# JiaoLab2021/varigraph

Measured on AMD Instinct MI355X. Metric: 150 bp reads/sec genotyped (k=27), higher is better.
Workload: dtype u64

## Files before the change

### include/vgmi.h

```cpp
#ifndef VGMI_H
#define VGMI_H

#include <stddef.h>
#include <stdint.h>

#ifdef __cplusplus
extern "C" {
#endif

typedef struct vgmi_ctx vgmi_ctx;

typedef enum vgmi_status {
    VGMI_OK = 0,
    VGMI_E_INVALID = -1,
    VGMI_E_NO_DEVICE = -2,
    VGMI_E_HIP = -3,
    VGMI_E_STATE = -4,
    VGMI_E_DUPLICATE_KEY = -5,
    VGMI_E_BAD_KEY = -6,
    VGMI_E_EMPTY_READ = -7,
    VGMI_E_NOMEM = -8
} vgmi_status;

int vgmi_device_count(void);
int vgmi_create(int device, size_t buffer_mib, vgmi_ctx **out);
void vgmi_destroy(vgmi_ctx *ctx);
const char *vgmi_last_error(const vgmi_ctx *ctx);
int vgmi_device_memory(vgmi_ctx *ctx, size_t *free_bytes, size_t *total_bytes);
void *vgmi_stream(vgmi_ctx *ctx);
int vgmi_device_of(vgmi_ctx *ctx, int *device);

int vgmi_table_upload(vgmi_ctx *ctx, const uint64_t *host_keys, size_t n_keys, uint32_t k);
int vgmi_table_image_bytes(vgmi_ctx *ctx, size_t *bytes);
int vgmi_table_export(vgmi_ctx *ctx, void *dev_dst, size_t bytes);
int vgmi_table_import(vgmi_ctx *ctx, const void *dev_src, size_t bytes);
int vgmi_table_clone(vgmi_ctx *dst, vgmi_ctx *src);
int vgmi_rccl_unique_id(void *id128);
int vgmi_table_broadcast(vgmi_ctx *ctx, int rank, int world, const void *id128);
typedef struct vgmi_comm vgmi_comm;
int vgmi_comm_create(int device, int rank, int world, const void *id128, vgmi_comm **out);
int vgmi_table_broadcast_comm(vgmi_ctx *ctx, vgmi_comm *comm);
int vgmi_table_snapshot(vgmi_ctx *ctx);
void vgmi_comm_destroy(vgmi_comm *comm);
int vgmi_table_info(vgmi_ctx *ctx, size_t *n_keys, uint32_t *k, size_t *n_slots, size_t *filter_bits);
int vgmi_table_lookup(vgmi_ctx *ctx, const uint64_t *host_keys, size_t n, uint32_t *index_out);
int vgmi_xtable_info(vgmi_ctx *ctx, size_t *n_lines, size_t *overflow_pairs);
int vgmi_ctable_info(vgmi_ctx *ctx, size_t *n_buckets, size_t *n_entries, size_t *n_unitigs, size_t *moved_entries,
                     size_t *overflow_kmers);
int vgmi_ctable_defer_info(vgmi_ctx *ctx, uint64_t *deferred_launches, uint64_t *plain_launches, uint32_t *n_bins,
                           uint32_t *region, uint32_t *room, uint32_t *cap);

int vgmi_nodes_upload(vgmi_ctx *ctx, const uint64_t *host_node_off, const uint32_t *host_key_index,
                      size_t n_nodes);
int vgmi_flags_upload(vgmi_ctx *ctx, const uint8_t *host_hom_flag);

int vgmi_counts_reset(vgmi_ctx *ctx);
int vgmi_reads_submit(vgmi_ctx *ctx, const char *host_bases, size_t n_bytes,
                      const uint64_t *host_read_off, size_t n_reads);
int vgmi_reads_submit_device(vgmi_ctx *ctx, const char *dev_bases, size_t n_bytes,
                             const uint64_t *dev_read_off, size_t n_reads);
int vgmi_read_base(vgmi_ctx *ctx, uint64_t *read_base);
int vgmi_counts_finish(vgmi_ctx *ctx, uint8_t *host_cov_out, uint8_t *host_cov_node_out,
                       uint64_t *host_hist256_out);
int vgmi_counts_finish_device(vgmi_ctx *ctx, uint8_t *dev_cov_out, uint8_t *dev_cov_node_out,
                              uint64_t *dev_hist256_out);
int vgmi_counts_export_device(vgmi_ctx *ctx, uint32_t *dev_counts_out );
int vgmi_counts_import_device(vgmi_ctx *ctx, const uint32_t *dev_counts );
int vgmi_count_kernel_ms(vgmi_ctx *ctx, float *ms, uint64_t *launches);

typedef struct vgmi_fastq vgmi_fastq;
int vgmi_fastq_open(vgmi_ctx *ctx, vgmi_fastq **out);
int vgmi_fastq_acquire(vgmi_fastq *fq, char **host_buf, size_t *capacity);
int vgmi_fastq_commit(vgmi_fastq *fq, size_t n_bytes);
int vgmi_fastq_text_capacity(vgmi_fastq *fq, size_t *text_bytes);
int vgmi_fastq_bgzf_want(vgmi_fastq *fq, size_t *comp_bytes);
int vgmi_fastq_commit_bgzf(vgmi_fastq *fq, size_t n_bytes, size_t *taken, size_t *n_text, int *not_bgzf);
int vgmi_fastq_open_bam(vgmi_ctx *ctx, uint64_t header_bytes, int32_t n_ref, vgmi_fastq **out);
int vgmi_fastq_open_fasta(vgmi_ctx *ctx, vgmi_fastq **out);
int vgmi_gunzip_buffer(vgmi_ctx *ctx, const void *host_gz, size_t n, void *host_out, size_t cap, size_t *n_out, size_t *consumed,
                       int *member_end, uint32_t *reason);
int vgmi_fastq_commit_gzip(vgmi_fastq *fq, size_t n_bytes, int at_eof, size_t *taken, size_t *n_text, int *stop);
int vgmi_fastq_gzip_status(vgmi_fastq *fq, uint64_t *device_text_bytes, uint32_t *reason);
int vgmi_fastq_bgzf_status(vgmi_fastq *fq, int *failed, uint64_t *good_compressed_bytes, uint32_t *reason);
int vgmi_fastq_close(vgmi_fastq *fq, uint64_t *n_records, uint64_t *n_bases, uint64_t *consumed_bytes, int *stopped,
                     char *tail_out, size_t tail_cap, size_t *tail_len);

int vgmi_sketch_keys(vgmi_ctx *ctx, const char *host_bases, size_t n_bytes,
                     const uint64_t *host_read_off, size_t n_reads, uint32_t k,
                     uint64_t *host_keys_out);

int vgmi_bloom_params(uint64_t n, double p, uint64_t *m, uint32_t *n_hash);
int vgmi_bloom_create(vgmi_ctx *ctx, uint64_t m, uint32_t n_hash, const uint64_t *host_seeds);
int vgmi_bloom_add_seq(vgmi_ctx *ctx, const char *host_bases, uint64_t len, uint32_t k);
int vgmi_bloom_add_seq_device(vgmi_ctx *ctx, const char *dev_bases, uint64_t len, uint32_t k);
int vgmi_bloom_fetch(vgmi_ctx *ctx, uint8_t *host_filter_out );
int vgmi_bloom_load(vgmi_ctx *ctx, const uint8_t *host_filter );
int vgmi_bloom_save_file(vgmi_ctx *ctx, const char *path);
int vgmi_bloom_load_file(vgmi_ctx *ctx, const char *path);
int vgmi_bloom_query(vgmi_ctx *ctx, const uint64_t *host_keys, size_t n, uint8_t *host_min_out,
                     uint8_t *host_all_nonzero_out);

typedef struct vgmi_hmm_chain {
    uint64_t first_step, n_steps;
    uint32_t keep_index, pad;
} vgmi_hmm_chain;
int vgmi_hmm_recursion(vgmi_ctx *ctx, uint32_t n_gt, uint32_t ploidy, const uint8_t *keep, uint32_t n_windows,
                       const void *obs, uint64_t n_rows, const uint32_t *row, const uint8_t *restart, const void *pow,
                       uint64_t n_steps, const void *uniform, const vgmi_hmm_chain *chains, uint32_t n_chains, void *out);
int vgmi_hmm_recursion_fre(vgmi_ctx *ctx, uint32_t n_gt, uint32_t ploidy, const void *freq, uint32_t n_tables, const void *obs,
                           uint64_t n_rows, const uint32_t *row, const uint8_t *restart, uint64_t n_steps, const void *uniform,
                           const vgmi_hmm_chain *chains, uint32_t n_chains, void *out);
int vgmi_hmm_calls(vgmi_ctx *ctx, uint32_t n_gt, uint32_t ploidy, const uint8_t *keep, uint32_t n_windows, const void *obs,
                   uint64_t n_rows, const uint32_t *row, const uint8_t *restart, const void *pow, uint64_t n_steps,
                   const void *uniform, const vgmi_hmm_chain *chains, uint32_t n_chains, const uint8_t *gid, const uint8_t *order,
                   const uint64_t *fwd_step, const uint64_t *bwd_step, void *prob, uint32_t *winner, void *alpha_beta_or_null);
int vgmi_hmm_calls_part(vgmi_ctx *ctx, uint32_t n_gt, uint32_t ploidy, const uint8_t *keep, uint32_t n_windows, const void *obs,
                        uint64_t row_lo, uint64_t row_hi, const uint32_t *row, const uint8_t *restart, const void *pow,
                        uint64_t step_lo, uint64_t step_hi, const void *uniform, const vgmi_hmm_chain *chains, uint32_t n_chains,
                        const uint8_t *gid, const uint8_t *order, const uint64_t *fwd_step, const uint64_t *bwd_step, void *prob,
                        uint32_t *winner);

typedef struct vgmi_hmm_part vgmi_hmm_part;
int vgmi_hmm_entries_upload(vgmi_ctx *ctx, const uint64_t *host_entries, size_t n_entries);
int vgmi_hmm_sample_upload(vgmi_ctx *ctx, const uint8_t *host_cov_node, size_t n_entries);
int vgmi_hmm_emissions(vgmi_ctx *ctx, uint32_t n_gt, uint32_t n_used, const uint8_t *used, const uint8_t *pos_a, const uint8_t *pos_b,
                       uint64_t top_mask, uint32_t bit_len, float ave, double lower, double upper, const void *tables,
                       uint64_t n_rows, const uint64_t *entry_begin, const uint32_t *entry_count, const uint16_t *gt0,
                       uint32_t *n_kept_out, uint8_t *flags_out, vgmi_hmm_part **out);
int vgmi_hmm_emissions_ploidy(vgmi_ctx *ctx, uint32_t n_gt, uint32_t ploidy, uint32_t n_used, const uint8_t *used, const uint8_t *pos,
                              uint64_t top_mask, uint32_t bit_len, float ave, double lower, double upper, const void *tables, uint64_t n_rows,
                              const uint64_t *entry_begin, const uint32_t *entry_count, const uint16_t *gt0, uint32_t *n_kept_out,
                              uint8_t *flags_out, vgmi_hmm_part **out);
int vgmi_hmm_part_set_rows(vgmi_hmm_part *part, uint64_t n, const uint64_t *rows, const void *obs_rows );
int vgmi_hmm_part_fix_rows(vgmi_hmm_part *part, uint64_t n, const uint64_t *rows, const uint32_t *fix_off, const uint32_t *fix_j,
                           const uint16_t *fix_mask);
int vgmi_hmm_part_calls(vgmi_hmm_part *part, uint32_t ploidy, const uint8_t *keep, uint32_t n_windows, const uint32_t *row,
                        const uint8_t *restart, const void *pow, uint64_t n_steps, const void *uniform, const vgmi_hmm_chain *chains,
                        uint32_t n_chains, const uint8_t *gid, const uint8_t *order, const uint64_t *fwd_step, const uint64_t *bwd_step,
                        void *prob, uint32_t *winner);
int vgmi_hmm_part_calls_fre(vgmi_hmm_part *part, uint32_t ploidy, const void *freq, uint32_t n_tables, const uint32_t *row,
                            const uint8_t *restart, uint64_t n_steps, const void *uniform, const vgmi_hmm_chain *chains, uint32_t n_chains,
                            const uint8_t *gid, const uint8_t *order, const uint64_t *fwd_step, const uint64_t *bwd_step, void *prob,
                            uint32_t *winner);
typedef struct vgmi_hmm_plan vgmi_hmm_plan;
int vgmi_hmm_plan_create(vgmi_ctx *ctx, uint32_t n_gt, uint32_t ploidy, const uint8_t *keep, uint32_t n_windows, uint64_t n_rows,
                         const uint32_t *row, const uint8_t *restart, const void *pow, uint64_t n_steps, const void *uniform,
                         const vgmi_hmm_chain *chains, uint32_t n_chains, const uint8_t *gid, const uint8_t *order, const uint64_t *fwd_step,
                         const uint64_t *bwd_step, vgmi_hmm_plan **out);
int vgmi_hmm_part_calls_plan(vgmi_hmm_part *part, const vgmi_hmm_plan *plan, void *prob, uint32_t *winner);
void vgmi_hmm_plan_free(vgmi_hmm_plan *plan);
int vgmi_hmm_tallies(vgmi_ctx *ctx, uint64_t n_rows, const uint64_t *entry_begin, const uint32_t *entry_count, const uint32_t *winner,
                     uint32_t n_gt, const uint8_t *hap_ab, uint32_t n_hap, uint64_t sel_mask, uint32_t *out, uint8_t *unique_out);
int vgmi_hmm_alive_upload(vgmi_ctx *ctx, const uint8_t *host_alive, size_t n_entries);
int vgmi_hmm_alive_fetch(vgmi_ctx *ctx, uint8_t *host_alive_out, size_t n_entries);
int vgmi_hmm_support(vgmi_ctx *ctx, uint32_t n_hap, uint32_t n_windows, uint64_t n_rows, const uint64_t *entry_begin,
                     const uint32_t *entry_count, const uint32_t *row_win, uint32_t *support_out );
int vgmi_hmm_emissions_select(vgmi_ctx *ctx, uint32_t n_gt, uint32_t n_used, const uint8_t *pos_a, const uint8_t *pos_b, uint32_t n_windows,
                              const uint8_t *win_used , const uint64_t *win_top_mask, uint32_t bit_len, float ave,
                              double lower, double upper, const void *tables, uint64_t n_rows, const uint64_t *entry_begin,
                              const uint32_t *entry_count, const uint32_t *row_win, const uint16_t *gt0, uint32_t *n_kept_out,
                              uint8_t *flags_out, vgmi_hmm_part **out);
int vgmi_hmm_tallies_select(vgmi_ctx *ctx, uint64_t n_rows, const uint64_t *entry_begin, const uint32_t *entry_count, const uint32_t *row_win,
                            const uint32_t *winner, uint32_t n_gt, const uint8_t *pos_a, const uint8_t *pos_b, uint32_t n_used,
                            uint32_t n_windows, const uint8_t *win_used, uint32_t *out, uint8_t *unique_out);
int vgmi_hmm_emissions_select_ploidy(vgmi_ctx *ctx, uint32_t n_gt, uint32_t ploidy, uint32_t n_windows, const uint32_t *win_n_gt,
                                     const uint8_t *win_haps , const uint64_t *win_top_mask, uint32_t bit_len,
                                     float ave, double lower, double upper, const void *tables, uint64_t n_rows, const uint64_t *entry_begin,
                                     const uint32_t *entry_count, const uint32_t *row_win, const uint64_t *gt0, uint32_t *n_kept_out,
                                     uint8_t *flags_out, vgmi_hmm_part **out);
int vgmi_hmm_part_fix_rows_wide(vgmi_hmm_part *part, uint64_t n, const uint64_t *rows, const uint32_t *fix_off, const uint32_t *fix_j,
                                const uint64_t *fix_mask);
int vgmi_hmm_tallies_ploidy(vgmi_ctx *ctx, uint32_t ploidy, uint32_t n_gt, uint32_t n_windows, const uint32_t *win_n_gt ,
                            const uint8_t *win_haps , const uint64_t *win_sel_mask ,
                            uint64_t n_rows, const uint64_t *entry_begin, const uint32_t *entry_count, const uint32_t *row_win ,
                            const uint32_t *winner, int use_alive, uint32_t *out , uint8_t *unique_out);
int vgmi_hmm_entries_upload_wide(vgmi_ctx *ctx, const uint8_t *f, const uint8_t *bits , size_t n_entries, uint32_t bit_len);
int vgmi_hmm_entries_reserve_wide(vgmi_ctx *ctx, size_t n_entries, uint32_t bit_len);
int vgmi_hmm_entries_fill_wide(vgmi_ctx *ctx, size_t first, size_t n, const uint8_t *f, const uint8_t *bits );
int vgmi_hmm_support_wide(vgmi_ctx *ctx, uint32_t bit_len, uint32_t n_hap, uint32_t n_windows, uint64_t n_rows, const uint64_t *entry_begin,
                          const uint32_t *entry_count, const uint32_t *row_win, uint32_t *support_out );
int vgmi_hmm_emissions_select_wide(vgmi_ctx *ctx, uint32_t n_gt, uint32_t n_used, const uint8_t *pos_a, const uint8_t *pos_b, uint32_t n_windows,
                                   const uint8_t *win_used , const uint64_t *win_top_mask ,
                                   uint32_t bit_len, float ave, double lower, double upper, const void *tables, uint64_t n_rows,
                                   const uint64_t *entry_begin, const uint32_t *entry_count, const uint32_t *row_win, const uint16_t *gt0,
                                   uint32_t *n_kept_out, uint8_t *flags_out, vgmi_hmm_part **out);
int vgmi_hmm_tallies_select_wide(vgmi_ctx *ctx, uint32_t bit_len, uint64_t n_rows, const uint64_t *entry_begin, const uint32_t *entry_count,
                                 const uint32_t *row_win, const uint32_t *winner, uint32_t n_gt, const uint8_t *pos_a, const uint8_t *pos_b,
                                 uint32_t n_used, uint32_t n_windows, const uint8_t *win_used, uint32_t *out, uint8_t *unique_out);
int vgmi_hmm_emissions_select_ploidy_wide(vgmi_ctx *ctx, uint32_t n_gt, uint32_t ploidy, uint32_t n_windows, const uint32_t *win_n_gt,
                                          const uint8_t *win_haps , const uint64_t *win_top_mask ,
                                          uint32_t bit_len, float ave, double lower, double upper, const void *tables, uint64_t n_rows,
                                          const uint64_t *entry_begin, const uint32_t *entry_count, const uint32_t *row_win,
                                          const uint64_t *gt0 , uint32_t *n_kept_out, uint8_t *flags_out, vgmi_hmm_part **out);
int vgmi_hmm_part_fix_rows_ploidy_wide(vgmi_hmm_part *part, uint64_t n, const uint64_t *rows, const uint32_t *fix_off, const uint32_t *fix_j,
                                       const uint64_t *fix_mask );
int vgmi_hmm_tallies_ploidy_wide(vgmi_ctx *ctx, uint32_t bit_len, uint32_t ploidy, uint32_t n_gt, uint32_t n_windows, const uint32_t *win_n_gt,
                                 const uint8_t *win_haps, const uint64_t *win_sel_mask , uint64_t n_rows,
                                 const uint64_t *entry_begin, const uint32_t *entry_count, const uint32_t *row_win, const uint32_t *winner,
                                 int use_alive, uint32_t *out , uint8_t *unique_out);
int vgmi_hmm_part_fetch(vgmi_hmm_part *part, void *obs_out);
void vgmi_hmm_part_free(vgmi_hmm_part *part);


#ifdef __cplusplus
}
#endif
#endif
```

### varigraph_amd/csrc/vgmi_api.cpp

```cpp
#include "vgmi_ctx.h"

namespace vgapi {

thread_local std::string g_create_error;

thread_local uint64_t t_err_ctx = 0;
thread_local std::string t_err_msg;

int fail(vgmi_ctx* c, int code, const std::string& msg)
{
    static std::mutex mu;
    std::lock_guard<std::mutex> lock(mu);
    if (c) {
        c->err = msg;
        t_err_ctx = c->id;
        t_err_msg = msg;
    } else g_create_error = msg;
    return code;
}

uint32_t ceil_log2(uint64_t x)
{
    uint32_t l = 0;
    while ((1ULL << l) < x) ++l;
    return l;
}

hipEvent_t get_event(vgmi_ctx* c)
{
    if (!c->event_pool.empty()) {
        hipEvent_t e = c->event_pool.back();
        c->event_pool.pop_back();
        return e;
    }
    hipEvent_t e = nullptr;
    if (hipEventCreate(&e) != hipSuccess) return nullptr;
    return e;
}

void free_table(vgmi_ctx* c)
{
    if (c->d_image) (void)hipFree(c->d_image);
    c->d_image = nullptr;
    if (c->d_snapshot) (void)hipFree(c->d_snapshot);
    c->d_snapshot = nullptr;
    c->image_bytes = 0;
    c->has_table = false;
    if (c->d_cov) (void)hipFree(c->d_cov);
    c->d_cov = nullptr;
    if (c->d_flag) (void)hipFree(c->d_flag);
    c->d_flag = nullptr;
    if (c->d_counts) (void)hipFree(c->d_counts);
    c->d_counts = nullptr;
    if (c->d_sat_dirty) (void)hipFree(c->d_sat_dirty);
    c->d_sat_dirty = nullptr;
    if (c->d_xt_lines) (void)hipFree(c->d_xt_lines);
    if (c->d_xt_counts) (void)hipFree(c->d_xt_counts);
    if (c->d_xt_id) (void)hipFree(c->d_xt_id);
    if (c->d_xt_over) (void)hipFree(c->d_xt_over);
    c->d_xt_over = nullptr;
    c->xt_over_keys = 0;
    if (c->d_ct_buckets && c->ct_vmm_bytes) {
        (void)hipMemUnmap(c->d_ct_buckets, c->ct_vmm_bytes);
        (void)hipMemRelease(c->ct_vmm_handle);
        (void)hipMemAddressFree(c->d_ct_buckets, c->ct_vmm_bytes);
        c->ct_vmm_bytes = 0;
    } else if (c->d_ct_buckets) (void)hipFree(c->d_ct_buckets);
    c->d_ct_buckets = nullptr;
    c->ct_entries = c->ct_unitigs = c->ct_moved = 0;
    for (void* q : {(void*)c->d_pt_index, (void*)c->d_pt_S, (void*)c->d_pt_VB, (void*)c->d_pt_SB, (void*)c->d_pt_SLOT, (void*)c->d_pt_PLACE})
        if (q) (void)hipFree(q);
    c->d_pt_index = nullptr;
    c->d_pt_S = c->d_pt_VB = c->d_pt_SB = c->d_pt_SLOT = c->d_pt_PLACE = nullptr;
    c->tv.pt = PathView{};
    c->d_xt_lines = nullptr;
    c->d_xt_counts = nullptr;
    c->d_xt_id = nullptr;
    c->tv.xt = XTableView{};
}

void free_nodes(vgmi_ctx* c)
{
    if (c->d_node_key_index) (void)hipFree(c->d_node_key_index);
    if (c->d_cov_node) (void)hipFree(c->d_cov_node);
    c->d_node_key_index = nullptr;
    c->d_cov_node = nullptr;
    c->n_nodes = 0;
    c->n_node_entries = 0;
}

int debit_list_of(vgmi_ctx* c, hipStream_t st, unsigned long long** out)
{
    {
        std::lock_guard<std::mutex> lk(c->mu);
        auto it = c->debit_lists.find(st);
        if (it != c->debit_lists.end()) {
            *out = it->second;
            return VGMI_OK;
        }
    }
    unsigned long long* list = nullptr;
    HIPCHK(c, hipMalloc(reinterpret_cast<void**>(&list), (size_t)VG_DEBIT_LIST * 8 + (size_t)VG_DEBIT_SUBLISTS * 64));
    std::lock_guard<std::mutex> lk(c->mu);
    c->debit_lists[st] = list;
    *out = list;
    return VGMI_OK;
}

int ctd_prepare(vgmi_ctx* c, size_t n_bytes, hipStream_t st, CtDefer* d)
{
    const char* const e_on = getenv("VGMI_CT_DEFER");
    const int on = e_on ? atoi(e_on) : VGMI_CT_DEFER_DEFAULT;
    const char* const e_min = getenv("VGMI_CT_DEFER_MIN");
    const size_t min_bytes = e_min ? (size_t)atoll(e_min) : (size_t)512 << 20;
    *d = CtDefer{};
    if (!on || !c->tv.xt.cb || n_bytes < min_bytes) return VGMI_OK;
    const size_t need = ctd_scratch_bytes(n_bytes, c->xt_n_counts, (uint32_t)c->n_cu, d);
    if (!need) return VGMI_OK;
    uint8_t* buf = nullptr;
    size_t have = 0;
    {
        std::lock_guard<std::mutex> lk(c->mu);
        auto it = c->ctd_scratch.find(st);
        if (it != c->ctd_scratch.end()) {
            buf = it->second.first;
            have = it->second.second;
        }
    }
    if (have < need) {
        if (buf) {
            HIPCHK(c, hipStreamSynchronize(st));
            (void)hipFree(buf);
            buf = nullptr;
        }
        if (hipMalloc(reinterpret_cast<void**>(&buf), need) != hipSuccess) {
            (void)hipGetLastError();
            std::lock_guard<std::mutex> lk(c->mu);
            c->ctd_scratch.erase(st);
            *d = CtDefer{};
            return VGMI_OK;
        }
        std::lock_guard<std::mutex> lk(c->mu);
        c->ctd_scratch[st] = std::make_pair(buf, need);
    }
    ctd_layout(buf, d);
    HIPCHK(c, launch_ctd_reset(*d, st));
    return VGMI_OK;
}

int launch_ctable_count(vgmi_ctx* c, const RowParams& p, size_t n_bytes, hipStream_t st)
{
    CtDefer d;
    int rc = ctd_prepare(c, n_bytes, st, &d);
    if (rc) return rc;
    {
        std::lock_guard<std::mutex> lk(c->mu);
        if (d.rec) {
            ++c->ctd_deferred;
            c->ctd_last[0] = d.n_bins, c->ctd_last[1] = d.region, c->ctd_last[2] = d.room, c->ctd_last[3] = d.cap;
        } else
            ++c->ctd_plain;
    }
    HIPCHK(c, launch_count27c(p, c->tv.xt, (uint32_t)c->n_cu, st, &d));
    if (d.rec) HIPCHK(c, launch_ctd_apply(c->tv.xt, d, (uint32_t)c->n_cu, st));
    return VGMI_OK;
}

int xt_clamp_if_due(vgmi_ctx* c, size_t n_bytes, hipStream_t st)
{
    bool due = false;
    {
        std::lock_guard<std::mutex> lk(c->mu);
        c->xt_bytes_since_clamp += n_bytes;
        if (c->xt_bytes_since_clamp >= (1ULL << 31)) {
            c->xt_bytes_since_clamp = 0;
            due = true;
        }
    }
    if (due) HIPCHK(c, launch_xclamp(c->tv.xt, c->xt_n_counts, st));
    return VGMI_OK;
}

}


uint32_t vgmi_dbg_env()
{
    static const uint32_t v = [] {
        const char* d = getenv("VGMI_DBG");
        const uint32_t x = d ? (uint32_t)atoi(d) : 0u;
#ifdef VGMI_ABLATION
        if (x) fprintf(stderr, "[vgmi] WARNING: VGMI_DBG=%u in an ablation build: counters and genotypes are WRONG on purpose\n", x);
        return x;
#else
        if (x) fprintf(stderr, "[vgmi] VGMI_DBG=%u ignored: this library was built without -DVGMI_ABLATION\n", x);
        return 0u;
#endif
    }();
    return v;
}

namespace vgapi {
RowParams row_params(vgmi_ctx* c, const char* d_bases, size_t n_bytes, uint32_t k)
{
    RowParams p{};
    p.bases = reinterpret_cast<const uint8_t*>(d_bases);
    p.n_bytes = n_bytes;
    p.k = k;
    p.status = c->d_status;
    p.table = c->tv;
    p.keys_out = nullptr;
    p.dbg = vgmi_dbg_env();
    static const uint32_t l1_min = [] {
        const char* e = getenv("VGMI_L1_MIN");
        const int v = e ? atoi(e) : 60;
        return (uint32_t)(v < 1 ? 1 : v > 64 ? 64 : v);
    }();
    p.l1_min = l1_min;
    p.bloom = c->bv;
    return p;
}

void rows_geometry(vgmi_ctx* c, bool flds, uint32_t& grid, uint32_t& block)
{
    if (flds) { block = 1024; grid = (uint32_t)c->n_cu; }
    else      { block = 256;  grid = (uint32_t)c->n_cu * 8; }
// ... 295 lines not shown
    if (!c) return VGMI_E_INVALID;
    if (!c->has_table) return fail(c, VGMI_E_STATE, "no table");
    if (n_bytes == 0) return VGMI_OK;
    if (!bases) return fail(c, VGMI_E_INVALID, "bases is NULL");
    if (bases[n_bytes - 1] != '\n') return fail(c, VGMI_E_INVALID, "a read block must end with '\\n'");
    if (n_reads > n_bytes) return fail(c, VGMI_E_INVALID, "n_reads > n_bytes");
    HIPCHK(c, hipSetDevice(c->device));
    const bool need_off = (c->hdr.k & 1) == 0;
    std::vector<uint64_t> derived;
    if (need_off && !read_off) {
        derived = offsets_from_newlines(bases, n_bytes);
        if (derived.size() != n_reads + 1) return fail(c, VGMI_E_INVALID, "n_reads does not match the number of '\\n'");
        read_off = derived.data();
    }
    size_t pos = 0, read_i = 0;
    while (pos < n_bytes) {
        size_t len = n_bytes - pos;
        size_t piece_reads = n_reads - read_i;
        if (len > c->buffer_bytes) {
            len = c->buffer_bytes;
            while (len > 0 && bases[pos + len - 1] != '\n') --len;
            if (len == 0) return fail(c, VGMI_E_INVALID, "a single read exceeds the staging buffer (--buffer)");
            if (need_off) {
                size_t j = read_i;
                while (read_off[j] < pos + len) ++j;
                piece_reads = j - read_i;
            } else {
                piece_reads = 0;
            }
        }
        Stage& s = c->stage[c->next_stage];
        c->next_stage ^= 1;
        int rc = ensure_stage(c, s);
        if (rc) return rc;
        if (s.busy) { HIPCHK(c, hipEventSynchronize(s.done)); s.busy = false; }
        if (s.after_reset) { HIPCHK(c, hipStreamWaitEvent(s.stream, c->reset_done, 0)); s.after_reset = false; }
        memcpy(s.h, bases + pos, len);
        HIPCHK(c, hipMemcpyAsync(s.d, s.h, len, hipMemcpyHostToDevice, s.stream));
        const uint64_t* d_off = nullptr;
        if (need_off) {
            if (s.d_off_cap < piece_reads + 1) {
                if (s.d_off) (void)hipFree(s.d_off);
                s.d_off_cap = (piece_reads + 1) * 2;
                HIPCHK(c, hipMalloc(reinterpret_cast<void**>(&s.d_off), s.d_off_cap * 8));
            }
            std::vector<uint64_t> rel(piece_reads + 1);
            for (size_t j = 0; j <= piece_reads; ++j) rel[j] = read_off[read_i + j] - pos;
            HIPCHK(c, hipMemcpy(s.d_off, rel.data(), rel.size() * 8, hipMemcpyHostToDevice));
            d_off = s.d_off;
        }
        rc = launch_count(c, s.d, len, d_off, piece_reads, s.stream);
        if (rc) return rc;
        HIPCHK(c, hipEventRecord(s.done, s.stream));
        s.busy = true;
        pos += len;
        read_i += piece_reads;
    }
    std::lock_guard<std::mutex> lk(c->mu);
    c->read_base += n_bytes - n_reads;
    return VGMI_OK;
}

int vgmi_read_base(vgmi_ctx* c, uint64_t* rb)
{
    if (!c || !rb) return VGMI_E_INVALID;
    *rb = c->read_base;
    return VGMI_OK;
}

static int finish_common(vgmi_ctx* c, uint8_t* d_cov, uint8_t* d_cov_node, unsigned long long* d_hist)
{
    for (auto& s : c->stage)
        if (s.busy) HIPCHK(c, hipStreamWaitEvent(c->stream, s.done, 0));
    if (d_hist) HIPCHK(c, hipMemsetAsync(d_hist, 0, 256 * 8, c->stream));
    if (c->tv.xt.counts) HIPCHK(c, launch_xcov(c->tv.xt, c->d_xt_id, c->hdr.n_keys, c->d_flag, d_cov, d_hist, c->stream));
    else HIPCHK(c, launch_cov(c->tv, c->d_key_slot, c->hdr.n_keys, c->d_flag, d_cov, d_hist, c->stream));
    if (d_cov_node && c->n_node_entries)
        HIPCHK(c, launch_node_gather(d_cov, c->d_node_key_index, c->n_node_entries, d_cov_node, c->stream));
    return VGMI_OK;
}

int vgmi_counts_finish(vgmi_ctx* c, uint8_t* cov_out, uint8_t* cov_node_out, uint64_t* hist_out)
{
    if (!c) return VGMI_E_INVALID;
    if (!c->has_table) return fail(c, VGMI_E_STATE, "no table");
    if (cov_node_out && !c->d_node_key_index) return fail(c, VGMI_E_STATE, "no nodes uploaded");
    if (hist_out && !c->d_flag) return fail(c, VGMI_E_STATE, "no flags uploaded");
    if (c->open_fastq) return fail(c, VGMI_E_STATE, "close the FASTQ streams first");
    HIPCHK(c, hipSetDevice(c->device));
    int rc = finish_common(c, c->d_cov, cov_node_out ? c->d_cov_node : nullptr, hist_out ? c->d_hist : nullptr);
    if (rc) return rc;
    if (cov_out && c->hdr.n_keys)
        HIPCHK(c, hipMemcpyAsync(cov_out, c->d_cov, c->hdr.n_keys, hipMemcpyDeviceToHost, c->stream));
    if (cov_node_out && c->n_node_entries)
        HIPCHK(c, hipMemcpyAsync(cov_node_out, c->d_cov_node, c->n_node_entries, hipMemcpyDeviceToHost, c->stream));
    if (hist_out) HIPCHK(c, hipMemcpyAsync(hist_out, c->d_hist, 256 * 8, hipMemcpyDeviceToHost, c->stream));
    HIPCHK(c, hipStreamSynchronize(c->stream));
    rc = sync_stages(c);
    if (rc) return rc;
    rc = collect_timing(c);
    if (rc) return rc;
    return check_status(c);
}

int vgmi_counts_finish_device(vgmi_ctx* c, uint8_t* dev_cov, uint8_t* dev_cov_node, uint64_t* dev_hist)
{
    if (!c) return VGMI_E_INVALID;
    if (!c->has_table) return fail(c, VGMI_E_STATE, "no table");
    if (dev_cov_node && !c->d_node_key_index) return fail(c, VGMI_E_STATE, "no nodes uploaded");
    if (dev_hist && !c->d_flag) return fail(c, VGMI_E_STATE, "no flags uploaded");
    HIPCHK(c, hipSetDevice(c->device));
    int rc = finish_common(c, dev_cov ? dev_cov : c->d_cov, dev_cov_node,
                           reinterpret_cast<unsigned long long*>(dev_hist));
    if (rc) return rc;
    HIPCHK(c, hipStreamSynchronize(c->stream));
    rc = sync_stages(c);
    if (rc) return rc;
    rc = collect_timing(c);
    if (rc) return rc;
    return check_status(c);
}

static int counts_xfer(vgmi_ctx* c, uint32_t* dev, bool import)
{
    if (!c || !dev) return VGMI_E_INVALID;
    if (!c->has_table) return fail(c, VGMI_E_STATE, "no table");
    if (reinterpret_cast<uintptr_t>(dev) & 3) return fail(c, VGMI_E_INVALID, "device pointer must be 4-byte aligned");
    HIPCHK(c, hipSetDevice(c->device));
    for (auto& s : c->stage)
        if (s.busy) HIPCHK(c, hipStreamWaitEvent(c->stream, s.done, 0));
    if (c->tv.xt.counts) HIPCHK(c, launch_xcounts_xfer(c->tv.xt, c->d_xt_id, dev, c->hdr.n_keys, import, c->stream));
    else HIPCHK(c, launch_counts_xfer(c->tv, c->d_key_slot, dev, c->hdr.n_keys, import, c->stream));
    HIPCHK(c, hipStreamSynchronize(c->stream));
    return VGMI_OK;
}

int vgmi_counts_export_device(vgmi_ctx* c, uint32_t* dev_counts_out) { return counts_xfer(c, dev_counts_out, false); }

int vgmi_counts_import_device(vgmi_ctx* c, const uint32_t* dev_counts)
{
    return counts_xfer(c, const_cast<uint32_t*>(dev_counts), true);
}

int vgmi_count_kernel_ms(vgmi_ctx* c, float* ms, uint64_t* launches)
{
    if (!c) return VGMI_E_INVALID;
    int rc = collect_timing(c);
    if (rc) return rc;
    if (ms) *ms = c->kernel_ms;
    if (launches) *launches = c->launches;
    return VGMI_OK;
}


int vgmi_sketch_keys(vgmi_ctx* c, const char* bases, size_t n_bytes, const uint64_t* read_off, size_t n_reads,
                     uint32_t k, uint64_t* keys_out)
{
    if (!c) return VGMI_E_INVALID;
    if (k < 1 || k > 28) return fail(c, VGMI_E_INVALID, "k must be in 1..28");
    if (n_bytes == 0) return VGMI_OK;
    if (!bases || !keys_out) return fail(c, VGMI_E_INVALID, "NULL buffer");
    if (bases[n_bytes - 1] != '\n') return fail(c, VGMI_E_INVALID, "a read block must end with '\\n'");
    HIPCHK(c, hipSetDevice(c->device));
    std::vector<uint64_t> derived;
    if (!(k & 1) && !read_off) {
        derived = offsets_from_newlines(bases, n_bytes);
        if (derived.size() != n_reads + 1) return fail(c, VGMI_E_INVALID, "n_reads does not match the number of '\\n'");
        read_off = derived.data();
    }
    char* d_b = nullptr;
    uint64_t* d_k = nullptr;
    uint64_t* d_off = nullptr;
    int rc = VGMI_OK;
    auto cleanup = [&]() {
        if (d_b) (void)hipFree(d_b);
        if (d_k) (void)hipFree(d_k);
        if (d_off) (void)hipFree(d_off);
    };
#define HIPCHK_CL(call) do { hipError_t ecl_ = (call); if (ecl_ != hipSuccess) { cleanup(); HIPCHK(c, ecl_); } } while (0)
    HIPCHK_CL(hipMalloc(reinterpret_cast<void**>(&d_b), n_bytes + 16));
    HIPCHK_CL(hipMalloc(reinterpret_cast<void**>(&d_k), n_bytes * 8));
    HIPCHK_CL(hipMemcpyAsync(d_b, bases, n_bytes, hipMemcpyHostToDevice, c->stream));
    HIPCHK_CL(hipMemsetAsync(c->d_status, 0, 4, c->stream));
    RowParams p = row_params(c, d_b, n_bytes, k);
    p.keys_out = d_k;
    if (k & 1) {
        uint32_t grid, block;
        rows_geometry(c, false, grid, block);
        HIPCHK_CL(launch_rows(K_MODE_KEYS, false, p, grid, block, c->stream));
    } else {
        HIPCHK_CL(hipMalloc(reinterpret_cast<void**>(&d_off), (n_reads + 1) * 8));
        HIPCHK_CL(hipMemcpyAsync(d_off, read_off, (n_reads + 1) * 8, hipMemcpyHostToDevice, c->stream));
        HIPCHK_CL(launch_seq(K_MODE_KEYS, p, d_off, n_reads, c->stream));
    }
    HIPCHK_CL(hipMemcpyAsync(keys_out, d_k, n_bytes * 8, hipMemcpyDeviceToHost, c->stream));
    HIPCHK_CL(hipStreamSynchronize(c->stream));
    rc = check_status(c);
    cleanup();
    return rc;
}

int vgmi_device_of(vgmi_ctx* c, int* device)
{
    if (!c || !device) return VGMI_E_INVALID;
    *device = c->device;
    return VGMI_OK;
}

int vgmi_device_memory(vgmi_ctx* c, size_t* free_bytes, size_t* total_bytes)
{
    if (!c) return VGMI_E_INVALID;
    HIPCHK(c, hipSetDevice(c->device));
    size_t f = 0, t = 0;
    HIPCHK(c, hipMemGetInfo(&f, &t));
    {
        std::lock_guard<std::mutex> lock(c->hmm_mu);
        for (const auto& b : c->hmm_blocks) f += b.second;
    }
    if (free_bytes) *free_bytes = f;
    if (total_bytes) *total_bytes = t;
    return VGMI_OK;
}

}
```

### varigraph_amd/csrc/vgmi_api_table.cpp

```cpp
#include "vgmi_ctx.h"

namespace vgapi {

void layout_image(ImageHeader& h, uint32_t k, uint64_t n_keys)
{
    memset(&h, 0, sizeof h);
    memcpy(h.magic, "VGMITBL1", 8);
    h.k = k;
    h.n_keys = n_keys;
    const bool smallk = k >= 19 && k <= 25 && n_keys <= VG_GRID_LDS_MAX_KEYS && !(getenv("VGMI_SMALLK") && getenv("VGMI_SMALLK")[0] == '0');
    const bool off_k = (getenv("VGMI_CTABLE_K") && getenv("VGMI_CTABLE_K")[0] == '0') || (getenv("VGMI_CTABLE") && getenv("VGMI_CTABLE")[0] == '0') ||
                       (getenv("VGMI_XTABLE") && getenv("VGMI_XTABLE")[0] == '0');
    const bool largek = ((k >= 19 && k <= 25 && n_keys > VG_GRID_LDS_MAX_KEYS) || ((k == 26 || k == 28) && n_keys > 0)) && n_keys < (1ULL << 31) - 16 && !off_k;
    const bool compact = (k == 27 || smallk || largek) && !getenv("VGMI_WIDE_SLOTS");
    h.slot_bytes = compact ? 8 : 16;
    uint64_t cap = 64;
    uint64_t lf_mul = compact ? 8 : 4;
    if (const char* e = getenv("VGMI_TABLE_MUL")) lf_mul = (uint64_t)atoi(e) > 1 ? (uint64_t)atoi(e) : 2;
    while (cap < lf_mul * n_keys) cap <<= 1;
    while (cap > (1ULL << 32) && cap / 2 >= 2 * n_keys) cap >>= 1;
    h.cap = cap;
    h.home_bucket_log2 = 0;
    if (k == 27 && n_keys > VG_GRID_LDS_MAX_KEYS) {
        h.home_bucket_log2 = 5;
// ... 323 lines not shown
        if (he == hipSuccess) he = hipMalloc(reinterpret_cast<void**>(&link2), n * 8);
        if (he == hipSuccess) he = hipMalloc(reinterpret_cast<void**>(&mark), n * 4);
        if (he == hipSuccess) he = hipMalloc(reinterpret_cast<void**>(&cursor), 8);
        if (he == hipSuccess) he = hipMalloc(reinterpret_cast<void**>(&c->d_xt_id), n * 4);
        if (he == hipSuccess) he = hipMemsetAsync(c->d_xt_id, 0xFF, n * 4, c->stream);
        if (he == hipSuccess) he = hipMemsetAsync(mark, 0, n * 4, c->stream);
        if (he == hipSuccess) he = hipMemsetAsync(cursor, 0, 8, c->stream);
        if (he == hipSuccess) he = launch_xtable_number(x, c->tv.slots8, c->d_key_slot, n, link, link2, c->d_xt_id, cursor, mark, c->d_status, c->stream);
        unsigned long long used = 0;
        if (he == hipSuccess) he = hipStreamSynchronize(c->stream);
        if (he == hipSuccess) he = hipMemcpy(&used, cursor, 8, hipMemcpyDeviceToHost);
        if (he == hipSuccess) he = hipMemcpy(&st, c->d_status, 4, hipMemcpyDeviceToHost);
        for (void* q : {(void*)link, (void*)link2, (void*)mark, (void*)cursor})
            if (q) (void)hipFree(q);
        HIPCHK(c, he);
        if ((st & 16u) || used != n) {
            (void)hipFree(c->d_xt_id);
            c->d_xt_id = nullptr;
            HIPCHK(c, hipMemsetAsync(c->d_status, 0, 4, c->stream));
        } else {
            rc = xtable_fill(c, x, c->d_xt_id);
            if (rc != VGMI_OK) return rc;
        }
    }
    c->tv.xt = x;
    return VGMI_OK;
}

int build_ptable(vgmi_ctx* c)
{
    const ImageHeader& h = c->hdr;
    c->tv.pt = PathView{};
    if (!(c->fast27_small || c->fastk_small) || h.n_keys == 0) return VGMI_OK;
    const uint32_t K = h.k;
    const uint32_t lead = K == 27 ? 15u : K - 12u;
    if (const char* e = getenv("VGMI_PTABLE"))
        if (e[0] == '0') return VGMI_OK;
    const uint64_t n = h.n_keys;
    uint32_t bucket_log2 = 13;
    while (bucket_log2 < 19 && (1ull << bucket_log2) < 8 * n) ++bucket_log2;
    uint32_t *key_of_slot = nullptr, *link = nullptr, *link2 = nullptr, *pos = nullptr, *mark = nullptr;
    unsigned long long* cursor = nullptr;
    ulonglong2* d_P = nullptr;
    hipError_t he = hipMalloc(reinterpret_cast<void**>(&key_of_slot), h.cap * 4);
    if (he == hipSuccess) he = hipMalloc(reinterpret_cast<void**>(&link), n * 8);
    if (he == hipSuccess) he = hipMalloc(reinterpret_cast<void**>(&link2), n * 8);
    if (he == hipSuccess) he = hipMalloc(reinterpret_cast<void**>(&pos), n * 4);
    if (he == hipSuccess) he = hipMalloc(reinterpret_cast<void**>(&mark), n * 4);
    if (he == hipSuccess) he = hipMalloc(reinterpret_cast<void**>(&cursor), 8);
    if (he == hipSuccess) he = hipMalloc(reinterpret_cast<void**>(&d_P), 2 * n * sizeof(ulonglong2));
    if (he == hipSuccess) he = hipMemsetAsync(pos, 0xFF, n * 4, c->stream);
    if (he == hipSuccess) he = hipMemsetAsync(mark, 0, n * 4, c->stream);
    if (he == hipSuccess) he = hipMemsetAsync(cursor, 0, 8, c->stream);
    if (he == hipSuccess) he = launch_ptable_order(c->tv, c->d_key_slot, n, key_of_slot, link, link2, pos, cursor, mark, c->d_status, c->stream);
    unsigned long long used = 0;
    uint32_t st = 0;
    if (he == hipSuccess) he = hipStreamSynchronize(c->stream);
    if (he == hipSuccess) he = hipMemcpy(&used, cursor, 8, hipMemcpyDeviceToHost);
    if (he == hipSuccess) he = hipMemcpy(&st, c->d_status, 4, hipMemcpyDeviceToHost);
    const bool ordered = !(st & 16u) && used == n;
    if (he == hipSuccess && (st & 16u)) he = hipMemsetAsync(c->d_status, 0, 4, c->stream);
    if (he == hipSuccess) he = launch_ptable_fill(c->tv, c->d_key_slot, ordered ? pos : nullptr, n, d_P, c->stream);
    std::vector<ulonglong2> P(2 * n);
    if (he == hipSuccess) he = hipStreamSynchronize(c->stream);
    if (he == hipSuccess) he = hipMemcpy(P.data(), d_P, 2 * n * sizeof(ulonglong2), hipMemcpyDeviceToHost);
    for (void* q : {(void*)key_of_slot, (void*)link, (void*)link2, (void*)pos, (void*)mark, (void*)cursor, (void*)d_P})
        if (q) (void)hipFree(q);
    HIPCHK(c, he);

    const uint64_t M54 = (1ULL << (2 * K)) - 1;
    std::vector<uint32_t> kpos(n);
    uint64_t chains = 0;
    for (uint64_t i = 0; i < n; ++i) {
        const uint64_t a = i ? (uint64_t)P[i - 1].x & M54 : 0, b = (uint64_t)P[i].x & M54;
        if (i == 0 || (b >> 2) != (a & (M54 >> 2))) ++chains;
        kpos[i] = (uint32_t)(i + (K - 1) * (chains - 1));
    }
    const uint64_t Th = n + (K - 1) * chains, T = 2 * Th, Tp = T + 64;
    if (Tp + 64 >= (1u << 19) - 1) return VGMI_OK;
    std::vector<uint8_t> base(Tp, 0), vb(Tp, 0);
    std::vector<uint32_t> slot(Tp, 0), chain_end(Tp, 0);
    {
        uint64_t span_start = 0;
        for (uint64_t i = 0; i < n; ++i) {
            const uint64_t km = (uint64_t)P[i].x & M54;
            for (uint32_t t = 0; t < K; ++t) base[32 + kpos[i] + t] = (uint8_t)((km >> (2 * (K - 1 - t))) & 3u);
            bool own_rc = false;
            if (!(K & 1u)) {
                uint64_t r = 0;
                for (uint32_t t = 0; t < K; ++t) r |= (3ull - ((km >> (2 * t)) & 3ull)) << (2 * (K - 1 - t));
                own_rc = r == km;
            }
            vb[32 + kpos[i]] = !own_rc;
            slot[32 + kpos[i]] = (uint32_t)P[i].y;
            vb[32 + T - K - kpos[i]] = !own_rc;
            slot[32 + T - K - kpos[i]] = (uint32_t)P[i].y;
            const bool last_of_chain = i + 1 == n || kpos[i + 1] != kpos[i] + 1;
            if (last_of_chain) {
                chain_end[span_start] = (uint32_t)(kpos[i] + K);
                span_start = kpos[i] + K;
            }
        }
        for (uint64_t j = 0; j < Th; ++j) base[32 + T - 1 - j] = (uint8_t)(3u - base[32 + j]);
        for (uint64_t j = 0; j < 32; ++j) base[Tp - 1 - j] = (uint8_t)(3u - base[j]);
    }
    const size_t s_words = (size_t)(Tp + 15) / 16 + 8, b_words = (size_t)(Tp + 31) / 32 + 4;
    std::vector<uint32_t> S(s_words, 0), VB(b_words, 0);
    for (uint64_t j = 0; j < Tp; ++j) {
        S[j >> 4] |= (uint32_t)base[j] << (2 * (15 - (j & 15)));
        if (vb[j]) VB[j >> 5] |= 1u << (j & 31);
    }
    std::vector<unsigned long long> index((size_t)4 << bucket_log2, 0ULL);
    uint64_t slow_cx = 0, bucket_ovf = 0;
    auto add = [&](uint32_t x, uint32_t place) {
        unsigned long long* B = &index[(size_t)(vg_idx_hash(x) >> (32 - bucket_log2)) << 2];
        for (int e = 0; e < 2; ++e) {
            unsigned long long& lo = B[2 * e];
            unsigned long long& hi = B[2 * e + 1];
            const uint32_t q0 = (uint32_t)(lo >> 24) & 0x7FFFFu, q1 = (uint32_t)(lo >> 43) & 0x7FFFFu;
            const uint32_t q2 = (uint32_t)hi & 0x7FFFFu, q3 = (uint32_t)(hi >> 19) & 0x7FFFFu;
            if (q0 == 0) {
                lo = (lo & (1ULL << 62)) | x | (unsigned long long)place << 24;
                return;
            }
            if (((uint32_t)lo & 0xFFFFFFu) != x) continue;
            if (q1 == 0) lo |= (unsigned long long)place << 43;
            else if (q2 == 0) hi |= place;
            else if (q3 == 0) hi |= (unsigned long long)place << 19;
            else if (!(hi >> 38 & 1)) {
                hi |= 1ULL << 38;
                ++slow_cx;
            }
            return;
        }
        if (!(B[0] >> 62 & 1)) ++bucket_ovf;
        B[0] |= 1ULL << 62;
    };
    for (uint64_t s0 = 0; s0 < Th;) {
        const uint64_t e0 = chain_end[s0];
        for (int halfno = 0; halfno < 2; ++halfno) {
            const uint64_t lo = halfno ? T - e0 : s0, hi = halfno ? T - s0 : e0;
            uint32_t x = 0;
            for (uint64_t b = lo; b < hi; ++b) {
                x = ((x << 2) | base[32 + b]) & 0xFFFFFFu;
                if (b + 1 < lo + 12) continue;
                const uint64_t first = b + 1 - 12;
                if (x <= vg_revcomp12(x)) add(x, (uint32_t)(32 + first - lead));
            }
        }
        s0 = e0;
    }
    c->pt_slow_cx = slow_cx;
    c->pt_bucket_ovf = bucket_ovf;
    he = hipMalloc(reinterpret_cast<void**>(&c->d_pt_index), index.size() * 8);
    if (he == hipSuccess) he = hipMalloc(reinterpret_cast<void**>(&c->d_pt_S), S.size() * 4);
    if (he == hipSuccess) he = hipMalloc(reinterpret_cast<void**>(&c->d_pt_VB), VB.size() * 4);
    const size_t pc_words = (size_t)Tp + 64;
    if (he == hipSuccess) he = hipMalloc(reinterpret_cast<void**>(&c->d_pt_SB), (VB.size() + pc_words) * 4);
    if (he == hipSuccess) he = hipMalloc(reinterpret_cast<void**>(&c->d_pt_SLOT), (size_t)(Tp + 64) * 4);
    if (he == hipSuccess) he = hipMemcpy(c->d_pt_index, index.data(), index.size() * 8, hipMemcpyHostToDevice);
    if (he == hipSuccess) he = hipMemcpy(c->d_pt_S, S.data(), S.size() * 4, hipMemcpyHostToDevice);
    if (he == hipSuccess) he = hipMemcpy(c->d_pt_VB, VB.data(), VB.size() * 4, hipMemcpyHostToDevice);
    if (he == hipSuccess) he = hipMemset(c->d_pt_SB, 0, (VB.size() + pc_words) * 4);
    if (he == hipSuccess) he = hipMemset(c->d_pt_SLOT, 0, (size_t)(Tp + 64) * 4);
    if (he == hipSuccess) he = hipMemcpy(c->d_pt_SLOT, slot.data(), (size_t)Tp * 4, hipMemcpyHostToDevice);
    {
        std::vector<uint32_t> place_of_slot(h.cap, 0u);
        for (uint64_t i = 0; i < n; ++i) place_of_slot[(uint32_t)P[i].y] = (uint32_t)(32 + kpos[i]);
        if (he == hipSuccess) he = hipMalloc(reinterpret_cast<void**>(&c->d_pt_PLACE), h.cap * 4);
        if (he == hipSuccess) he = hipMemcpy(c->d_pt_PLACE, place_of_slot.data(), h.cap * 4, hipMemcpyHostToDevice);
    }
    HIPCHK(c, he);
    c->pt_sb_bytes = (VB.size() + pc_words) * 4;
    if (getenv("VGMI_VERBOSE"))
        fprintf(stderr, "[vgmi] path table: %llu k-mers in %llu chains, %llu bases, %llu 12-mers with a fifth place, %llu buckets with a third 12-mer\n",
                (unsigned long long)n, (unsigned long long)chains, (unsigned long long)Tp, (unsigned long long)slow_cx, (unsigned long long)bucket_ovf);
    c->tv.pt.index = c->d_pt_index;
    c->tv.pt.S = c->d_pt_S;
    c->tv.pt.VB = c->d_pt_VB;
    c->tv.pt.SB = c->d_pt_SB;
    c->tv.pt.SLOT = c->d_pt_SLOT;
    c->tv.pt.PLACE = c->d_pt_PLACE;
    const char* pcv = getenv("VGMI_PT_POSCOUNT");
    c->tv.pt.PC = pcv && pcv[0] == '0' ? nullptr : c->d_pt_SB + VB.size();
    c->tv.pt.bucket_log2 = bucket_log2;
    c->tv.pt.Tp = (uint32_t)Tp;
    return VGMI_OK;
}

}

extern "C" {


int vgmi_table_upload(vgmi_ctx* c, const uint64_t* keys, size_t n_keys, uint32_t k)
{
    if (!c) return VGMI_E_INVALID;
    if (k < 1 || k > 28) return fail(c, VGMI_E_INVALID, "k must be in 1..28 (reference assert, kmer.cpp:124)");
    if (n_keys && !keys) return fail(c, VGMI_E_INVALID, "keys is NULL");
    if (n_keys >= (1ULL << 31)) return fail(c, VGMI_E_INVALID, "too many keys");
    HIPCHK(c, hipSetDevice(c->device));
    HIPCHK(c, hipStreamSynchronize(c->stream));
    free_table(c);
    layout_image(c->hdr, k, n_keys);
    c->image_bytes = c->hdr.total_bytes;
    HIPCHK(c, hipMalloc(reinterpret_cast<void**>(&c->d_image), c->image_bytes));
    HIPCHK(c, hipMemsetAsync(c->d_image, 0, c->image_bytes, c->stream));
    HIPCHK(c, hipMemcpyAsync(c->d_image, &c->hdr, sizeof c->hdr, hipMemcpyHostToDevice, c->stream));
    HIPCHK(c, hipMemsetAsync(c->d_status, 0, 4, c->stream));
    int rc = adopt_image(c);
    if (rc) return rc;
    HIPCHK(c, launch_table_clear(c->tv, c->stream));
    uint64_t* d_keys = nullptr;
    if (n_keys) {
        HIPCHK(c, hipMalloc(reinterpret_cast<void**>(&d_keys), n_keys * 8));
        HIPCHK(c, hipMemcpyAsync(d_keys, keys, n_keys * 8, hipMemcpyHostToDevice, c->stream));
        hipError_t e = launch_table_insert(c->tv, d_keys, n_keys, k, c->d_key_slot,
                                           const_cast<uint32_t*>(c->tv.filter), const_cast<uint32_t*>(c->tv.grid),
                                           c->hdr.grid_mer == 12, c->d_status, c->stream);
        if (e != hipSuccess) { (void)hipFree(d_keys); HIPCHK(c, e); }
    }
    hipError_t e = hipStreamSynchronize(c->stream);
    if (d_keys) (void)hipFree(d_keys);
    HIPCHK(c, e);
    rc = check_status(c);
    if (rc) { free_table(c); return rc; }
    rc = build_xtable(c);
    if (rc) { free_table(c); return rc; }
    rc = build_ptable(c);
    if (rc) { free_table(c); return rc; }
    c->read_base = 0;
    return VGMI_OK;
}

int vgmi_table_lookup(vgmi_ctx* c, const uint64_t* keys, size_t n, uint32_t* index_out)
{
    if (!c || (n && (!keys || !index_out))) return VGMI_E_INVALID;
    if (!c->has_table) return fail(c, VGMI_E_STATE, "no table");
    if (n == 0) return VGMI_OK;
    HIPCHK(c, hipSetDevice(c->device));
    const TableView tv = c->tv;
    const uint64_t cap = c->hdr.cap, n_keys = c->hdr.n_keys;
    const size_t chunk = std::min<size_t>(n, (size_t)1 << 25);
    hipStream_t st = nullptr;
    uint32_t* key_of_slot = nullptr;
    uint64_t* d_keys[2] = {nullptr, nullptr};
    uint32_t* d_out[2] = {nullptr, nullptr};
    hipEvent_t done[2] = {nullptr, nullptr};
    hipError_t he = hipStreamCreateWithFlags(&st, hipStreamNonBlocking);
    if (he == hipSuccess && tv.slots8) {
        he = hipMalloc(reinterpret_cast<void**>(&key_of_slot), cap * 4);
        if (he == hipSuccess) he = hipMemsetAsync(key_of_slot, 0xFF, cap * 4, st);
        if (he == hipSuccess) he = launch_table_key_of_slot(c->d_key_slot, n_keys, key_of_slot, st);
    }
    for (int b = 0; b < 2 && he == hipSuccess; ++b) {
        he = hipMalloc(reinterpret_cast<void**>(&d_keys[b]), chunk * 8);
        if (he == hipSuccess) he = hipMalloc(reinterpret_cast<void**>(&d_out[b]), chunk * 4);
        if (he == hipSuccess) he = hipEventCreateWithFlags(&done[b], hipEventDisableTiming);
    }
    size_t at[2] = {0, 0}, len[2] = {0, 0};
    auto collect = [&](int b) {
        if (he != hipSuccess || !len[b]) return;
        he = hipEventSynchronize(done[b]);
        len[b] = 0;
    };
    int b = 0;
    for (size_t off = 0; off < n && he == hipSuccess; off += chunk, b ^= 1) {
        collect(b);
        if (he != hipSuccess) break;
        at[b] = off;
        len[b] = std::min(chunk, n - off);
        he = hipMemcpyAsync(d_keys[b], keys + off, len[b] * 8, hipMemcpyHostToDevice, st);
        if (he == hipSuccess) he = launch_table_lookup(tv, d_keys[b], len[b], c->hdr.k, key_of_slot, d_out[b], st);
        if (he == hipSuccess) he = hipMemcpyAsync(index_out + off, d_out[b], len[b] * 4, hipMemcpyDeviceToHost, st);
        if (he == hipSuccess) he = hipEventRecord(done[b], st);
    }
    if (he == hipSuccess) he = hipStreamSynchronize(st);
    for (int q = 0; q < 2; ++q) {
        if (d_keys[q]) (void)hipFree(d_keys[q]);
        if (d_out[q]) (void)hipFree(d_out[q]);
        if (done[q]) (void)hipEventDestroy(done[q]);
    }
    if (key_of_slot) (void)hipFree(key_of_slot);
    if (st) (void)hipStreamDestroy(st);
    (void)at;
    HIPCHK(c, he);
    return VGMI_OK;
}

int vgmi_table_image_bytes(vgmi_ctx* c, size_t* bytes)
{
    if (!c || !bytes) return VGMI_E_INVALID;
    if (!c->has_table) return fail(c, VGMI_E_STATE, "no table");
    *bytes = c->image_bytes;
    return VGMI_OK;
}

int vgmi_table_export(vgmi_ctx* c, void* dev_dst, size_t bytes)
{
    if (!c || !dev_dst) return VGMI_E_INVALID;
    if (!c->has_table) return fail(c, VGMI_E_STATE, "no table");
    if (bytes < c->image_bytes) return fail(c, VGMI_E_INVALID, "destination smaller than the image");
    HIPCHK(c, hipSetDevice(c->device));
    HIPCHK(c, hipMemcpyAsync(dev_dst, c->d_image, c->image_bytes, hipMemcpyDeviceToDevice, c->stream));
    HIPCHK(c, hipStreamSynchronize(c->stream));
    return VGMI_OK;
}

int vgmi_table_snapshot(vgmi_ctx* c)
{
    if (!c) return VGMI_E_INVALID;
    if (!c->has_table) return fail(c, VGMI_E_STATE, "no table");
    HIPCHK(c, hipSetDevice(c->device));
    if (c->d_snapshot) (void)hipFree(c->d_snapshot);
    c->d_snapshot = nullptr;
    HIPCHK(c, hipMalloc(reinterpret_cast<void**>(&c->d_snapshot), c->image_bytes));
    HIPCHK(c, hipMemcpyAsync(c->d_snapshot, c->d_image, c->image_bytes, hipMemcpyDeviceToDevice, c->stream));
    HIPCHK(c, hipStreamSynchronize(c->stream));
    return VGMI_OK;
}

int vgmi_table_import(vgmi_ctx* c, const void* dev_src, size_t bytes)
{
    if (!c || !dev_src) return VGMI_E_INVALID;
    if (bytes < sizeof(ImageHeader)) return fail(c, VGMI_E_INVALID, "image too small");
    HIPCHK(c, hipSetDevice(c->device));
    HIPCHK(c, hipStreamSynchronize(c->stream));
    ImageHeader h;
    HIPCHK(c, hipMemcpy(&h, dev_src, sizeof h, hipMemcpyDeviceToHost));
    if (memcmp(h.magic, "VGMITBL1", 8) != 0 || h.total_bytes > bytes || h.k < 1 || h.k > 28)
        return fail(c, VGMI_E_INVALID, "not a table image");
    ImageHeader chk;
    layout_image(chk, h.k, h.n_keys);
    if (memcmp(&chk, &h, sizeof h) != 0) return fail(c, VGMI_E_INVALID, "table image layout mismatch");
    free_table(c);
    c->hdr = h;
    c->image_bytes = h.total_bytes;
// ... 100 lines not shown
```

### varigraph_amd/csrc/vgmi_ctx.h

```cpp
#ifndef VGMI_CTX_H
#define VGMI_CTX_H
#include "../../include/vgmi.h"

#include <dlfcn.h>
#include <hip/hip_runtime.h>

#include <atomic>
#include <chrono>
#include <cmath>
#include <cstdio>
#include <cstdlib>
#include <cstring>
#include <map>
#include <mutex>
#include <string>
#include <vector>

#include "vgmi_device.h"
#include "vgmi_kernels.h"

using namespace vgk;

struct ImageHeader {
    char magic[8];
    uint32_t k;
    uint32_t filter_words_log2;
    uint64_t n_keys;
    uint64_t cap;
    uint64_t off_slots, off_key_slot, off_filter, off_grid, total_bytes;
    uint32_t grid_words_log2;
    uint32_t slot_bytes;
    uint32_t home_bucket_log2;
    uint32_t home_by_offset;
    uint32_t grid_mer;
    uint8_t pad[256 - 8 - 4 - 4 - 8 - 8 - 40 - 8 - 4 - 4 - 4];
};
static_assert(sizeof(ImageHeader) == 256, "image header is 256 bytes");

struct Stage {
    char* h = nullptr;
    char* d = nullptr;
    uint64_t* d_off = nullptr;
    size_t d_off_cap = 0;
    hipStream_t stream = nullptr;
    hipEvent_t done = nullptr;
    bool busy = false;
    bool after_reset = false;
};

struct ncclUniqueIdBytes { char internal[128]; };

struct vgmi_ctx {
    uint64_t id = 0;
    int device = 0;
    int n_cu = 0;
    size_t buffer_bytes = 0;
    std::string err;
    hipStream_t stream = nullptr;
    unsigned long long* d_hmm_entries = nullptr;
    uint8_t* d_hmm_cov = nullptr;
    uint8_t* d_hmm_alive = nullptr;
    size_t hmm_n_entries = 0;
    uint8_t* d_hmm_f = nullptr;
    unsigned long long* d_hmm_bits = nullptr;
    uint32_t hmm_bit_len = 0, hmm_words = 0;
    std::mutex hmm_mu;
    std::vector<std::pair<uint8_t*, size_t>> hmm_blocks;

    uint8_t* d_image = nullptr;
    uint8_t* d_snapshot = nullptr;
    size_t image_bytes = 0;
    ImageHeader hdr{};
    bool has_table = false;
    TableView tv{};
    uint32_t* d_key_slot = nullptr;
    uint64_t xt_bytes_since_clamp = 0;
    uint64_t xt_n_counts = 0;
    unsigned long long* d_xt_lines = nullptr;
    uint32_t* d_xt_counts = nullptr;
    uint32_t* d_xt_id = nullptr;
    ulonglong2* d_xt_over = nullptr;
    uint4* d_ct_buckets = nullptr;
    size_t ct_vmm_bytes = 0;
    hipMemGenericAllocationHandle_t ct_vmm_handle{};
    uint64_t ct_entries = 0, ct_unitigs = 0, ct_moved = 0;
    unsigned long long* d_pt_index = nullptr;
    uint32_t *d_pt_S = nullptr, *d_pt_VB = nullptr, *d_pt_SB = nullptr, *d_pt_SLOT = nullptr, *d_pt_PLACE = nullptr;
    size_t pt_sb_bytes = 0;
    uint64_t pt_slow_cx = 0, pt_bucket_ovf = 0;
    uint64_t xt_over_keys = 0;
    uint8_t* d_sat_dirty = nullptr;
    uint64_t n_sat_regions = 0;
    uint32_t* d_counts = nullptr;
    uint64_t n_counts = 0;
    bool filter_in_lds = false;
    bool fast27 = false;
    bool fast27_lds = false;
    bool fast27_small = false;
    bool fastk_small = false;
    uint32_t wgs_per_cu = 0;
    bool force_generic = false;

    size_t n_nodes = 0;
    uint64_t n_node_entries = 0;
    uint32_t* d_node_key_index = nullptr;
    uint8_t* d_flag = nullptr;
    uint8_t* d_cov = nullptr;
    uint8_t* d_cov_node = nullptr;
    unsigned long long* d_hist = nullptr;
    uint32_t* d_status = nullptr;
    std::map<hipStream_t, std::pair<uint8_t*, size_t>> ctd_scratch;
    uint64_t ctd_deferred = 0, ctd_plain = 0;
    uint32_t ctd_last[4] = {0, 0, 0, 0};
    std::map<hipStream_t, unsigned long long*> debit_lists;

    std::mutex mu;
    int open_fastq = 0;
    std::vector<struct vgmi_fastq*> fastq_pool;
    uint64_t read_base = 0;
    hipEvent_t reset_done = nullptr;
    Stage stage[2];
    int next_stage = 0;
    std::vector<std::pair<hipEvent_t, hipEvent_t>> timed;
    std::vector<hipEvent_t> event_pool;
    float kernel_ms = 0.f;
    uint64_t launches = 0;

    bool has_bloom = false;
    uint8_t* bb_scratch = nullptr;
    size_t bb_cap = 0;
    BloomView bv{};
    uint64_t bloom_seeds64[VG_BLOOM_MAX_HASH] = {0};
    size_t bloom_alloc = 0;
};

namespace vgapi {

extern thread_local std::string g_create_error;
int fail(vgmi_ctx* c, int code, const std::string& msg);
uint32_t ceil_log2(uint64_t x);
hipEvent_t get_event(vgmi_ctx* c);
void free_table(vgmi_ctx* c);
void free_nodes(vgmi_ctx* c);
void layout_image(ImageHeader& h, uint32_t k, uint64_t n_keys);
int adopt_image(vgmi_ctx* c);
bool xtable_wanted(const ImageHeader& h);
bool ctable_wanted(const ImageHeader& h);
int launch_count(vgmi_ctx* c, const char* d_bases, size_t n_bytes, const uint64_t* d_read_off, size_t n_reads, hipStream_t st,
                 const unsigned long long* n_bytes_dev = nullptr, const unsigned long long* n_reads_dev = nullptr);
int collect_timing(vgmi_ctx* c);
int ensure_stage(vgmi_ctx* c, Stage& s);
int sync_stages(vgmi_ctx* c);
std::vector<uint64_t> offsets_from_newlines(const char* b, size_t n);
int check_status(vgmi_ctx* c);
RowParams row_params(vgmi_ctx* c, const char* d_bases, size_t n_bytes, uint32_t k);
void rows_geometry(vgmi_ctx* c, bool flds, uint32_t& grid, uint32_t& block);
void fastq_free(vgmi_fastq* f);

}
using namespace vgapi;

#define HIPCHK(c, call)                                                                            \
    do {                                                                                           \
        hipError_t e_ = (call);                                                                    \
        if (e_ != hipSuccess) {                                                                    \
            char b_[512];                                                                          \
            snprintf(b_, sizeof b_, "%s:%d: %s failed: %s", __FILE__, __LINE__, #call,             \
                     hipGetErrorString(e_));                                                       \
            return fail((c), VGMI_E_HIP, b_);                                                      \
        }                                                                                          \
    } while (0)

#endif
```

### varigraph_amd/csrc/vgmi_kernels.h

```cpp
#ifndef VGMI_KERNELS_H
#define VGMI_KERNELS_H
#include <hip/hip_runtime.h>
#include <stdint.h>

#include "vgmi_count_plan.h"
#include "vgmi_ctable.h"
#include "vgmi_device.h"

#ifdef VGMI_ABLATION
#define VG_DBG(x) (x)
#else
#define VG_DBG(x) 0u
#endif
uint32_t vgmi_dbg_env();

namespace vgk {

enum { K_MODE_COUNT = 0, K_MODE_KEYS = 1, K_MODE_BLOOM = 2, K_MODE_DEBIT = 3 };

#define XT_HOPS 3u
struct XTableView {
    unsigned long long* lines;
    uint32_t n_lines;
    uint32_t tag_bits;
    uint32_t id_shift;
    uint32_t* counts;
    const ulonglong2* over;
    uint32_t over_mask;
    const uint4* cb;
    uint32_t n_buckets;
    uint32_t k;
};

struct PathView {
    const unsigned long long* index;
    const uint32_t* S;
    const uint32_t* VB;
    uint32_t* SB;
    const uint32_t* SLOT;
    const uint32_t* PLACE;
    uint32_t* PC;
    uint32_t bucket_log2;
    uint32_t Tp;
};

struct TableView {
    VgSlot* slots;
    unsigned long long* slots8;
    uint64_t cap_mask;
    uint32_t k;
    uint32_t home_bucket_log2;
    uint32_t home_by_offset;
    const uint32_t* filter;
    uint32_t filter_words_log2;
    uint32_t filter_shift;
    const uint32_t* grid;
    uint32_t grid_words_log2;
    uint8_t* sat_dirty;
    XTableView xt;
    PathView pt;
    uint32_t* counts;
};

#define VG_BLOOM_MAX_HASH 32
struct BloomView {
    uint8_t* filter;
    uint64_t m;
    uint64_t magic;
    uint32_t n_hash;
    uint32_t seeds[VG_BLOOM_MAX_HASH];
};

struct RowParams {
    const uint8_t* bases;
    uint64_t n_bytes;
    uint64_t row_begin;
    uint64_t row_end;
    uint64_t emit_from;
    uint32_t k;
    uint32_t dbg;
    uint32_t* status;
    const unsigned long long* n_bytes_dev;
    uint32_t tail27;
    uint32_t l1_min;
    TableView table;
    uint64_t* keys_out;
    BloomView bloom;
};

struct FqState {
    unsigned long long n_records;
    unsigned long long n_bases;
    unsigned long long consumed;
    unsigned long long packed_bytes;
    uint32_t stopped;
    uint32_t tail_len;
    uint32_t start;
    uint32_t consumed_end;
    uint32_t n_lines, n_good, first_bad, dirty;
};
struct FqBuffers {
    const uint8_t* raw;
    uint8_t* raw_next;
    uint8_t* packed;
    uint32_t* tile;
    uint32_t* nlpos;
    uint32_t* rec_bytes;
    uint32_t* out_off;
    uint32_t* block_sum;
    FqState* state;
    uint32_t cap_lines, tail_max;
};
hipError_t launch_fastq_init(FqState* st, uint32_t tail_max, hipStream_t s);
hipError_t launch_fastq_chunk(const FqBuffers& b, uint32_t n_new, hipStream_t s, const uint32_t* n_new_dev = nullptr);
hipError_t launch_scan_small(uint32_t* v, uint32_t n, uint32_t* total, hipStream_t s);

hipError_t launch_fastq_lines(const FqBuffers& b, uint32_t n_new, hipStream_t s, const uint32_t* n_new_dev = nullptr);

struct FaBuffers {
    FqBuffers q;
    unsigned long long* total;
    unsigned long long* bsum;
    uint32_t* dest;
    uint32_t* rec_d;
    uint32_t* rec_pos;
};
__host__ __device__ inline uint32_t fasta_cap_rec(uint32_t cap_lines) { return cap_lines / 2u + 4u; }
hipError_t launch_fasta_chunk(const FaBuffers& b, uint32_t n_new, hipStream_t s, const uint32_t* n_new_dev = nullptr);

struct BamState {
    unsigned long long hdr_left;
    uint32_t n_cand;
    uint32_t last;
    uint32_t n_kept;
    uint32_t pad;
};
struct BamBuffers {
    const uint8_t* raw;
    uint8_t* raw_next;
    uint8_t* packed;
    uint32_t* tile;
    uint32_t* cand;
    uint32_t *j0, *ja, *jb;
    uint8_t* mark;
    uint32_t* rec_bytes;
    uint32_t* out_off;
    uint32_t* block_sum;
    FqState* state;
    BamState* bam;
    uint32_t cap_cand, tail_max;
    int32_t n_ref;
};
hipError_t launch_bam_init(BamState* bs, unsigned long long header_bytes, hipStream_t s);
hipError_t launch_bam_chunk(const BamBuffers& b, uint32_t n_new, hipStream_t s, const uint32_t* n_new_dev = nullptr);

struct BgzfMember {
    uint32_t c_off, c_len;
    uint32_t u_off, u_len;
    uint32_t crc, pad;
};
struct BgzfVerdict {
    uint32_t first_bad_batch, first_bad_member, reason;
    uint32_t good_bytes;
    uint32_t batches;
};
struct BloomBinPlan {
    int ok;
    uint32_t n_chunks, n_bins, n_sub, bin_shift, cap1, cap2;
    size_t scratch_bytes;
};
BloomBinPlan bloom_bin_plan(uint64_t m, uint32_t n_hash, uint64_t n_keys_max);
hipError_t launch_bloom_binned(const BloomView& b, const uint64_t* keys, uint64_t n_keys, const BloomBinPlan& plan, uint8_t* scratch, int n_cu, hipStream_t st,
                               int* overflowed);
uint32_t bgzf_wave_slots(int n_cu);
hipError_t launch_bgzf_inflate(const uint8_t* comp, const BgzfMember* members, uint32_t n_members, uint8_t* out_base, uint32_t* status,
                               const uint32_t* crc_table, BgzfVerdict* verdict, hipStream_t s);

struct GzSegHost {
    uint32_t start_bit, stop_bit, sym_off, sym_cap, win_avail, pad;
};
struct GzSegOutHost {
    uint32_t n_sym, end_bit, status, final_block;
};
hipError_t launch_gz_find(const uint8_t* comp, uint32_t n_bytes, uint32_t sub_bytes, uint32_t n_sub, uint32_t per, uint32_t* starts, hipStream_t st);
hipError_t launch_gz_decode(const uint8_t* comp, uint32_t n_bytes, const void* segs, uint32_t n_seg, uint16_t* pool, void* outs, hipStream_t st);
hipError_t launch_gz_resolve(const uint16_t* pool, const void* segs, const void* outs, const uint64_t* text_off, uint32_t n_seg, uint16_t* w1, uint8_t* t,
                             uint8_t* text, hipStream_t st);
uint32_t gz_groups(uint32_t n_seg);
struct GzCrcState {
    uint32_t r, pad;
    uint64_t len;
};
hipError_t launch_gz_crc(const uint8_t* text, uint64_t n, uint32_t* chunk_r, GzCrcState* state, hipStream_t st);
size_t gz_crc_chunks(size_t n_text);
uint32_t gz_crc_finish(uint32_t r, uint64_t len);

struct HmmChain {
// ... 6 lines not shown
    uint32_t n_gt, ploidy;
    const uint8_t* keep;
    const uint8_t* obs;
    const uint32_t* row;
    const uint8_t* restart;
    const uint8_t* pow;
    const uint8_t* uniform;
    const HmmChain* chains;
    uint8_t* out;
    uint32_t dbg;
};
hipError_t launch_hmm_recursion(const HmmParams& P, uint32_t n_chains, hipStream_t st);
struct HmmFreParams {
    uint32_t n_gt, ploidy;
    const uint8_t* freq;
    const uint8_t* obs;
    const uint32_t* row;
    const uint8_t* restart;
    const uint8_t* uniform;
    const HmmChain* chains;
    uint8_t* out;
};
hipError_t launch_hmm_recursion_fre(const HmmFreParams& P, uint32_t n_chains, hipStream_t st);
struct HmmPostParams {
    uint32_t n_gt;
    uint64_t row0;
    const uint8_t* ab;
    const uint64_t* fwd_step;
    const uint64_t* bwd_step;
    const uint8_t* gid;
    const uint8_t* order;
    uint8_t* prob;
    uint32_t* winner;
};
hipError_t launch_hmm_posterior(const HmmPostParams& P, uint64_t n_rows, hipStream_t st);
struct HmmEntries {
    const uint8_t* f;
    uint32_t W;
    const unsigned long long* words;
};
struct HmmEmitParams {
    HmmEntries ent;
    const uint8_t* cov;
    const uint64_t* entry_begin;
    const uint32_t* entry_count;
    const uint16_t* gt0;
    uint64_t row_lo;
    uint32_t n_gt, n_used, bl8;
    uint8_t used[16], pos_a[128], pos_b[128];
    uint8_t pos_more[6][128];
    uint32_t ploidy;
    unsigned long long top_mask;
    float ave;
    double lower, upper;
    const uint8_t* tables;
    uint8_t* obs;
    uint32_t* n_kept;
    uint8_t* flags;
    const uint64_t* fix_rows;
    const uint32_t* fix_off;
    const uint32_t* fix_j;
    const uint16_t* fix_mask;
    const uint32_t* row_win;
    const uint8_t* win_used;
    const unsigned long long* win_top_mask;
    uint8_t* alive;
};
hipError_t launch_hmm_emissions(const HmmEmitParams& P, uint64_t n_rows, hipStream_t st);
struct HmmEmitWinParams {
    HmmEntries ent;
    const uint8_t* cov;
    uint8_t* alive;
    const uint64_t* entry_begin;
    const uint32_t* entry_count;
    const uint32_t* row_win;
    const unsigned long long* gt0;
    uint32_t n_gt, ploidy, bl8;
    float ave;
    double lower, upper;
    const uint8_t* tables;
    const uint32_t* win_n_gt;
    const uint8_t* win_haps;
    const unsigned long long* win_top_mask;
    const unsigned long long* win_used_mask;
    uint8_t* obs;
    uint32_t* n_kept;
    uint8_t* flags;
    uint64_t n_items;
    const uint64_t* fix_rows;
    const uint32_t* fix_off;
    const uint32_t* fix_j;
    const unsigned long long* fix_mask;
};
hipError_t launch_hmm_emissions_win(const HmmEmitWinParams& P, hipStream_t st);
hipError_t launch_hmm_support(const HmmEntries& ent, const uint8_t* cov, const uint8_t* alive, const uint64_t* entry_begin, const uint32_t* entry_count,
                              const uint32_t* row_win, uint64_t n_rows, uint32_t n_hap, uint32_t* support, hipStream_t st);
hipError_t launch_hmm_tally_select(const HmmEntries& ent, const uint8_t* cov, const uint8_t* alive, const uint64_t* entry_begin, const uint32_t* entry_count,
                                   const uint32_t* row_win, const uint32_t* winner, const uint8_t* pos_ab, const uint8_t* win_used, uint32_t n_gt, uint64_t n_rows,
                                   uint32_t* out, uint8_t* uniq, hipStream_t st);
hipError_t launch_hmm_tally_ploidy(const HmmEntries& ent, const uint8_t* cov, const uint8_t* alive, const uint64_t* entry_begin, const uint32_t* entry_count,
                                   const uint32_t* row_win, const uint32_t* winner, const uint32_t* win_n_gt, const uint8_t* win_haps,
                                   const unsigned long long* win_sel_mask, uint32_t n_gt, uint32_t ploidy, uint32_t bl8, uint64_t n_rows, uint32_t* out, uint8_t* uniq,
                                   hipStream_t st);
hipError_t launch_hmm_scatter_rows(uint8_t* obs, const uint64_t* rows, const uint8_t* src, uint32_t n_gt, uint64_t n, hipStream_t st);
size_t hmm_lds_bytes(uint32_t n_gt, uint32_t ploidy);
hipError_t launch_hmm_tally(const unsigned long long* packed, const uint8_t* cov, const uint64_t* entry_begin, const uint32_t* entry_count, const uint32_t* winner,
                            const uint8_t* hap_ab, uint32_t n_gt, uint32_t n_hap, unsigned long long sel_mask, uint64_t n_rows, uint32_t* out, uint8_t* uniq,
                            hipStream_t st);

hipError_t launch_xtable_build(const XTableView& t, const unsigned long long* slots8, const uint32_t* key_slot, const uint32_t* id_of_key,
                               uint64_t n_keys, uint32_t* over_list, uint32_t over_cap, unsigned long long* over_n, hipStream_t st);
hipError_t launch_xtable_over(ulonglong2* over, uint32_t over_mask, const unsigned long long* slots8, const uint32_t* key_slot,
                              const uint32_t* id_of_key, const uint32_t* over_list, uint64_t n_over, hipStream_t st);
hipError_t launch_xtable_number(const XTableView& t, const unsigned long long* slots8, const uint32_t* key_slot, uint64_t n, uint32_t* link,
                                uint32_t* link2, uint32_t* id_of_key, unsigned long long* cursor, uint32_t* mark, uint32_t* status,
                                hipStream_t st);
hipError_t launch_count27x(const RowParams& p, const XTableView& t, uint32_t grid, hipStream_t st);
hipError_t launch_ctable_okmer(const TableView& t, const uint32_t* key_slot, uint32_t* pos_of_key, const uint32_t* link2, uint64_t n, bool identity,
                               unsigned long long* okmer, uint32_t* id_of_key, unsigned long long* n_unitigs, hipStream_t st);
hipError_t launch_ctable_build(const XTableView& t, const unsigned long long* okmer, uint64_t n_places, uint32_t* over_list, uint32_t over_cap,
                               unsigned long long* over_n, unsigned long long* n_moved, hipStream_t st);
hipError_t launch_ctable_over(ulonglong2* over, uint32_t over_mask, const unsigned long long* okmer, const uint32_t* over_list, uint64_t n_over,
                              uint32_t k, hipStream_t st);
#define CTD_CHUNK 256u
#ifndef VGMI_CT_DEFER_DEFAULT
#define VGMI_CT_DEFER_DEFAULT 1
#endif
#define CTD_MAX_BINS 2048u
struct CtDefer {
    uint2* rec;
    uint32_t cap;
    unsigned int* cursor;
    uint32_t n_bins, room;
    unsigned int* bin_cursor;
    uint32_t* binned;
    uint64_t n_counts;
    uint32_t region, inv;
    uint32_t n_wg;
};
hipError_t launch_count27c(const RowParams& p, const XTableView& t, uint32_t n_cu, hipStream_t st, const CtDefer* defer = nullptr);
size_t ctd_scratch_bytes(uint64_t n_bytes, uint64_t n_counts, uint32_t n_cu, CtDefer* layout);
void ctd_layout(uint8_t* scratch, CtDefer* d);
hipError_t launch_ctd_reset(const CtDefer& d, hipStream_t st);
hipError_t launch_ctd_apply(const XTableView& t, const CtDefer& d, uint32_t n_cu, hipStream_t st);
hipError_t launch_xclamp(const XTableView& t, uint64_t n, hipStream_t st);
hipError_t launch_xcov(const XTableView& t, const uint32_t* id_of_key, uint64_t n, const uint8_t* flag, uint8_t* cov, unsigned long long* hist,
                       hipStream_t st);
hipError_t launch_xcounts_xfer(const XTableView& t, const uint32_t* id_of_key, uint32_t* ext, uint64_t n, bool import, hipStream_t st);
hipError_t launch_count27(bool lds_bitmap, const RowParams& p, uint32_t grid, uint32_t block, hipStream_t st);
hipError_t launch_count27s(const RowParams& p, uint32_t grid, hipStream_t st);
hipError_t launch_ptable_order(const TableView& t, const uint32_t* key_slot, uint64_t n, uint32_t* key_of_slot, uint32_t* link, uint32_t* link2,
                               uint32_t* pos_of_key, unsigned long long* cursor, uint32_t* mark, uint32_t* status, hipStream_t st, uint32_t align = 1);
hipError_t launch_ptable_check(const uint32_t* pos_of_key, uint64_t n, uint64_t total, uint32_t* mark, uint32_t* status, hipStream_t st);
hipError_t launch_ptable_fill(const TableView& t, const uint32_t* key_slot, const uint32_t* pos_of_key, uint64_t n, ulonglong2* P, hipStream_t st);
hipError_t launch_rows(int mode, bool flds, const RowParams& p, uint32_t grid, uint32_t block, hipStream_t st);
hipError_t launch_bloom_even(const RowParams& p, hipStream_t st);
hipError_t launch_seq(int mode, const RowParams& p, const uint64_t* read_off, uint64_t n_reads, hipStream_t st, const unsigned long long* n_reads_dev = nullptr);
#define VG_DEBIT_LIST (1u << 20)
#define VG_DEBIT_SUBLISTS 256u
hipError_t launch_even_debit(const RowParams& p, const uint64_t* read_off, uint64_t n_reads, unsigned long long* list, uint32_t list_cap, hipStream_t st,
                             const unsigned long long* n_reads_dev = nullptr);
hipError_t launch_read_offsets(const uint8_t* packed, uint64_t n_bytes_bound, const unsigned long long* n_bytes_dev, uint32_t* tile, uint64_t* read_off,
                               uint64_t cap_reads, unsigned long long* n_reads_dev, hipStream_t st);
size_t read_offsets_tiles(uint64_t n_bytes_bound);
hipError_t launch_table_clear(const TableView& t, hipStream_t st);
hipError_t launch_table_insert(const TableView& t, const uint64_t* keys, uint64_t n, uint32_t k, uint32_t* key_slot,
                               uint32_t* filter_rw, uint32_t* grid_rw, bool grid12, uint32_t* status, hipStream_t st);
hipError_t launch_table_key_of_slot(const uint32_t* key_slot, uint64_t n, uint32_t* key_of_slot, hipStream_t st);
hipError_t launch_table_lookup(const TableView& t, const uint64_t* keys, uint64_t n, uint32_t k, const uint32_t* key_of_slot, uint32_t* out,
                               hipStream_t st);
hipError_t launch_counts_reset(const TableView& t, hipStream_t st);
hipError_t launch_cov(const TableView& t, const uint32_t* key_slot, uint64_t n, const uint8_t* flag,
                      uint8_t* cov, unsigned long long* hist, hipStream_t st);
hipError_t launch_counts_xfer(const TableView& t, const uint32_t* key_slot, uint32_t* ext, uint64_t n, bool import,
                              hipStream_t st);
hipError_t launch_node_gather(const uint8_t* cov, const uint32_t* key_index, uint64_t n, uint8_t* cov_node, hipStream_t st);
hipError_t launch_bloom_query(const BloomView& b, const uint64_t* keys, uint64_t n, uint8_t* min_out, uint8_t* nz_out,
                              hipStream_t st);

}
#endif
```

### varigraph_amd/csrc/vgmi_kernels.hip

```cpp
#include <hip/hip_runtime.h>
#include <stdint.h>

#include "vgmi_device.h"
#include "vgmi_kernels.h"
#include "vgmi_xtable.h"

namespace vgk {

__device__ __forceinline__ uint32_t funnel(uint32_t hi, uint32_t lo, uint32_t sh)
{
    return __builtin_amdgcn_alignbit(hi, lo, sh);
}

__device__ __forceinline__ uint32_t rc_word(uint32_t x)
{
    uint32_t r = __builtin_bitreverse32(x);
    r = ((r >> 1) & 0x55555555u) | ((r & 0x55555555u) << 1);
    return ~r;
}

__device__ __forceinline__ uint64_t mod_u64(uint64_t x, uint64_t m, uint64_t magic)
{
    uint64_t q = __umul64hi(x, magic);
    uint64_t r = x - q * m;
    while (r >= m) r -= m;
    return r;
}

__device__ __forceinline__ void bloom_inc(uint8_t* filter, uint64_t pos)
{
    uint32_t* w = reinterpret_cast<uint32_t*>(filter + (pos & ~3ULL));
    const uint32_t sh = (uint32_t)(pos & 3) * 8;
    uint32_t old = __hip_atomic_load(w, __ATOMIC_RELAXED, __HIP_MEMORY_SCOPE_AGENT);
    for (;;) {
        if (((old >> sh) & 0xFFu) == 0xFFu) return;
        const uint32_t prev = atomicCAS(w, old, old + (1u << sh));
        if (prev == old) return;
        old = prev;
    }
}

__device__ __forceinline__ void bloom_add_key(const BloomView& b, uint64_t key)
{
    for (uint32_t i = 0; i < b.n_hash; ++i) {
        const uint64_t pos = mod_u64(vg_murmur_sum(key, b.seeds[i]), b.m, b.magic);
        bloom_inc(b.filter, pos);
    }
}

__device__ __forceinline__ void bloom_add_key_n(const BloomView& b, uint64_t key, uint32_t n)
{
    for (uint32_t i = 0; i < b.n_hash; ++i) {
        const uint64_t pos = mod_u64(vg_murmur_sum(key, b.seeds[i]), b.m, b.magic);
        uint32_t* w = reinterpret_cast<uint32_t*>(b.filter + (pos & ~3ULL));
        const uint32_t sh = (uint32_t)(pos & 3) * 8;
        uint32_t old = __hip_atomic_load(w, __ATOMIC_RELAXED, __HIP_MEMORY_SCOPE_AGENT);
        for (;;) {
            const uint32_t v = (old >> sh) & 0xFFu;
            if (v == 0xFFu) break;
            const uint32_t nv = v + n > 255u ? 255u : v + n;
            const uint32_t prev = atomicCAS(w, old, (old & ~(0xFFu << sh)) | (nv << sh));
            if (prev == old) break;
            old = prev;
        }
    }
}

#define VG_BPRIV_CELLS 128u
__device__ __forceinline__ void bloom_add_wave(const BloomView& b, unsigned long long* cell_key, uint32_t* cell_cnt, bool active,
                                               uint64_t key)
{
    uint32_t slot = 0;
    bool owner = false;
    if (active) {
        slot = (uint32_t)((key * 0x9E3779B97F4A7C15ULL) >> 57);
        for (;;) {
            const unsigned long long old = atomicCAS(&cell_key[slot], ~0ULL, (unsigned long long)key);
            if (old == ~0ULL) { owner = true; break; }
            if (old == key) break;
            slot = (slot + 1) & (VG_BPRIV_CELLS - 1);
        }
        atomicAdd(&cell_cnt[slot], 1u);
    }
    __builtin_amdgcn_fence(__ATOMIC_ACQ_REL, "wavefront");
    __builtin_amdgcn_wave_barrier();
    if (owner) {
        const uint32_t n = cell_cnt[slot];
        cell_cnt[slot] = 0;
        cell_key[slot] = ~0ULL;
        bloom_add_key_n(b, key, n);
    }
    __builtin_amdgcn_fence(__ATOMIC_ACQ_REL, "wavefront");
    __builtin_amdgcn_wave_barrier();
}

__device__ __forceinline__ uint32_t* count_cell(const TableView& t, uint64_t s, uint32_t key_index)
{
    if (t.slots8) return &t.counts[s];
    return t.counts ? &t.counts[key_index] : &t.slots[s].count;
}

__device__ __forceinline__ uint32_t* pt_cell(const TableView& t, uint64_t s)
{
    if (!t.pt.PC) return nullptr;
    const uint32_t pos = t.pt.PLACE[s];
    if (pos == 0u) return nullptr;
    const uint32_t mir = t.pt.Tp - t.k - pos;
    return t.pt.PC + (pos < mir ? pos : mir);
}
__device__ __forceinline__ uint32_t pt_counted(const TableView& t, uint64_t s)
{
    const uint32_t* const pc = pt_cell(t, s);
    return pc ? *pc : 0u;
}

__device__ __forceinline__ uint64_t table_home(const TableView& t, uint64_t canon)
{
    if (t.home_bucket_log2) return vg_thash_local(canon, vg_revcomp(canon, 27), t.home_bucket_log2, t.home_by_offset != 0) & t.cap_mask;
    return vg_thash(canon) & t.cap_mask;
}

__device__ __forceinline__ void table_count(const TableView& t, uint64_t canon)
{
    if (t.xt.cb) {
        ct_count(t.xt, canon);
        return;
    }
    if (t.xt.lines) {
        xt_count(t.xt, canon, 0);
        return;
    }
    uint64_t s = table_home(t, canon);
    if (t.slots8) {
        for (;;) {
            const uint64_t c = t.slots8[s];
            if (c == VG_EMPTY) return;
            if ((c & VG_SLOT_KMER_MASK) == canon) {
                if (!(c & VG_SLOT_SAT) && atomicAdd(&t.counts[s], 1u) == 254u) {
                    atomicOr(reinterpret_cast<unsigned int*>(&t.slots8[s]) + 1, (unsigned int)(VG_SLOT_SAT >> 32));
                    if (t.sat_dirty) t.sat_dirty[s >> 11] = 1;
                    if (t.pt.PLACE) {
                        const uint32_t pos = t.pt.PLACE[s];
                        if (pos != 0u) {
                            const uint32_t mir = t.pt.Tp - t.k - pos;
                            atomicOr(&t.pt.SB[pos >> 5], 1u << (pos & 31u));
                            atomicOr(&t.pt.SB[mir >> 5], 1u << (mir & 31u));
                        }
                    }
                }
                return;
            }
            if (!(c & VG_SLOT_CHAIN)) return;
            s = (s + 1) & t.cap_mask;
        }
    }
    for (;;) {
        const uint4 v = *reinterpret_cast<const uint4*>(&t.slots[s]);
        const uint64_t c = ((uint64_t)v.y << 32) | v.x;
        if (c == VG_EMPTY) return;
        if ((c & VG_SLOT_KMER_MASK) == canon) {
            if (t.counts) atomicAdd(&t.counts[v.w], 1u);
            else if (v.z < 255u) atomicAdd(&t.slots[s].count, 1u);
            return;
        }
        if (!(c & VG_SLOT_CHAIN)) return;
        s = (s + 1) & t.cap_mask;
    }
}

__device__ __forceinline__ void table_debit(const TableView& t, uint64_t canon)
{
    if (t.xt.cb) {
        const uint32_t id = ct_find(t.xt, canon);
        if (id != 0xFFFFFFFFu) atomicSub(t.xt.counts + id, 1u);
        return;
    }
    if (!t.slots8) return;
    uint64_t s = table_home(t, canon);
    for (;;) {
        const uint64_t c = t.slots8[s];
        if (c == VG_EMPTY) return;
        if ((c & VG_SLOT_KMER_MASK) == canon) {
            atomicSub(&t.counts[s], 1u);
            return;
        }
        if (!(c & VG_SLOT_CHAIN)) return;
        s = (s + 1) & t.cap_mask;
    }
}

__device__ __forceinline__ bool filter_test_global(const TableView& t, uint64_t canon)
{
    const uint32_t w = t.filter[vg_fhash_word(canon) >> t.filter_shift];
    const uint32_t m = vg_fhash_bits(canon, t.filter_words_log2);
    return (w & m) == m;
}

enum { MODE_COUNT = 0, MODE_KEYS = 1, MODE_BLOOM = 2, MODE_DEBIT = 3 };

#define VG_QCAP 128u

__device__ __forceinline__ uint4 load_chunk(const uint8_t* bases, uint64_t n_bytes, uint64_t off)
{
    if (off + 16 <= n_bytes) return *reinterpret_cast<const uint4*>(bases + off);
    uint32_t w[4];
#pragma unroll
    for (int i = 0; i < 4; ++i) {
        uint32_t x = 0;
#pragma unroll
        for (int b = 0; b < 4; ++b) {
            const uint64_t o = off + 4 * i + b;
            const uint32_t c = o < n_bytes ? bases[o] : (uint32_t)'\n';
            x |= c << (8 * b);
        }
        w[i] = x;
    }
    return make_uint4(w[0], w[1], w[2], w[3]);
}

__device__ __forceinline__ void encode16(const uint4 raw, const uint8_t* lut, uint32_t& be, uint32_t& inv)
{
    const uint32_t w[4] = {raw.x, raw.y, raw.z, raw.w};
    uint32_t acc = 0, flags = 0;
#pragma unroll
    for (int i = 0; i < 4; ++i) {
#pragma unroll
        for (int b = 0; b < 4; ++b) {
            const uint8_t* e = lut + ((w[i] >> (8 * b)) & 0xFFu);
            acc = (acc << 2) | e[0];
            flags = (flags << 1) | e[256];
        }
    }
    be = acc;
    inv = __builtin_bitreverse32(flags) >> 16;
}

__device__ __forceinline__ void stage_lut(uint8_t* lut, uint32_t tid, uint32_t nthreads)
{
    for (uint32_t i = tid; i < 256; i += nthreads) {
        const uint32_t c = vg_nt4(i);
        lut[i] = (uint8_t)(c & 3u);
        lut[256 + i] = (uint8_t)(c >> 2);
    }
}

template <int MODE>
__device__ __forceinline__ void drain_queue(const TableView& t, uint64_t* queue, uint32_t head, uint32_t n, uint32_t lane)
{
    __builtin_amdgcn_fence(__ATOMIC_ACQ_REL, "wavefront");
    if (lane < n) {
        const uint64_t canon = queue[(head + lane) & (VG_QCAP - 1)];
        table_count(t, canon);
    }
    __builtin_amdgcn_fence(__ATOMIC_ACQ_REL, "wavefront");
}

template <int MODE, bool FLDS>
__global__ __launch_bounds__(1024) void rows_kernel(RowParams p)
{
    extern __shared__ __attribute__((aligned(16))) uint8_t smem[];
    const uint32_t tid = threadIdx.x;
    const uint32_t lane = tid & 63u;
    const uint32_t wave = tid >> 6;
    const uint32_t nwaves = blockDim.x >> 6;

    size_t off = 0;
    uint32_t* s_filter = reinterpret_cast<uint32_t*>(smem);
    if (FLDS) off += (size_t)4 << p.table.filter_words_log2;
    uint64_t* s_queue = reinterpret_cast<uint64_t*>(smem + off) + (size_t)wave * VG_QCAP;
    if (MODE == MODE_COUNT) off += (size_t)nwaves * VG_QCAP * 8;
    unsigned long long* s_bkey = reinterpret_cast<unsigned long long*>(smem + off) + (size_t)wave * VG_BPRIV_CELLS;
    if (MODE == MODE_BLOOM) off += (size_t)nwaves * VG_BPRIV_CELLS * 8;
    uint32_t* s_bcnt = reinterpret_cast<uint32_t*>(smem + off) + (size_t)wave * VG_BPRIV_CELLS;
    if (MODE == MODE_BLOOM) off += (size_t)nwaves * VG_BPRIV_CELLS * 4;
    if (MODE == MODE_BLOOM)
        for (uint32_t i = lane; i < VG_BPRIV_CELLS; i += 64) {
            s_bkey[i] = ~0ULL;
            s_bcnt[i] = 0;
        }
    uint8_t* s_lut = smem + off;
    stage_lut(s_lut, tid, blockDim.x);
    if (FLDS) {
        const uint32_t nq = 1u << (p.table.filter_words_log2 - 2);
        const uint4* src = reinterpret_cast<const uint4*>(p.table.filter);
        uint4* dst = reinterpret_cast<uint4*>(s_filter);
        for (uint32_t i = tid; i < nq; i += blockDim.x) dst[i] = src[i];
    }
    __syncthreads();

    uint64_t n_bytes = p.n_bytes, row_begin = p.row_begin, emit_from = p.emit_from;
    if (p.n_bytes_dev) {
        n_bytes = *p.n_bytes_dev;
        emit_from = vg_row_split(p.tail27, n_bytes).emit_from;
        row_begin = emit_from >> 10;
        if (emit_from >= n_bytes) return;
    }
    const uint64_t total_rows = (n_bytes + 1023) >> 10;
    if (row_begin >= total_rows) return;
    const uint64_t span = total_rows - row_begin;
// ... 31 lines not shown
        uint32_t be, inv;
        encode16(raw, s_lut, be, inv);
        const uint32_t rcw = rc_word(be);
        const uint32_t r1_be = __shfl(be, src1), r2_be = __shfl(be, src2);
        const uint32_t r1_rc = __shfl(rcw, src1), r2_rc = __shfl(rcw, src2);
        const uint32_t r1_inv = __shfl(inv, src1), r2_inv = __shfl(inv, src2);
        const uint32_t F0 = be;
        const uint32_t F1 = lane >= 1 ? r1_be : pr1_be;
        const uint32_t F2 = lane >= 2 ? r2_be : pr2_be;
        const uint32_t R2 = rcw;
        const uint32_t R1 = lane >= 1 ? r1_rc : pr1_rc;
        const uint32_t R0 = lane >= 2 ? r2_rc : pr2_rc;
        const uint32_t i1 = lane >= 1 ? r1_inv : pr1_inv;
        const uint32_t i2 = lane >= 2 ? r2_inv : pr2_inv;
        pr1_be = r1_be; pr2_be = r2_be; pr1_rc = r1_rc; pr2_rc = r2_rc; pr1_inv = r1_inv; pr2_inv = r2_inv;

        uint64_t sm = ((uint64_t)inv << 32) | ((uint64_t)i1 << 16) | (uint64_t)i2;
        {
            uint32_t span = 1;
            while (2 * span <= K) { sm |= sm << span; span *= 2; }
            if (span < K) sm |= sm << (K - span);
        }
        const uint32_t bad = (uint32_t)(sm >> 32);

        {
            const uint32_t prev_bit = (i1 >> 15) & 1u;
            const uint32_t adj = inv & ((inv << 1) | prev_bit);
            if (__builtin_expect(__ballot(adj != 0) != 0, 0)) {
                if (adj) {
                    const uint64_t base_off = (r << 10) + lane * 16;
                    for (uint32_t t = 0; t < 16; ++t) {
                        if (!((adj >> t) & 1u)) continue;
                        const uint64_t o = base_off + t;
                        if (o >= n_bytes) continue;
                        if (p.bases[o] == '\n' && (o == 0 || p.bases[o - 1] == '\n')) atomicOr(p.status, 1u);
                    }
                }
            }
        }
        for (uint32_t j = 0; j < 16; ++j) {
            const uint32_t fs = 2 * (15 - j);
            const uint32_t f_lo = funnel(F1, F0, fs) & mask_lo;
            const uint32_t f_hi = funnel(F2, F1, fs) & mask_hi;
            const uint32_t rs = rc_off + 2 * j;
            uint32_t r_lo, r_hi;
            if (rs < 32) {
                r_lo = funnel(R1, R0, rs);
                r_hi = funnel(R2, R1, rs);
            } else if (rs < 64) {
                r_lo = funnel(R2, R1, rs - 32);
                r_hi = R2 >> (rs - 32);
            } else {
                r_lo = R2 >> (rs - 64);
                r_hi = 0;
            }
            r_lo &= mask_lo;
            r_hi &= mask_hi;
            const uint64_t fwd = ((uint64_t)f_hi << 32) | f_lo;
            const uint64_t rc = ((uint64_t)r_hi << 32) | r_lo;
            const uint64_t canon = fwd < rc ? fwd : rc;
            const bool valid = ((bad >> j) & 1u) == 0;

            if (MODE == MODE_KEYS) {
                const uint64_t pos = (r << 10) + lane * 16 + j;
                if (pos < n_bytes) p.keys_out[pos] = valid ? (vg_hash64(canon, mask) << 8 | K) : ~0ULL;
            } else if (MODE == MODE_BLOOM) {
                const uint64_t pos = (r << 10) + lane * 16 + j;
                if (VG_DBG(p.dbg) & 128u) {
                    if (valid && pos < n_bytes) bloom_add_key(p.bloom, vg_hash64(canon, mask) << 8 | K);
                } else {
                    bloom_add_wave(p.bloom, s_bkey, s_bcnt, valid && pos < n_bytes, vg_hash64(canon, mask) << 8 | K);
                }
            } else {
                const bool emit = valid && (r << 10) + lane * 16 + j >= emit_from;
                bool pass;
                if (FLDS) {
                    const uint32_t h = vg_fhash_word(canon);
                    const uint32_t w = s_filter[h >> p.table.filter_shift];
                    const uint32_t m = vg_fhash_bits_small(h);
                    pass = emit && ((w & m) == m);
                } else {
                    pass = emit && filter_test_global(p.table, canon);
                }
                const uint64_t ball = __ballot(pass);
                if (ball) {
                    if (pass) {
                        const uint32_t rank = __builtin_amdgcn_mbcnt_hi((uint32_t)(ball >> 32),
                                              __builtin_amdgcn_mbcnt_lo((uint32_t)ball, 0u));
                        s_queue[(qtail + rank) & (VG_QCAP - 1)] = canon;
                    }
                    qtail += (uint32_t)__popcll(ball);
                    if (qtail - qhead >= 64u) {
                        drain_queue<MODE>(p.table, s_queue, qhead, 64u, lane);
                        qhead += 64u;
                    }
                }
            }
        }
    }
    if (MODE == MODE_COUNT) {
        if (qtail != qhead) drain_queue<MODE>(p.table, s_queue, qhead, qtail - qhead, lane);
    }
}

#define VG_Q_KMER_MASK ((1ULL << 54) - 1)
#define VG_SAT_REGION_LOG2 11u
#define VG_RUNQ 80u
#define VG_RUN_BATCH 5u
#define VG_REQ 64u

#define VG_HOT_CLOBBERS "v116", "v117", "v118", "v120", "v121", "v122", "v123", "v124", "v125", "v126", "v127"
#define VG_HOT_CLOBBERS_S "v116", "v117", "v118", "v119", "v120", "v121", "v122", "v123", "v124", "v125", "v126", "v127"

template <int R>
__device__ __forceinline__ void vm_load_row(const uint8_t* ptr)
{
    if (R == 0) asm volatile("global_load_dwordx3 v[116:118], %0, off nt ; VGHOT" : : "v"(ptr) : VG_HOT_CLOBBERS);
    else asm volatile("global_load_dwordx3 v[120:122], %0, off nt ; VGHOT" : : "v"(ptr) : VG_HOT_CLOBBERS);
}
template <int R>
__device__ __forceinline__ void vms_load_row(const uint8_t* ptr)
{
    if (R == 0) asm volatile("global_load_dwordx4 v[116:119], %0, off nt ; VGHOT" : : "v"(ptr) : VG_HOT_CLOBBERS_S);
    else asm volatile("global_load_dwordx4 v[120:123], %0, off nt ; VGHOT" : : "v"(ptr) : VG_HOT_CLOBBERS_S);
}
__device__ __forceinline__ void vms_load_slot(const void* ptr)
{
    asm volatile("global_load_dwordx2 v[124:125], %0, off ; VGHOT" : : "v"(ptr) : VG_HOT_CLOBBERS_S);
}
__device__ __forceinline__ void vms_atomic_inc(uint32_t* ptr, uint32_t one)
{
    asm volatile("global_atomic_add v126, %0, %1, off sc0 ; VGHOT" : : "v"(ptr), "v"(one) : "memory", VG_HOT_CLOBBERS_S);
}
__device__ __forceinline__ uint2 vms_slot_value()
{
    uint2 v;
    asm volatile("v_mov_b32 %0, v124 ; VGHOT\n\tv_mov_b32 %1, v125 ; VGHOT" : "=v"(v.x), "=v"(v.y));
    return v;
}
__device__ __forceinline__ uint32_t vms_atomic_old()
{
    uint32_t v;
    asm volatile("v_mov_b32 %0, v126 ; VGHOT" : "=v"(v));
    return v;
}

#define VG_HOT_CLOBBERS_P "v76", "v77", "v78", "v79", "v80", "v81", "v82", "v83", "v84", "v85", "v86", "v87", "v88", "v89", "v90", "v91", \
                          "v92", "v93", "v94", "v95", "v96", "v97", "v98", "v99", "v100", "v101", "v102", "v103", "v104", "v105", "v106", "v107", \
                          "v108", "v109", "v110", "v111", "v112", "v113", "v114", "v115", VG_HOT_CLOBBERS_S
__device__ __forceinline__ void vmp_load_index(const void* ptr)
{
    asm volatile("global_load_dwordx4 v[108:111], %0, off ; VGHOT\n\tglobal_load_dwordx4 v[112:115], %0, off offset:16 ; VGHOT" : : "v"(ptr) : VG_HOT_CLOBBERS_P);
}
#define VG_SEQ_ASM(C, SQ, VBR, SBR) \
    if (c == C) asm volatile("global_load_dwordx4 " SQ ", %0, off ; VGHOT\n\tglobal_load_dwordx2 " VBR ", %1, off ; VGHOT\n\tglobal_load_dwordx2 " SBR ", %2, off ; VGHOT" \
                             : : "v"(sq), "v"(vb), "v"(sb) : VG_HOT_CLOBBERS_P)
template <int c>
__device__ __forceinline__ void vmp_load_place(const void* sq, const void* vb, const void* sb)
{
    VG_SEQ_ASM(0, "v[92:95]", "v[76:77]", "v[78:79]");
    VG_SEQ_ASM(1, "v[96:99]", "v[80:81]", "v[82:83]");
    VG_SEQ_ASM(2, "v[100:103]", "v[84:85]", "v[86:87]");
    VG_SEQ_ASM(3, "v[104:107]", "v[88:89]", "v[90:91]");
}
#define VG_MOV4(A, B, C, D) asm volatile("v_mov_b32 %0, " A " ; VGHOT\n\tv_mov_b32 %1, " B " ; VGHOT\n\tv_mov_b32 %2, " C " ; VGHOT\n\tv_mov_b32 %3, " D " ; VGHOT" \
                                         : "=v"(v.x), "=v"(v.y), "=v"(v.z), "=v"(v.w))
template <int e>
__device__ __forceinline__ uint4 vmp_index_value()
{
    uint4 v;
    if (e == 0) VG_MOV4("v108", "v109", "v110", "v111");
    else VG_MOV4("v112", "v113", "v114", "v115");
    return v;
}
template <int c>
__device__ __forceinline__ uint4 vmp_seq_value()
{
    uint4 v;
    if (c == 0) VG_MOV4("v92", "v93", "v94", "v95");
    if (c == 1) VG_MOV4("v96", "v97", "v98", "v99");
    if (c == 2) VG_MOV4("v100", "v101", "v102", "v103");
    if (c == 3) VG_MOV4("v104", "v105", "v106", "v107");
    return v;
}
template <int c>
__device__ __forceinline__ uint4 vmp_bits_value()
{
    uint4 v;
    if (c == 0) VG_MOV4("v76", "v77", "v78", "v79");
    if (c == 1) VG_MOV4("v80", "v81", "v82", "v83");
    if (c == 2) VG_MOV4("v84", "v85", "v86", "v87");
    if (c == 3) VG_MOV4("v88", "v89", "v90", "v91");
    return v;
}
__device__ __forceinline__ void vm_load_dword4_sync(const uint32_t* base, const uint32_t (&idx)[4], uint32_t (&v)[4])
{
    const uint32_t o0 = idx[0] << 2, o1 = idx[1] << 2, o2 = idx[2] << 2, o3 = idx[3] << 2;
    asm volatile("global_load_dword %0, %4, %8 ; VGHOT\n\tglobal_load_dword %1, %5, %8 ; VGHOT\n\tglobal_load_dword %2, %6, %8 ; VGHOT\n\t"
                 "global_load_dword %3, %7, %8 ; VGHOT\n\ts_waitcnt vmcnt(0) ; VGHOT"
                 : "=&v"(v[0]), "=&v"(v[1]), "=&v"(v[2]), "=&v"(v[3]) : "v"(o0), "v"(o1), "v"(o2), "v"(o3), "s"(base) : "memory", VG_HOT_CLOBBERS_P);
}
__device__ __forceinline__ void vm_atomic_add4_sync(uint32_t* base, const uint32_t (&idx)[4], const uint32_t (&add)[4], uint32_t (&old)[4])
{
    const uint32_t o0 = idx[0] << 2, o1 = idx[1] << 2, o2 = idx[2] << 2, o3 = idx[3] << 2;
    asm volatile("global_atomic_add %0, %4, %8, %12 sc0 ; VGHOT\n\tglobal_atomic_add %1, %5, %9, %12 sc0 ; VGHOT\n\t"
                 "global_atomic_add %2, %6, %10, %12 sc0 ; VGHOT\n\tglobal_atomic_add %3, %7, %11, %12 sc0 ; VGHOT\n\ts_waitcnt vmcnt(0) ; VGHOT"
                 : "=&v"(old[0]), "=&v"(old[1]), "=&v"(old[2]), "=&v"(old[3])
                 : "v"(o0), "v"(o1), "v"(o2), "v"(o3), "v"(add[0]), "v"(add[1]), "v"(add[2]), "v"(add[3]), "s"(base) : "memory", VG_HOT_CLOBBERS_P);
}
__device__ __forceinline__ void vm_atomic_inc4_masked_sync(uint32_t* base, const uint32_t (&off)[4], uint32_t one, uint32_t (&old)[4])
{
    unsigned long long sv;
    asm volatile("s_mov_b64 %[sv], exec ; VGHOT\n\t"
                 "v_cmp_ne_u32_e32 vcc, -1, %[o0] ; VGHOT\n\ts_and_b64 exec, %[sv], vcc ; VGHOT\n\tglobal_atomic_add %[r0], %[o0], %[one], %[b] sc0 ; VGHOT\n\t"
                 "s_mov_b64 exec, %[sv] ; VGHOT\n\tv_cmp_ne_u32_e32 vcc, -1, %[o1] ; VGHOT\n\ts_and_b64 exec, %[sv], vcc ; VGHOT\n\tglobal_atomic_add %[r1], %[o1], %[one], %[b] sc0 ; VGHOT\n\t"
                 "s_mov_b64 exec, %[sv] ; VGHOT\n\tv_cmp_ne_u32_e32 vcc, -1, %[o2] ; VGHOT\n\ts_and_b64 exec, %[sv], vcc ; VGHOT\n\tglobal_atomic_add %[r2], %[o2], %[one], %[b] sc0 ; VGHOT\n\t"
                 "s_mov_b64 exec, %[sv] ; VGHOT\n\tv_cmp_ne_u32_e32 vcc, -1, %[o3] ; VGHOT\n\ts_and_b64 exec, %[sv], vcc ; VGHOT\n\tglobal_atomic_add %[r3], %[o3], %[one], %[b] sc0 ; VGHOT\n\t"
                 "s_mov_b64 exec, %[sv] ; VGHOT\n\ts_waitcnt vmcnt(0) ; VGHOT"
                 : [sv] "=&s"(sv), [r0] "+v"(old[0]), [r1] "+v"(old[1]), [r2] "+v"(old[2]), [r3] "+v"(old[3])
                 : [o0] "v"(off[0]), [o1] "v"(off[1]), [o2] "v"(off[2]), [o3] "v"(off[3]), [one] "v"(one), [b] "s"(base) : "vcc", "memory", VG_HOT_CLOBBERS_P);
}
__device__ __forceinline__ uint32_t vm_load_dword_sync(const uint32_t* ptr)
{
    uint32_t v;
    asm volatile("global_load_dword %0, %1, off ; VGHOT\n\ts_waitcnt vmcnt(0) ; VGHOT" : "=&v"(v) : "v"(ptr) : "memory");
    return v;
}
__device__ __forceinline__ uint32_t vm_atomic_inc_sync(uint32_t* ptr, uint32_t one)
{
    uint32_t old;
    asm volatile("global_atomic_add %0, %1, %2, off sc0 ; VGHOT\n\ts_waitcnt vmcnt(0) ; VGHOT" : "=&v"(old) : "v"(ptr), "v"(one) : "memory");
    return old;
}
__device__ __forceinline__ void vm_wait4(uint32_t n)
{
    asm volatile("s_cmp_lt_u32 %0, 4 ; VGHOT\n\t"
                 "s_cbranch_scc1 1f ; VGHOT\n\t"
                 "s_waitcnt vmcnt(4) ; VGHOT\n\t"
                 "s_branch 9f ; VGHOT\n"
                 "1:\n\t"
                 "s_cmp_lt_u32 %0, 2 ; VGHOT\n\t"
                 "s_cbranch_scc1 2f ; VGHOT\n\t"
                 "s_cmp_eq_u32 %0, 2 ; VGHOT\n\t"
                 "s_cbranch_scc1 3f ; VGHOT\n\t"
                 "s_waitcnt vmcnt(3) ; VGHOT\n\t"
                 "s_branch 9f ; VGHOT\n"
                 "3:\n\t"
                 "s_waitcnt vmcnt(2) ; VGHOT\n\t"
                 "s_branch 9f ; VGHOT\n"
                 "2:\n\t"
                 "s_cmp_eq_u32 %0, 0 ; VGHOT\n\t"
                 "s_cbranch_scc1 4f ; VGHOT\n\t"
                 "s_waitcnt vmcnt(1) ; VGHOT\n\t"
                 "s_branch 9f ; VGHOT\n"
                 "4:\n\t"
                 "s_waitcnt vmcnt(0) ; VGHOT\n"
                 "9:"
                 : : "s"(__builtin_amdgcn_readfirstlane((int)n)) : "scc", "memory");
}

template <bool COMPACT>
__device__ __forceinline__ void vm_load_slot(const void* ptr)
{
    if (COMPACT) asm volatile("global_load_dwordx2 v[124:125], %0, off ; VGHOT" : : "v"(ptr) : VG_HOT_CLOBBERS);
    else asm volatile("global_load_dwordx4 v[124:127], %0, off ; VGHOT" : : "v"(ptr) : VG_HOT_CLOBBERS);
}
__device__ __forceinline__ void vm_atomic_inc(uint32_t* ptr, uint32_t one)
{
    asm volatile("global_atomic_add v123, %0, %1, off sc0 ; VGHOT" : : "v"(ptr), "v"(one) : "memory", VG_HOT_CLOBBERS);
}
template <int N>
__device__ __forceinline__ void vm_wait_imm()
{
    asm volatile("s_waitcnt vmcnt(%0) ; VGHOT" : : "n"(N) : "memory");
}
__device__ __forceinline__ void vm_wait(uint32_t n)
{
    asm volatile("s_cmp_lt_u32 %0, 2 ; VGHOT\n\t"
                 "s_cbranch_scc1 1f ; VGHOT\n\t"
                 "s_waitcnt vmcnt(2) ; VGHOT\n\t"
                 "s_branch 3f ; VGHOT\n"
                 "1:\n\t"
                 "s_cmp_eq_u32 %0, 0 ; VGHOT\n\t"
                 "s_cbranch_scc1 2f ; VGHOT\n\t"
                 "s_waitcnt vmcnt(1) ; VGHOT\n\t"
                 "s_branch 3f ; VGHOT\n"
                 "2:\n\t"
                 "s_waitcnt vmcnt(0) ; VGHOT\n"
                 "3:"
                 : : "s"(__builtin_amdgcn_readfirstlane((int)n)) : "scc", "memory");
}
template <bool COMPACT>
__device__ __forceinline__ uint4 vm_load_slot_sync(const void* ptr)
{
    if (COMPACT) {
        typedef uint32_t u32x2_t __attribute__((ext_vector_type(2)));
        u32x2_t v;
        asm volatile("global_load_dwordx2 %0, %1, off ; VGHOT\n\ts_waitcnt vmcnt(0) ; VGHOT" : "=&v"(v) : "v"(ptr) : "memory");
        return make_uint4(v.x, v.y, 0u, 0u);
    }
    typedef uint32_t u32x4_t __attribute__((ext_vector_type(4)));
    u32x4_t v;
    asm volatile("global_load_dwordx4 %0, %1, off ; VGHOT\n\ts_waitcnt vmcnt(0) ; VGHOT" : "=&v"(v) : "v"(ptr) : "memory");
    return make_uint4(v.x, v.y, v.z, v.w);
}
__device__ __forceinline__ uint32_t vm_load_byte_sync(const uint8_t* ptr)
{
    uint32_t v;
    asm volatile("global_load_ubyte %0, %1, off ; VGHOT\n\ts_waitcnt vmcnt(0) ; VGHOT" : "=&v"(v) : "v"(ptr) : "memory");
    return v;
}
__device__ __forceinline__ void vm_atomic_or_sync(uint32_t* ptr, uint32_t bits)
{
    asm volatile("global_atomic_or %0, %1, off ; VGHOT\n\ts_waitcnt vmcnt(0) ; VGHOT" : : "v"(ptr), "v"(bits) : "memory");
}
__device__ __forceinline__ void vm_store_byte_sync(uint8_t* ptr, uint32_t v)
{
    asm volatile("global_store_byte %0, %1, off ; VGHOT\n\ts_waitcnt vmcnt(0) ; VGHOT" : : "v"(ptr), "v"(v) : "memory");
}
template <bool COMPACT>
__device__ __forceinline__ uint4 vm_slot_value()
{
    uint4 v = make_uint4(0u, 0u, 0u, 0u);
    if (COMPACT) asm volatile("v_mov_b32 %0, v124 ; VGHOT\n\tv_mov_b32 %1, v125 ; VGHOT" : "=v"(v.x), "=v"(v.y));
    else asm volatile("v_mov_b32 %0, v124 ; VGHOT\n\tv_mov_b32 %1, v125 ; VGHOT\n\tv_mov_b32 %2, v126 ; VGHOT\n\tv_mov_b32 %3, v127 ; VGHOT"
                      : "=v"(v.x), "=v"(v.y), "=v"(v.z), "=v"(v.w));
    return v;
}
__device__ __forceinline__ uint32_t vm_atomic_old()
{
    uint32_t v;
    asm volatile("v_mov_b32 %0, v123 ; VGHOT" : "=v"(v));
    return v;
}

#define VG_ROW27 768u

#define VG_LUT27_BYTES 4096u
typedef __attribute__((address_space(3))) const uint16_t lds_u16;
typedef __attribute__((address_space(3))) const uint32_t lds_u32;

__device__ __forceinline__ void stage_lut27(uint32_t tid, uint32_t nthreads)
{
    typedef __attribute__((address_space(3))) uint16_t lds_u16_rw;
    for (uint32_t i = tid; i < 2048; i += nthreads) {
        const uint32_t set = i >> 10, b = (i >> 8) & 3u, c = vg_nt4(i & 255u);
        reinterpret_cast<lds_u16_rw*>((uintptr_t)0)[i] =
            (uint16_t)(((c & 3u) << (2 * (3 - b))) | ((c >> 2) << ((set ? 12 : 8) + b)));
    }
}

struct Addr4 { uint32_t a0, a1, a2, a3; };

#define VG_SDWA_X2(REG, B) "v_lshlrev_b32_sdwa %" #B ", %4, " REG " dst_sel:DWORD dst_unused:UNUSED_PAD src0_sel:DWORD src1_sel:BYTE_" #B " ; VGHOT\n\t"
#define VG_SDWA_ROW(REG) asm volatile(VG_SDWA_X2(REG, 0) VG_SDWA_X2(REG, 1) VG_SDWA_X2(REG, 2) VG_SDWA_X2(REG, 3) \
                                      : "=&v"(a.a0), "=&v"(a.a1), "=&v"(a.a2), "=&v"(a.a3) : "v"(one))
template <int R, int D>
__device__ __forceinline__ Addr4 lut_addr4(const uint32_t one)
{
    Addr4 a;
    if (R == 0 && D == 0) VG_SDWA_ROW("v116");
    if (R == 0 && D == 1) VG_SDWA_ROW("v117");
    if (R == 0 && D == 2) VG_SDWA_ROW("v118");
    if (R == 1 && D == 0) VG_SDWA_ROW("v120");
    if (R == 1 && D == 1) VG_SDWA_ROW("v121");
    if (R == 1 && D == 2) VG_SDWA_ROW("v122");
    return a;
}

template <int R, int D>
__device__ __forceinline__ Addr4 luts_addr4(const uint32_t one)
{
    Addr4 a;
    if (R == 0 && D == 0) VG_SDWA_ROW("v116");
    if (R == 0 && D == 1) VG_SDWA_ROW("v117");
    if (R == 0 && D == 2) VG_SDWA_ROW("v118");
    if (R == 0 && D == 3) VG_SDWA_ROW("v119");
    if (R == 1 && D == 0) VG_SDWA_ROW("v120");
    if (R == 1 && D == 1) VG_SDWA_ROW("v121");
    if (R == 1 && D == 2) VG_SDWA_ROW("v122");
    if (R == 1 && D == 3) VG_SDWA_ROW("v123");
    return a;
}

// ... 220 lines not shown
                if (vm_load_byte_sync(bases + o) == '\n' && (o == 0 || vm_load_byte_sync(bases + o - 1) == '\n'))
                    vm_atomic_or_sync(p.status, 1u);
            }
        }
    };

    const uint32_t n_it = (uint32_t)(r1 - rs), n_warm = (uint32_t)(r0 - rs);
    const uint8_t* rowp = bases + rs * (2 * VG_ROW27);
    vm_load_row<0>(rowp + lane_off);
    vm_load_row<1>(rowp + VG_ROW27 + lane_off);
    for (uint32_t it = 0; it < n_it; ++it) {
        vm_wait(n_after_row);
        const Addr4 a0 = lut_addr4<0, 0>(one), a1 = lut_addr4<0, 1>(one), a2 = lut_addr4<0, 2>(one);
        const Addr4 c0 = lut_addr4<1, 0>(one), c1 = lut_addr4<1, 1>(one), c2 = lut_addr4<1, 2>(one);
        const uint8_t* const cur = rowp;
        if (it + 1 < n_it) rowp += 2 * VG_ROW27;
        vm_load_row<0>(rowp + lane_off);
        vm_load_row<1>(rowp + VG_ROW27 + lane_off);
        n_after_row = 0;
        n_after_slot += 2;
        if (run_n >= VG_RUN_BATCH || req_n >= 32u) drain_step();

        const uint32_t g0 = encode4<0>(a0), g1 = encode4<1>(a1), g2 = encode4<0>(a2);
        const uint32_t h0 = encode4<0>(c0), h1 = encode4<1>(c1), h2 = encode4<0>(c2);
        const uint32_t beA = __builtin_amdgcn_perm(g0, __builtin_amdgcn_perm(g1, g2, 0x0c0c0400u), 0x0c040100u);
        const uint32_t invA = ((g0 | g1) >> 8) | (g2 & 0xF00u);
        const uint32_t beB = __builtin_amdgcn_perm(h0, __builtin_amdgcn_perm(h1, h2, 0x0c0c0400u), 0x0c040100u);
        const uint32_t invB = ((h0 | h1) >> 8) | (h2 & 0xF00u);
        auto ror1 = [](uint32_t v) __attribute__((always_inline)) -> uint32_t {
            return (uint32_t)__builtin_amdgcn_update_dpp(0, (int)v, 0x13C , 0xF, 0xF, false);
        };
        const uint32_t a1_be = ror1(beA), a1_inv = ror1(invA), b1_be = ror1(beB), b1_inv = ror1(invB);
        const uint32_t a2_be = ror1(a1_be), a2_inv = ror1(a1_inv), b2_be = ror1(b1_be), b2_inv = ror1(b1_inv);
        const uint32_t a3_be = ror1(a2_be), a3_inv = ror1(a2_inv), b3_be = ror1(b2_be), b3_inv = ror1(b2_inv);
        const uint32_t beA1 = lane >= 1 ? a1_be : pr1_be, beA2 = lane >= 2 ? a2_be : pr2_be, beA3 = lane >= 3 ? a3_be : pr3_be;
        const uint32_t iA1 = lane >= 1 ? a1_inv : pr1_inv, iA2 = lane >= 2 ? a2_inv : pr2_inv, iA3 = lane >= 3 ? a3_inv : pr3_inv;
        const uint32_t beB1 = lane >= 1 ? b1_be : a1_be, beB2 = lane >= 2 ? b2_be : a2_be, beB3 = lane >= 3 ? b3_be : a3_be;
        const uint32_t iB1 = lane >= 1 ? b1_inv : a1_inv, iB2 = lane >= 2 ? b2_inv : a2_inv, iB3 = lane >= 3 ? b3_inv : a3_inv;
        pr1_be = b1_be; pr2_be = b2_be; pr3_be = b3_be; pr1_inv = b1_inv; pr2_inv = b2_inv; pr3_inv = b3_inv;
        if (it < n_warm) continue;

        {
            const uint32_t adjA = invA & ((invA << 1) | (iA1 >> 11));
            const uint32_t adjB = invB & ((invB << 1) | (iB1 >> 11));
            if (__builtin_expect(__ballot((adjA | adjB) != 0) != 0, 0)) {
                empty_read_check(adjA, cur);
                empty_read_check(adjB, cur + VG_ROW27);
            }
        }

        const RowScan sa = scan_probe(beA, invA, beA1, beA2, beA3, iA1, iA2, iA3);
        const RowScan sb = scan_probe(beB, invB, beB1, beB2, beB3, iB1, iB2, iB3);
        const uint64_t ballA = __builtin_amdgcn_ballot_w64(sa.ok16 && (sa.gw32 & sa.gm) == sa.gm && sa.vm != 0);
        const uint64_t ballB = __builtin_amdgcn_ballot_w64(sb.ok16 && (sb.gw32 & sb.gm) == sb.gm && sb.vm != 0);
        const uint32_t nA = (uint32_t)__builtin_popcountll(ballA), nB = (uint32_t)__builtin_popcountll(ballB);
        if (VG_DBG(p.dbg) & 1u) continue;
        enqueue(sa, ballA, run_head + run_n);
        run_n += nA;
        while (run_n + nB > VG_RUNQ) drain_step();
        enqueue(sb, ballB, run_head + run_n);
        run_n += nB;
        if (run_n >= VG_RUN_BATCH || req_n >= 32u) drain_step();
        while (run_n >= 3 * VG_RUN_BATCH || req_n >= 48u) drain_step();
    }
    do {
        drain_step();
    } while (run_n != 0 || req_n != 0 || __builtin_amdgcn_ballot_w64(b_active) != 0);
    vm_wait_imm<0>();
}

#define VG_ROW27S 1024u
#define VG_RUN_BATCH_S 4u

template <bool PT, uint32_t K = 27>
__global__ __launch_bounds__(1024) void count27s_kernel(RowParams p)
{
    static_assert(K == 27 || (PT && K >= 19 && K <= 25), "count27s_kernel: k = 27, or the path-table form for k = 19 .. 25 (a run of k + 7 bases is two words)");
    constexpr uint32_t MASK_HI = (1u << (2 * K - 32)) - 1;
    extern __shared__ __attribute__((aligned(16))) uint8_t smem[];
    const uint32_t tid = threadIdx.x;
    const uint32_t lane = tid & 63u;
    const uint32_t wave = tid >> 6;
    const uint32_t nwaves = blockDim.x >> 6;
    typedef uint32_t u32x4 __attribute__((ext_vector_type(4)));
    typedef __attribute__((address_space(3))) u32x4 lds_u4_rw;
    typedef __attribute__((address_space(3))) uint64_t lds_u64_rw;
    const uint32_t wave_u = (uint32_t)__builtin_amdgcn_readfirstlane((int)wave);
    const uint32_t rings0 = VG_LUT27_BYTES + VG_GRID_LDS_WORDS * 4u;
    const uint32_t runs_base = rings0 + wave_u * (VG_RUNQ * 16u);
    const uint32_t req_base = rings0 + nwaves * (VG_RUNQ * 16u) + wave_u * (VG_REQ * 8u);
    stage_lut27(tid, blockDim.x);
    {
        const uint4* src = reinterpret_cast<const uint4*>(p.table.grid);
        uint4* dst = reinterpret_cast<uint4*>(smem + VG_LUT27_BYTES);
        for (uint32_t i = tid; i < VG_GRID_LDS_WORDS / 4; i += blockDim.x) dst[i] = src[i];
    }
    __syncthreads();
    unsigned long long* const slots8 = p.table.slots8;
    uint32_t* const counts = p.table.counts;
    const uint64_t cap_mask = p.table.cap_mask;

    const uint64_t total_pairs = p.n_bytes_dev ? *p.n_bytes_dev / (2 * VG_ROW27S) : p.row_end >> 1;
    const uint64_t total_waves = (uint64_t)gridDim.x * nwaves;
    const uint64_t ppw = (total_pairs + total_waves - 1) / total_waves;
    const uint64_t gw = (uint64_t)blockIdx.x * nwaves + wave_u;
    const uint64_t r0v = gw * ppw;
    const uint64_t r1v = r0v + ppw < total_pairs ? r0v + ppw : total_pairs;
    const uint64_t r0 = ((uint64_t)(uint32_t)__builtin_amdgcn_readfirstlane((int)(r0v >> 32)) << 32) |
                        (uint32_t)__builtin_amdgcn_readfirstlane((int)(uint32_t)r0v);
    const uint64_t r1 = ((uint64_t)(uint32_t)__builtin_amdgcn_readfirstlane((int)(r1v >> 32)) << 32) |
                        (uint32_t)__builtin_amdgcn_readfirstlane((int)(uint32_t)r1v);
    if (r0 >= r1) return;
    uint32_t one;
    asm volatile("v_mov_b32 %0, 1" : "=v"(one));
    const uint32_t lane_off = lane * 16u;
    const uint8_t* const bases = p.bases;

    uint32_t pr1_be = 0, pr2_be = 0, pr1_inv = 0xFFFFu, pr2_inv = 0xFFFFu;
    const uint64_t rs = r0 > 0 ? r0 - 1 : r0;

    uint32_t n_after_row = 0, n_after_slot = 2;
    uint64_t b_canon = 0, b_slot = 0;
    bool b_active = false;
    uint64_t p_slot = 0;
    bool p_bumped = false;

    const uint32_t my_run = lane >> 4, my_win = lane & 15u;
    const uint32_t my_sh = 2 * (15 - my_win);
    uint32_t run_head = 0, run_n = 0, req_head = 0, req_n = 0;
    auto ring_slot = [](uint32_t pos) -> uint32_t {
        const uint32_t w = pos - VG_RUNQ;
        return w < pos ? w : pos;
    };

    auto probe_issue = [&](bool act, uint64_t kmer, uint64_t dist) __attribute__((always_inline)) {
        const uint64_t rc = vg_revcomp(kmer, K);
        const uint64_t canon = kmer < rc ? kmer : rc;
        b_canon = canon | (dist << 54);
        b_slot = (vg_thash(canon) + dist) & cap_mask;
        b_active = act;
        if (act) vms_load_slot(&slots8[b_slot]);
        ++n_after_row;
        n_after_slot = 0;
    };
    constexpr uint32_t RQ = 112;
    const uint32_t rq_base = rings0 + wave_u * (VG_RUNQ * 16u + VG_REQ * 8u);
    auto rq_wrap = [](uint32_t pos) -> uint32_t { return pos >= RQ ? pos - RQ : pos; };
    const unsigned long long* const pt_index = p.table.pt.index;
    const uint32_t* const ptS = p.table.pt.S;
    const uint32_t* const ptVB = p.table.pt.VB;
    uint32_t* const ptSB = p.table.pt.SB;
    const uint32_t* const ptSLOT = p.table.pt.SLOT;
    uint32_t* const ptPC = p.table.pt.PC;
    const uint32_t pt_Tp = p.table.pt.Tp, pt_bshift = 32u - p.table.pt.bucket_log2;
    const uint32_t l1_min = (uint32_t)__builtin_amdgcn_readfirstlane((int)p.l1_min);
    uint32_t n_after_idx = 8, n_after_seq = 8;
    u32x4 l1_run = {0u, 0u, 0u, 0u};
    uint32_t l1_n = 0, l1_phase = 0;
    uint32_t pl[4] = {0u, 0u, 0u, 0u};
    bool l1_slow = false;
    auto hot = [&](uint32_t k) __attribute__((always_inline)) {
        n_after_row += k;
        n_after_idx += k;
        n_after_seq += k;
    };
    auto slow_count = [&](uint32_t klo, uint32_t khi) __attribute__((always_inline)) {
        const uint64_t kmer = (uint64_t)khi << 32 | klo, rc = vg_revcomp(kmer, K);
        if (!(K & 1u) && kmer == rc) return;
        const uint64_t canon = kmer < rc ? kmer : rc;
        uint64_t sl = vg_thash(canon) & cap_mask;
        for (;;) {
            const uint4 v = vm_load_slot_sync<true>(&slots8[sl]);
            const uint64_t c = ((uint64_t)v.y << 32) | v.x;
            if (c == VG_EMPTY) break;
            if ((c & VG_SLOT_KMER_MASK) == canon) {
                if (!(c & VG_SLOT_SAT) && vm_atomic_inc_sync(&counts[sl], one) == 254u) {
                    vm_atomic_or_sync(reinterpret_cast<uint32_t*>(&slots8[sl]) + 1, (uint32_t)(VG_SLOT_SAT >> 32));
                    vm_store_byte_sync(p.table.sat_dirty + (sl >> VG_SAT_REGION_LOG2), 1u);
                    const uint32_t pos = vm_load_dword_sync(p.table.pt.PLACE + sl);
                    if (pos != 0u) {
                        const uint32_t mir = pt_Tp - K - pos;
                        vm_atomic_or_sync(ptSB + (pos >> 5), 1u << (pos & 31u));
                        vm_atomic_or_sync(ptSB + (mir >> 5), 1u << (mir & 31u));
                    }
                }
                break;
            }
            if (!(c & VG_SLOT_CHAIN)) break;
            sl = (sl + 1) & cap_mask;
        }
    };
    auto resolve_issue = [&]() __attribute__((always_inline)) {
        l1_n = run_n < 64u ? run_n : 64u;
        if (lane < l1_n && !(VG_DBG(p.dbg) & 2048u)) {
            l1_run = *reinterpret_cast<lds_u4_rw*>((uintptr_t)(rq_base + rq_wrap(run_head + lane) * 16u));
            vmp_load_index(pt_index + ((uint64_t)(vg_idx_hash(l1_run.w & 0xFFFFFFu) >> pt_bshift) << 2));
        }
        run_head = rq_wrap(run_head + l1_n);
        run_n -= l1_n;
        hot(2);
        n_after_idx = 0;
        l1_phase = 1;
        __builtin_amdgcn_wave_barrier();
    };
    auto resolve_places = [&]() __attribute__((always_inline)) {
        vm_wait4(n_after_idx);
        const uint4 e0 = vmp_index_value<0>(), e1 = vmp_index_value<1>();
        const uint32_t cx = l1_run.w & 0xFFFFFFu;
        const bool act = lane < l1_n && !(VG_DBG(p.dbg) & (1024u | 2048u));
        const bool as_is = ((l1_run.w >> 24) & 1u) != 0;
        const bool m0 = ((e0.x ^ cx) & 0xFFFFFFu) == 0 && (((e0.x >> 24) | (e0.y << 8)) & 0x7FFFFu) != 0;
        const bool m1 = ((e1.x ^ cx) & 0xFFFFFFu) == 0 && (((e1.x >> 24) | (e1.y << 8)) & 0x7FFFFu) != 0;
        const uint4 e = m0 ? e0 : e1;
        const bool found = m0 || m1;
        const uint32_t q0 = ((e.x >> 24) | (e.y << 8)) & 0x7FFFFu, q1 = (e.y >> 11) & 0x7FFFFu;
        const uint32_t q2 = e.z & 0x7FFFFu, q3 = ((e.z >> 19) | (e.w << 13)) & 0x7FFFFu;
        const bool more = ((e.w >> 6) & 1u) != 0;
        l1_slow = act && (found ? more : ((e0.y >> 30) & 1u) != 0);
        const bool ok = act && found && !more;
        const uint32_t flip = pt_Tp - (K == 27 ? 42u : 2u * K - 12u);
        pl[0] = ok ? (as_is ? q0 : flip - q0) : 0u;
        pl[1] = ok && q1 != 0 ? (as_is ? q1 : flip - q1) : 0u;
        pl[2] = ok && q2 != 0 ? (as_is ? q2 : flip - q2) : 0u;
        pl[3] = ok && q3 != 0 ? (as_is ? q3 : flip - q3) : 0u;
        if (__builtin_amdgcn_ballot_w64(pl[0] != 0)) {
            if (pl[0] != 0) vmp_load_place<0>(ptS + (pl[0] >> 4), ptVB + (pl[0] >> 5), ptSB + (pl[0] >> 5));
            hot(3);
        }
        if (__builtin_amdgcn_ballot_w64(pl[1] != 0)) {
            if (pl[1] != 0) vmp_load_place<1>(ptS + (pl[1] >> 4), ptVB + (pl[1] >> 5), ptSB + (pl[1] >> 5));
            hot(3);
        }
        if (__builtin_expect(__builtin_amdgcn_ballot_w64(pl[2] != 0) != 0, 0)) {
            if (pl[2] != 0) vmp_load_place<2>(ptS + (pl[2] >> 4), ptVB + (pl[2] >> 5), ptSB + (pl[2] >> 5));
            hot(3);
            if (__builtin_amdgcn_ballot_w64(pl[3] != 0)) {
                if (pl[3] != 0) vmp_load_place<3>(ptS + (pl[3] >> 4), ptVB + (pl[3] >> 5), ptSB + (pl[3] >> 5));
                hot(3);
            }
        }
        n_after_seq = 0;
        l1_phase = 2;
    };
    auto windows_at = [&](uint32_t place, const uint4 sq, const uint4 bits, uint32_t vm16, uint32_t& hits) __attribute__((always_inline)) -> uint32_t {
        if constexpr (K != 27) {
            const uint32_t sh = 128u - 2u * (K + 7u) - 2u * (place & 15u);
            const bool far = sh >= 64u;
            const uint32_t x0 = funnel(far ? sq.x : sq.y, far ? sq.y : sq.z, sh & 31u);
            const uint32_t x1 = funnel(far ? 0u : sq.x, far ? sq.x : sq.y, sh & 31u);
            const uint32_t d0 = x0 ^ l1_run.x, d1 = (x1 ^ l1_run.y) & ((K + 7u == 32u) ? 0xFFFFFFFFu : (1u << ((2u * (K + 7u) - 32u) & 31u)) - 1u);
            const uint32_t tr = (d0 | (d0 >> 1)) & 0x1555u;
            const uint32_t mask_r = tr ? (1u << (7u - ((31u - (uint32_t)__builtin_clz(tr)) >> 1))) - 1u : 0xFFu;
            const uint32_t fl = d1 >> 6;
            const uint32_t tl = (fl | (fl >> 1)) & 0x1555555u;
            const uint32_t mask_l = tl ? ~((2u << (K - 13u - ((uint32_t)__builtin_ctz(tl) >> 1))) - 1u) & 0xFFu : 0xFFu;
            const uint32_t starts = funnel(bits.y, bits.x, place & 31u) & 0xFFu;
            const uint32_t sats = funnel(bits.w, bits.z, place & 31u) & 0xFFu;
            hits = mask_l & mask_r & starts & vm16;
            return hits & ~sats;
        }
        const uint32_t sh = 44u - 2u * (place & 15u);
        const bool far = sh >= 32u;
        const uint32_t x0 = funnel(far ? sq.y : sq.z, far ? sq.z : sq.w, sh & 31u);
        const uint32_t x1 = funnel(far ? sq.x : sq.y, far ? sq.y : sq.z, sh & 31u);
        const uint32_t x2 = funnel(far ? 0u : sq.x, far ? sq.x : sq.y, sh & 31u);
        const uint32_t d0 = x0 ^ l1_run.x, d1 = x1 ^ l1_run.y, d2 = (x2 ^ l1_run.z) & 0xFFFFFu;
        const uint32_t tr = (d0 | (d0 >> 1)) & 0x15555555u;
        const uint32_t mask_r = tr ? (1u << (15u - ((31u - (uint32_t)__builtin_clz(tr)) >> 1))) - 1u : 0xFFFFu;
        const uint32_t fl = funnel(d2, d1, 22) & 0x3FFFFFFFu;
        const uint32_t tl = (fl | (fl >> 1)) & 0x15555555u;
        const uint32_t mask_l = tl ? ~((1u << (15u - ((uint32_t)__builtin_ctz(tl) >> 1))) - 1u) & 0xFFFFu : 0xFFFFu;
        const uint32_t starts = funnel(bits.y, bits.x, place & 31u) & 0xFFFFu;
        const uint32_t sats = funnel(bits.w, bits.z, place & 31u) & 0xFFFFu;
        hits = mask_l & mask_r & starts & vm16;
        return hits & ~sats;
    };
    auto bump_all = [&](uint32_t todo, uint32_t place) __attribute__((always_inline)) {
        if (ptPC != nullptr) {
            const uint64_t busy = __builtin_amdgcn_ballot_w64(todo != 0);
            uint32_t left = ((uint32_t)busy | (uint32_t)(busy >> 16) | (uint32_t)(busy >> 32) | (uint32_t)(busy >> 48)) & 0xFFFFu;
#pragma unroll 1
            while (left != 0) {
                uint32_t off[4], old[4] = {0u, 0u, 0u, 0u};
#pragma unroll
                for (int q = 0; q < 4; ++q) {
                    const bool on = left != 0;
                    const uint32_t src = ((lane & 48u) + (on ? (uint32_t)__builtin_ctz(left) : 0u)) << 2;
                    left &= left - 1u;
                    const uint32_t t = (uint32_t)__builtin_amdgcn_ds_bpermute((int)src, (int)todo);
                    const uint32_t pos = (uint32_t)__builtin_amdgcn_ds_bpermute((int)src, (int)place) + (lane & 15u);
                    const uint32_t mir = pt_Tp - K - pos;
                    off[q] = on && ((t >> (lane & 15u)) & 1u) ? (pos < mir ? pos : mir) << 2 : 0xFFFFFFFFu;
                }
                vm_atomic_inc4_masked_sync(ptPC, off, one, old);
#pragma unroll
                for (int q = 0; q < 4; ++q) {
                    if (off[q] != 0xFFFFFFFFu && old[q] == 254u) {
                        const uint32_t pos = off[q] >> 2, mir = pt_Tp - K - pos;
                        const uint32_t sl = vm_load_dword_sync(ptSLOT + pos);
                        if (!(K & 1u) && (int32_t)vm_load_dword_sync(counts + sl) < 0) continue;
                        vm_atomic_or_sync(reinterpret_cast<uint32_t*>(&slots8[sl]) + 1, (uint32_t)(VG_SLOT_SAT >> 32));
                        vm_store_byte_sync(p.table.sat_dirty + (sl >> VG_SAT_REGION_LOG2), 1u);
                        vm_atomic_or_sync(ptSB + (pos >> 5), 1u << (pos & 31u));
                        vm_atomic_or_sync(ptSB + (mir >> 5), 1u << (mir & 31u));
                    }
                }
            }
            return;
        }
#pragma unroll 1
        while (__builtin_amdgcn_ballot_w64(todo != 0) != 0) {
            if (todo != 0) {
                uint32_t pos[4], sl[4], old[4];
                bool live[4];
#pragma unroll
                for (int q = 0; q < 4; ++q) {
                    live[q] = todo != 0;
                    pos[q] = place + (live[q] ? (uint32_t)__builtin_ctz(todo) : 0u);
                    todo &= todo - 1u;
                }
                vm_load_dword4_sync(ptSLOT, pos, sl);
                const uint32_t add[4] = {1u, live[1] ? 1u : 0u, live[2] ? 1u : 0u, live[3] ? 1u : 0u};
                const uint32_t at[4] = {sl[0], live[1] ? sl[1] : sl[0], live[2] ? sl[2] : sl[0], live[3] ? sl[3] : sl[0]};
                vm_atomic_add4_sync(counts, at, add, old);
#pragma unroll
                for (int q = 0; q < 4; ++q) {
                    if (live[q] && old[q] == 254u) {
                        vm_atomic_or_sync(reinterpret_cast<uint32_t*>(&slots8[sl[q]]) + 1, (uint32_t)(VG_SLOT_SAT >> 32));
                        vm_store_byte_sync(p.table.sat_dirty + (sl[q] >> VG_SAT_REGION_LOG2), 1u);
                        const uint32_t mir = pt_Tp - K - pos[q];
                        vm_atomic_or_sync(ptSB + (pos[q] >> 5), 1u << (pos[q] & 31u));
                        vm_atomic_or_sync(ptSB + (mir >> 5), 1u << (mir & 31u));
                    }
                }
            }
        }
    };
    auto resolve_compare = [&]() __attribute__((always_inline)) {
        vm_wait4(n_after_seq);
        const uint32_t vm16 = K == 27 ? (l1_run.z >> 20) | ((l1_run.w >> 28) << 12) : l1_run.z & 0xFFu;
        uint32_t hits = 0, todo[4] = {0u, 0u, 0u, 0u};
        if (pl[0] != 0) todo[0] = windows_at(pl[0], vmp_seq_value<0>(), vmp_bits_value<0>(), vm16, hits);
        if (pl[1] != 0) todo[1] = windows_at(pl[1], vmp_seq_value<1>(), vmp_bits_value<1>(), vm16, hits);
        if (__builtin_expect(__builtin_amdgcn_ballot_w64(pl[2] != 0) != 0, 0)) {
            if (pl[2] != 0) todo[2] = windows_at(pl[2], vmp_seq_value<2>(), vmp_bits_value<2>(), vm16, hits);
            if (pl[3] != 0) todo[3] = windows_at(pl[3], vmp_seq_value<3>(), vmp_bits_value<3>(), vm16, hits);
        }
        if (VG_DBG(p.dbg) & 512u) todo[0] = todo[1] = todo[2] = todo[3] = 0;
        if (__builtin_expect(__builtin_amdgcn_ballot_w64((todo[0] | todo[1] | todo[2] | todo[3]) != 0) != 0, 0)) {
            bump_all(todo[0], pl[0]);
            bump_all(todo[1], pl[1]);
            if (__builtin_amdgcn_ballot_w64((todo[2] | todo[3]) != 0) != 0) {
                bump_all(todo[2], pl[2]);
                bump_all(todo[3], pl[3]);
            }
        }
        if (__builtin_expect(__builtin_amdgcn_ballot_w64(l1_slow && !(VG_DBG(p.dbg) & 4096u)) != 0, 0)) {
            uint64_t left = __builtin_amdgcn_ballot_w64(l1_slow);
            while (left) {
                const uint32_t src = (uint32_t)__builtin_ctzll(left);
                left &= left - 1;
                const uint32_t rx = (uint32_t)__builtin_amdgcn_readlane((int)l1_run.x, (int)src), ry = (uint32_t)__builtin_amdgcn_readlane((int)l1_run.y, (int)src);
                const uint32_t rz = (uint32_t)__builtin_amdgcn_readlane((int)l1_run.z, (int)src), rw = (uint32_t)__builtin_amdgcn_readlane((int)l1_run.w, (int)src);
                if constexpr (K != 27) {
                    if (lane < 8u && (((rz & 0xFFu) >> lane) & 1u)) {
                        const uint32_t sh2 = 2u * (7u - lane);
                        slow_count(funnel(ry, rx, sh2), (ry >> sh2) & MASK_HI);
                    }
                    continue;
                }
                const uint32_t v16 = (rz >> 20) | ((rw >> 28) << 12);
                if (lane < 16u && ((v16 >> lane) & 1u)) {
                    const uint32_t sh2 = 2u * (15u - lane);
                    slow_count(funnel(ry, rx, sh2), funnel(rz, ry, sh2) & MASK_HI);
                }
            }
        }
        l1_phase = 0;
    };
    auto l1_advance = [&]() __attribute__((always_inline)) {
        if (l1_phase == 2) resolve_compare();
        else if (l1_phase == 1) resolve_places();
    };

    auto drain_hash = [&]() __attribute__((always_inline)) {
        vm_wait(n_after_slot);
        {
            const uint32_t old = vms_atomic_old();
            const bool sat = p_bumped && old == 254u;
            if (__builtin_expect(__builtin_amdgcn_ballot_w64(sat) != 0, 0)) {
                if (sat) {
                    vm_atomic_or_sync(reinterpret_cast<uint32_t*>(&slots8[p_slot]) + 1, (uint32_t)(VG_SLOT_SAT >> 32));
                    vm_store_byte_sync(p.table.sat_dirty + (p_slot >> VG_SAT_REGION_LOG2), 1u);
                }
            }
        }
        const uint2 tv = vms_slot_value();
        bool again = false;
        uint32_t* bump = nullptr;
        if (b_active) {
            const uint64_t c = ((uint64_t)tv.y << 32) | tv.x;
            const uint64_t canon = b_canon & VG_Q_KMER_MASK;
            if (c != VG_EMPTY && (c & VG_SLOT_KMER_MASK) == canon) {
                if (!(c & VG_SLOT_SAT)) bump = &counts[b_slot];
            } else if (c != VG_EMPTY && (c & VG_SLOT_CHAIN)) {
                again = !(VG_DBG(p.dbg) & 64u);
            }
        }
        const uint64_t ball = __builtin_amdgcn_ballot_w64(again);
        if (ball != 0) {
            const uint32_t n = (uint32_t)__builtin_popcountll(ball);
            const bool fits = req_n + n <= VG_REQ && (b_canon >> 54) < 1023u;
            if (__builtin_expect(__builtin_amdgcn_ballot_w64(again && !fits) == 0, 1)) {
                if (again) {
                    const uint32_t pos = __builtin_amdgcn_mbcnt_hi((uint32_t)(ball >> 32),
                                         __builtin_amdgcn_mbcnt_lo((uint32_t)ball, req_head + req_n));
                    *reinterpret_cast<lds_u64_rw*>((uintptr_t)(req_base + (pos & (VG_REQ - 1)) * 8u)) = b_canon + (1ULL << 54);
                }
                req_n += n;
            } else if (again) {
                const uint64_t canon = b_canon & VG_Q_KMER_MASK;
                uint64_t sl = b_slot;
                for (;;) {
                    sl = (sl + 1) & cap_mask;
                    const uint4 v = vm_load_slot_sync<true>(&slots8[sl]);
                    const uint64_t c = ((uint64_t)v.y << 32) | v.x;
                    if (c != VG_EMPTY && (c & VG_SLOT_KMER_MASK) == canon) {
                        if (!(c & VG_SLOT_SAT)) { bump = &counts[sl]; b_slot = sl; }
                        break;
                    }
                    if (c == VG_EMPTY || !(c & VG_SLOT_CHAIN)) break;
                }
            }
        }
        p_bumped = bump != nullptr;
        p_slot = b_slot;
        if (__builtin_amdgcn_ballot_w64(bump != nullptr)) {
            if (bump) vms_atomic_inc(bump, one);
            ++n_after_row;
        }
        __builtin_amdgcn_wave_barrier();
        const bool do_req = req_n >= 32u || run_n == 0;
        const uint32_t take_req = do_req ? (req_n < 64u ? req_n : 64u) : 0u;
        const uint32_t take_run = do_req ? 0u : (run_n < VG_RUN_BATCH_S ? run_n : VG_RUN_BATCH_S);
        const uint32_t rq_head = req_head, rn_head = run_head;
        req_head += take_req;
        req_n -= take_req;
        run_head += take_run;
        if (run_head >= VG_RUNQ) run_head -= VG_RUNQ;
        run_n -= take_run;
        if (do_req) {
            const bool have = lane < take_req;
            uint64_t e = 0;
            if (have) e = *reinterpret_cast<lds_u64_rw*>((uintptr_t)(req_base + ((rq_head + lane) & (VG_REQ - 1)) * 8u));
            if (take_req) probe_issue(have, e & VG_Q_KMER_MASK, e >> 54);
            else b_active = false;
        } else {
            const bool have = my_run < take_run;
            u32x4 e = {0u, 0u, 0u, 0u};
            if (have) e = *reinterpret_cast<lds_u4_rw*>((uintptr_t)(runs_base + ring_slot(rn_head + my_run) * 16u));
            const uint32_t lo = funnel(e.y, e.x, my_sh);
            const uint32_t hi = funnel(e.z, e.y, my_sh) & MASK_HI;
            probe_issue(have && ((e.w >> my_win) & 1u) && (!(VG_DBG(p.dbg) & 32u) || my_win == (__builtin_ctz(e.w) & 15u)),
                        ((uint64_t)hi << 32) | lo, 0);
        }
        __builtin_amdgcn_wave_barrier();
    };

    auto drain_step = [&]() __attribute__((always_inline)) { drain_hash(); };
    auto make_room = [&]() __attribute__((always_inline)) {
        while (l1_phase != 0) l1_advance();
        resolve_issue();
    };

    struct RowScan { uint32_t W0, W1, W2, vm, gm, gw32, cm; };
    auto scan_probe = [&](uint32_t be, uint32_t inv, uint32_t be1, uint32_t be2, uint32_t i1, uint32_t i2) __attribute__((always_inline)) -> RowScan {
        RowScan r;
        r.W0 = be;
        r.W1 = be1;
        r.W2 = be2;
        const uint32_t B = (i2 >> 5) | (i1 << 11);
        const uint32_t a = (inv << 1) & 0xFFFFu;
        const uint32_t bad_b = B ? (0xFFFFFFFFu >> __builtin_clz(B)) : 0u;
        r.vm = ~(a | (0u - a) | bad_b) & 0xFFFFu;
        const uint32_t mer = be1 & 0xFFFFFFu, rcm = vg_revcomp12(mer);
        const uint32_t cm = mer < rcm ? mer : rcm;
        r.cm = cm | (mer <= rcm ? 1u << 24 : 0u);
        const uint32_t h1 = vg_mul24(cm, 0x9E3779u), h2 = vg_mul24(cm, 0x85EBCBu);
        r.gm = (1u << (h2 >> 27)) | (1u << ((h2 >> 22) & 31u)) | (1u << ((h2 >> 17) & 31u));
        r.gw32 = *reinterpret_cast<lds_u32*>((uintptr_t)(((h1 >> (32 - VG_GRID_LDS_WORDS_LOG2)) << 2) + VG_LUT27_BYTES));
        return r;
    };
    auto enqueue = [&](const RowScan& r, uint64_t ball, uint32_t tail) __attribute__((always_inline)) {
        if (__builtin_amdgcn_inverse_ballot_w64(ball)) {
            const uint32_t d0 = funnel(r.W1, r.W0, 2);
            const uint32_t d1 = funnel(r.W2, r.W1, 2);
            const uint32_t d2 = r.W2 >> 2;
            const uint32_t pos = __builtin_amdgcn_mbcnt_hi((uint32_t)(ball >> 32), __builtin_amdgcn_mbcnt_lo((uint32_t)ball, tail));
            if (PT)
                *reinterpret_cast<lds_u4_rw*>((uintptr_t)(rq_base + rq_wrap(pos) * 16u)) =
                    u32x4{d0, d1, (d2 & 0xFFFFFu) | (r.vm << 20), r.cm | ((r.vm >> 12) << 28)};
            else
                *reinterpret_cast<lds_u4_rw*>((uintptr_t)(runs_base + ring_slot(pos) * 16u)) = u32x4{d0, d1, d2, r.vm};
        }
    };
    auto scan_probe_k = [&](uint32_t be, uint32_t inv, uint32_t be1, uint32_t be2, uint32_t i1, uint32_t i2, uint32_t H) __attribute__((always_inline)) -> RowScan {
        RowScan r;
        r.W0 = be;
        r.W1 = be1;
        r.W2 = be2;
        const uint32_t g = 32u + 8u * H;
        const uint64_t I = (uint64_t)i2 | (uint64_t)i1 << 16 | (uint64_t)inv << 32;
        const uint32_t B = (uint32_t)(I >> (g + 1u - K)) & ((1u << K) - 1u);
        const uint32_t a = (uint32_t)(I >> g) & 0xFEu;
        const uint32_t bad_b = B ? (0xFFFFFFFFu >> __builtin_clz(B)) : 0u;
        r.vm = ~(a | (0u - a) | bad_b) & 0xFFu;
        const uint32_t mer = funnel(be1, be, 30u - 16u * H) & 0xFFFFFFu, rcm = vg_revcomp12(mer);
        const uint32_t cm = mer < rcm ? mer : rcm;
        r.cm = cm | (mer <= rcm ? 1u << 24 : 0u);
        const uint32_t h1 = vg_mul24(cm, 0x9E3779u), h2 = vg_mul24(cm, 0x85EBCBu);
        r.gm = (1u << (h2 >> 27)) | (1u << ((h2 >> 22) & 31u)) | (1u << ((h2 >> 17) & 31u));
        r.gw32 = *reinterpret_cast<lds_u32*>((uintptr_t)(((h1 >> (32 - VG_GRID_LDS_WORDS_LOG2)) << 2) + VG_LUT27_BYTES));
        return r;
    };
    auto enqueue_k = [&](const RowScan& r, uint64_t ball, uint32_t tail, uint32_t H) __attribute__((always_inline)) {
        if (__builtin_amdgcn_inverse_ballot_w64(ball)) {
            const uint32_t sh = 16u - 16u * H;
            const uint32_t d0 = funnel(r.W1, r.W0, sh);
// ... 824 lines not shown
```

### varigraph_amd/csrc/vgmi_ptable.hip

```cpp
#include <hip/hip_runtime.h>
#include <stdint.h>

#include "vgmi_device.h"
#include "vgmi_kernels.h"

namespace vgk {

#define PT_NONE 0xFFFFFFFFu
#define PT_MASK54 VG_SLOT_KMER_MASK

__device__ __forceinline__ uint32_t pt_find(const TableView& t, uint64_t canon)
{
    uint64_t s = (t.home_bucket_log2 ? vg_thash_local(canon, vg_revcomp(canon, t.k), t.home_bucket_log2, t.home_by_offset != 0) : vg_thash(canon)) & t.cap_mask;
    for (;;) {
        const uint64_t c = t.slots8[s];
        if (c == VG_EMPTY) return PT_NONE;
        if ((c & VG_SLOT_KMER_MASK) == canon) return (uint32_t)s;
        if (!(c & VG_SLOT_CHAIN)) return PT_NONE;
        s = (s + 1) & t.cap_mask;
    }
}

__global__ void pt_key_of_slot_kernel(const uint32_t* key_slot, uint64_t n, uint32_t* key_of_slot)
{
    const uint64_t i = (uint64_t)blockIdx.x * blockDim.x + threadIdx.x;
    if (i < n) key_of_slot[key_slot[i]] = (uint32_t)i;
}

__global__ void pt_links_kernel(TableView t, const uint32_t* key_slot, const uint32_t* key_of_slot, uint64_t n, uint32_t* link)
{
    const uint64_t g = (uint64_t)blockIdx.x * blockDim.x + threadIdx.x;
    if (g >= 2 * n) return;
    const uint64_t i = g >> 1;
    const uint32_t side = (uint32_t)g & 1u;
    const uint64_t K = t.slots8[key_slot[i]] & PT_MASK54;
    const uint64_t kmask = (1ULL << (2 * t.k)) - 1;
    uint32_t found = PT_NONE, cnt = 0, enter = 0;
    for (uint64_t b = 0; b < 4; ++b) {
        const uint64_t N = side ? ((K << 2) | b) & kmask : (K >> 2) | (b << (2 * t.k - 2));
        const uint64_t rc = vg_revcomp(N, t.k);
        const bool flipped = N > rc;
        const uint32_t s = pt_find(t, flipped ? rc : N);
        if (s == PT_NONE) continue;
        ++cnt;
        found = key_of_slot[s];
        enter = side ? (flipped ? 1u : 0u) : (flipped ? 0u : 1u);
    }
    link[g] = (cnt == 1 && found != (uint32_t)i && found < 0x7FFFFFFFu) ? (found | enter << 31) : PT_NONE;
}

__global__ void pt_mutual_kernel(const uint32_t* link, uint32_t* link2, uint64_t n)
{
    const uint64_t g = (uint64_t)blockIdx.x * blockDim.x + threadIdx.x;
    if (g >= 2 * n) return;
    const uint32_t l = link[g];
    uint32_t out = PT_NONE;
    if (l != PT_NONE) {
        const uint64_t nb = l & 0x7FFFFFFFu, es = l >> 31;
        const uint32_t back = link[2 * nb + es];
        if (back != PT_NONE && (back & 0x7FFFFFFFu) == (uint32_t)(g >> 1) && (back >> 31) == ((uint32_t)g & 1u)) out = l;
    }
    link2[g] = out;
}

__global__ void pt_walk_kernel(const uint32_t* link2, uint64_t n, uint32_t* pos_of_key, unsigned long long* cursor, uint32_t align)
{
    const uint64_t g = (uint64_t)blockIdx.x * blockDim.x + threadIdx.x;
    if (g >= 2 * n) return;
    if (link2[g] != PT_NONE) return;
    const uint32_t start = (uint32_t)(g >> 1), s0 = (uint32_t)g & 1u;
    uint32_t cur = start, out = s0 ^ 1u;
    uint64_t len = 1;
    for (;;) {
        const uint32_t l = link2[2ull * cur + out];
        if (l == PT_NONE || len > n) break;
        cur = l & 0x7FFFFFFFu;
        out = (l >> 31) ^ 1u;
        ++len;
    }
    const bool own = start < cur || (start == cur && (s0 == 0u || link2[2ull * start] != PT_NONE));
    if (!own || len > n) return;
    const uint64_t base = atomicAdd(cursor, (unsigned long long)((len + align - 1) / align * align));
    cur = start;
    out = s0 ^ 1u;
    for (uint64_t pos = 0; pos < len; ++pos) {
        pos_of_key[cur] = (uint32_t)(base + pos) | out << 31;
        const uint32_t l = link2[2ull * cur + out];
        if (l == PT_NONE) break;
        cur = l & 0x7FFFFFFFu;
        out = (l >> 31) ^ 1u;
    }
}

__global__ void pt_rest_kernel(uint64_t n, uint32_t* pos_of_key, unsigned long long* cursor)
{
    const uint64_t i = (uint64_t)blockIdx.x * blockDim.x + threadIdx.x;
    if (i >= n) return;
    if (pos_of_key[i] == PT_NONE) pos_of_key[i] = (uint32_t)atomicAdd(cursor, 1ULL) | 1u << 31;
}

__global__ void pt_check_kernel(const uint32_t* pos_of_key, uint64_t n, uint64_t total, uint32_t* mark, uint32_t* status)
{
    const uint64_t i = (uint64_t)blockIdx.x * blockDim.x + threadIdx.x;
    if (i >= n) return;
    const uint32_t pos = pos_of_key[i] & 0x7FFFFFFFu;
    if (pos >= total || atomicAdd(&mark[pos], 1u) != 0u) atomicOr(status, 16u);
}

__global__ void pt_fill_kernel(TableView t, const uint32_t* key_slot, const uint32_t* pos_of_key, uint64_t n, ulonglong2* P)
{
    const uint64_t i = (uint64_t)blockIdx.x * blockDim.x + threadIdx.x;
    if (i >= n) return;
    const uint32_t slot = key_slot[i];
    const uint64_t K = t.slots8[slot] & PT_MASK54, R = vg_revcomp(K, t.k);
    const uint32_t pk = pos_of_key ? pos_of_key[i] : ((uint32_t)i | 1u << 31);
    const uint64_t pos = pk & 0x7FFFFFFFu;
    const bool as_is = (pk >> 31) != 0;
    P[pos] = make_ulonglong2(as_is ? K : R, slot);
    P[2 * n - 1 - pos] = make_ulonglong2(as_is ? R : K, slot);
}

hipError_t launch_ptable_order(const TableView& t, const uint32_t* key_slot, uint64_t n, uint32_t* key_of_slot, uint32_t* link, uint32_t* link2,
                               uint32_t* pos_of_key, unsigned long long* cursor, uint32_t* mark, uint32_t* status, hipStream_t st, uint32_t align)
{
    if (n == 0) return hipSuccess;
    const uint32_t g2 = (uint32_t)((2 * n + 255) / 256), g1 = (uint32_t)((n + 255) / 256);
    hipLaunchKernelGGL(pt_key_of_slot_kernel, dim3(g1), dim3(256), 0, st, key_slot, n, key_of_slot);
    hipLaunchKernelGGL(pt_links_kernel, dim3(g2), dim3(256), 0, st, t, key_slot, key_of_slot, n, link);
    hipLaunchKernelGGL(pt_mutual_kernel, dim3(g2), dim3(256), 0, st, link, link2, n);
    hipLaunchKernelGGL(pt_walk_kernel, dim3(g2), dim3(256), 0, st, link2, n, pos_of_key, cursor, align ? align : 1u);
    hipLaunchKernelGGL(pt_rest_kernel, dim3(g1), dim3(256), 0, st, n, pos_of_key, cursor);
    if (mark) hipLaunchKernelGGL(pt_check_kernel, dim3(g1), dim3(256), 0, st, pos_of_key, n, n, mark, status);
    return hipGetLastError();
}

hipError_t launch_ptable_check(const uint32_t* pos_of_key, uint64_t n, uint64_t total, uint32_t* mark, uint32_t* status, hipStream_t st)
{
    if (n == 0) return hipSuccess;
    hipLaunchKernelGGL(pt_check_kernel, dim3((uint32_t)((n + 255) / 256)), dim3(256), 0, st, pos_of_key, n, total, mark, status);
    return hipGetLastError();
}

hipError_t launch_ptable_fill(const TableView& t, const uint32_t* key_slot, const uint32_t* pos_of_key, uint64_t n, ulonglong2* P, hipStream_t st)
{
    if (n == 0) return hipSuccess;
    hipLaunchKernelGGL(pt_fill_kernel, dim3((uint32_t)((n + 255) / 256)), dim3(256), 0, st, t, key_slot, pos_of_key, n, P);
    return hipGetLastError();
}

}
```

### varigraph_amd/vgmi.py

```python
import ctypes as C
import os

import numpy as np

_HERE = os.path.dirname(os.path.abspath(__file__))
LIB_PATH = os.path.join(_HERE, "libvgmi.so")

OK = 0
E_INVALID, E_NO_DEVICE, E_HIP, E_STATE, E_DUPLICATE_KEY, E_BAD_KEY, E_EMPTY_READ, E_NOMEM = range(-1, -9, -1)


class VgmiError(RuntimeError):
    def __init__(self, code, msg):
        super().__init__(f"vgmi error {code}: {msg}")
        self.code = code


def load_library():
    if not os.path.exists(LIB_PATH):
        raise ImportError(
            f"{LIB_PATH} is missing: build it with `python -m varigraph_amd.build` "
            "(hipcc --offload-arch=gfx950). There is no CPU fallback.")
    try:
        import torch
    except Exception:
        pass
    lib = C.CDLL(LIB_PATH)
    vp, u64, u32, sz, i32 = C.c_void_p, C.c_uint64, C.c_uint32, C.c_size_t, C.c_int
    sig = {
        "vgmi_device_count": (i32, []),
        "vgmi_create": (i32, [i32, sz, C.POINTER(vp)]),
        "vgmi_destroy": (None, [vp]),
        "vgmi_last_error": (C.c_char_p, [vp]),
        "vgmi_stream": (vp, [vp]),
        "vgmi_device_of": (i32, [vp, C.POINTER(i32)]),
        "vgmi_device_memory": (i32, [vp, C.POINTER(sz), C.POINTER(sz)]),
        "vgmi_table_upload": (i32, [vp, vp, sz, u32]),
        "vgmi_table_image_bytes": (i32, [vp, C.POINTER(sz)]),
        "vgmi_table_export": (i32, [vp, vp, sz]),
        "vgmi_table_import": (i32, [vp, vp, sz]),
        "vgmi_table_clone": (i32, [vp, vp]),
        "vgmi_rccl_unique_id": (i32, [vp]),
        "vgmi_table_broadcast": (i32, [vp, i32, i32, vp]),
        "vgmi_comm_create": (i32, [i32, i32, i32, vp, C.POINTER(vp)]),
        "vgmi_table_broadcast_comm": (i32, [vp, vp]),
        "vgmi_table_snapshot": (i32, [vp]),
        "vgmi_comm_destroy": (None, [vp]),
        "vgmi_table_info": (i32, [vp, C.POINTER(sz), C.POINTER(u32), C.POINTER(sz), C.POINTER(sz)]),
        "vgmi_xtable_info": (i32, [vp, C.POINTER(sz), C.POINTER(sz)]),
        "vgmi_ctable_info": (i32, [vp, C.POINTER(sz), C.POINTER(sz), C.POINTER(sz), C.POINTER(sz), C.POINTER(sz)]),
        "vgmi_ctable_defer_info": (i32, [vp, C.POINTER(u64), C.POINTER(u64), C.POINTER(u32), C.POINTER(u32), C.POINTER(u32), C.POINTER(u32)]),
        "vgmi_table_lookup": (i32, [vp, vp, sz, vp]),
        "vgmi_nodes_upload": (i32, [vp, vp, vp, sz]),
        "vgmi_flags_upload": (i32, [vp, vp]),
        "vgmi_counts_reset": (i32, [vp]),
        "vgmi_reads_submit": (i32, [vp, vp, sz, vp, sz]),
        "vgmi_reads_submit_device": (i32, [vp, vp, sz, vp, sz]),
        "vgmi_read_base": (i32, [vp, C.POINTER(u64)]),
        "vgmi_counts_finish": (i32, [vp, vp, vp, vp]),
        "vgmi_counts_finish_device": (i32, [vp, vp, vp, vp]),
        "vgmi_count_kernel_ms": (i32, [vp, C.POINTER(C.c_float), C.POINTER(u64)]),
        "vgmi_counts_export_device": (i32, [vp, vp]),
        "vgmi_counts_import_device": (i32, [vp, vp]),
        "vgmi_fastq_open": (i32, [vp, C.POINTER(vp)]),
        "vgmi_fastq_open_bam": (i32, [vp, C.c_uint64, i32, C.POINTER(vp)]),
        "vgmi_fastq_open_fasta": (i32, [vp, C.POINTER(vp)]),
        "vgmi_fastq_acquire": (i32, [vp, C.POINTER(vp), C.POINTER(sz)]),
        "vgmi_fastq_text_capacity": (i32, [vp, C.POINTER(sz)]),
        "vgmi_fastq_commit": (i32, [vp, sz]),
        "vgmi_fastq_commit_bgzf": (i32, [vp, sz, C.POINTER(sz), C.POINTER(sz), C.POINTER(i32)]),
        "vgmi_fastq_bgzf_status": (i32, [vp, C.POINTER(i32), C.POINTER(u64), C.POINTER(u32)]),
        "vgmi_fastq_commit_gzip": (i32, [vp, sz, i32, C.POINTER(sz), C.POINTER(sz), C.POINTER(i32)]),
        "vgmi_fastq_gzip_status": (i32, [vp, C.POINTER(u64), C.POINTER(u32)]),
        "vgmi_gunzip_buffer": (i32, [vp, vp, sz, vp, sz, C.POINTER(sz), C.POINTER(sz), C.POINTER(i32), C.POINTER(u32)]),
        "vgmi_fastq_close": (i32, [vp, C.POINTER(u64), C.POINTER(u64), C.POINTER(u64), C.POINTER(i32), vp, sz, C.POINTER(sz)]),
        "vgmi_sketch_keys": (i32, [vp, vp, sz, vp, sz, u32, vp]),
        "vgmi_bloom_params": (i32, [u64, C.c_double, C.POINTER(u64), C.POINTER(u32)]),
        "vgmi_bloom_create": (i32, [vp, u64, u32, vp]),
        "vgmi_bloom_add_seq": (i32, [vp, vp, u64, u32]),
        "vgmi_bloom_add_seq_device": (i32, [vp, vp, u64, u32]),
        "vgmi_hmm_recursion": (i32, [vp, u32, u32, vp, u32, vp, C.c_uint64, vp, vp, vp, C.c_uint64, vp, vp, u32, vp]),
        "vgmi_hmm_recursion_fre": (i32, [vp, u32, u32, vp, u32, vp, C.c_uint64, vp, vp, C.c_uint64, vp, vp, u32, vp]),
        "vgmi_hmm_calls": (i32, [vp, u32, u32, vp, u32, vp, C.c_uint64, vp, vp, vp, C.c_uint64, vp, vp, u32, vp, vp, vp, vp, vp, vp, vp]),
        "vgmi_hmm_calls_part": (i32, [vp, u32, u32, vp, u32, vp, C.c_uint64, C.c_uint64, vp, vp, vp, C.c_uint64, C.c_uint64, vp, vp, u32,
                                      vp, vp, vp, vp, vp, vp]),
        "vgmi_hmm_entries_upload": (i32, [vp, vp, sz]),
        "vgmi_hmm_sample_upload": (i32, [vp, vp, sz]),
        "vgmi_hmm_emissions": (i32, [vp, u32, u32, vp, vp, vp, C.c_uint64, u32, C.c_float, C.c_double, C.c_double, vp, C.c_uint64, vp, vp, vp, vp, vp,
                                      C.POINTER(vp)]),
        "vgmi_hmm_emissions_ploidy": (i32, [vp, u32, u32, u32, vp, vp, C.c_uint64, u32, C.c_float, C.c_double, C.c_double, vp, C.c_uint64, vp, vp, vp, vp, vp,
                                      C.POINTER(vp)]),
        "vgmi_hmm_alive_upload": (i32, [vp, vp, sz]),
        "vgmi_hmm_alive_fetch": (i32, [vp, vp, sz]),
        "vgmi_hmm_support": (i32, [vp, u32, u32, C.c_uint64, vp, vp, vp, vp]),
        "vgmi_hmm_emissions_select": (i32, [vp, u32, u32, vp, vp, u32, vp, vp, u32, C.c_float, C.c_double, C.c_double, vp, C.c_uint64, vp, vp, vp, vp,
                                            vp, vp, C.POINTER(vp)]),
        "vgmi_hmm_emissions_select_ploidy": (i32, [vp, u32, u32, u32, vp, vp, vp, u32, C.c_float, C.c_double, C.c_double, vp, C.c_uint64, vp, vp, vp, vp,
                                                   vp, vp, C.POINTER(vp)]),
        "vgmi_hmm_part_fix_rows_wide": (i32, [vp, C.c_uint64, vp, vp, vp, vp]),
        "vgmi_hmm_tallies_select": (i32, [vp, C.c_uint64, vp, vp, vp, vp, u32, vp, vp, u32, u32, vp, vp, vp]),
        "vgmi_hmm_tallies_ploidy": (i32, [vp, u32, u32, u32, vp, vp, vp, C.c_uint64, vp, vp, vp, vp, C.c_int, vp, vp]),
        "vgmi_hmm_entries_upload_wide": (i32, [vp, vp, vp, sz, u32]),
        "vgmi_hmm_entries_reserve_wide": (i32, [vp, sz, u32]),
        "vgmi_hmm_entries_fill_wide": (i32, [vp, sz, sz, vp, vp]),
        "vgmi_hmm_support_wide": (i32, [vp, u32, u32, u32, C.c_uint64, vp, vp, vp, vp]),
        "vgmi_hmm_emissions_select_wide": (i32, [vp, u32, u32, vp, vp, u32, vp, vp, u32, C.c_float, C.c_double, C.c_double, vp, C.c_uint64, vp, vp, vp, vp,
                                                 vp, vp, C.POINTER(vp)]),
        "vgmi_hmm_tallies_select_wide": (i32, [vp, u32, C.c_uint64, vp, vp, vp, vp, u32, vp, vp, u32, u32, vp, vp, vp]),
        "vgmi_hmm_emissions_select_ploidy_wide": (i32, [vp, u32, u32, u32, vp, vp, vp, u32, C.c_float, C.c_double, C.c_double, vp, C.c_uint64, vp, vp, vp, vp,
                                                        vp, vp, C.POINTER(vp)]),
        "vgmi_hmm_part_fix_rows_ploidy_wide": (i32, [vp, C.c_uint64, vp, vp, vp, vp]),
        "vgmi_hmm_tallies_ploidy_wide": (i32, [vp, u32, u32, u32, u32, vp, vp, vp, C.c_uint64, vp, vp, vp, vp, C.c_int, vp, vp]),
        "vgmi_hmm_part_set_rows": (i32, [vp, C.c_uint64, vp, vp]),
        "vgmi_hmm_part_fix_rows": (i32, [vp, C.c_uint64, vp, vp, vp, vp]),
        "vgmi_hmm_plan_create": (i32, [vp, u32, u32, vp, u32, C.c_uint64, vp, vp, vp, C.c_uint64, vp, vp, u32, vp, vp, vp, vp, C.POINTER(vp)]),
        "vgmi_hmm_part_calls_plan": (i32, [vp, vp, vp, vp]),
        "vgmi_hmm_plan_free": (None, [vp]),
        "vgmi_hmm_part_calls": (i32, [vp, u32, vp, u32, vp, vp, vp, C.c_uint64, vp, vp, u32, vp, vp, vp, vp, vp, vp]),
        "vgmi_hmm_part_calls_fre": (i32, [vp, u32, vp, u32, vp, vp, C.c_uint64, vp, vp, u32, vp, vp, vp, vp, vp, vp]),
        "vgmi_hmm_part_fetch": (i32, [vp, vp]),
        "vgmi_hmm_part_free": (None, [vp]),
        "vgmi_bloom_fetch": (i32, [vp, vp]),
        "vgmi_bloom_save_file": (i32, [vp, C.c_char_p]),
        "vgmi_bloom_load_file": (i32, [vp, C.c_char_p]),
        "vgmi_bloom_load": (i32, [vp, vp]),
        "vgmi_bloom_query": (i32, [vp, vp, sz, vp, vp]),
    }
    for name, (res, args) in sig.items():
        fn = getattr(lib, name)
        fn.restype = res
        fn.argtypes = args
    return lib, sorted(sig)


_lib = None
SYMBOLS = None


def lib():
    global _lib, SYMBOLS
    if _lib is None:
        _lib, SYMBOLS = load_library()
    return _lib


def _ptr(a):
    if a is None:
        return None
    if isinstance(a, int):
        return C.c_void_p(a)
    if isinstance(a, np.ndarray):
        assert a.flags["C_CONTIGUOUS"]
        return C.c_void_p(a.ctypes.data)
    if isinstance(a, (bytes, bytearray)):
        return C.cast(C.c_char_p(bytes(a)), C.c_void_p)
    if hasattr(a, "data_ptr"):
        return C.c_void_p(a.data_ptr())
    raise TypeError(type(a))


def bloom_params(n, p):
    m, nh = C.c_uint64(), C.c_uint32()
    lib().vgmi_bloom_params(n, p, C.byref(m), C.byref(nh))
    return m.value, nh.value


def synth_reference(seed, length):
    from . import synthlib
    return synthlib.reference(seed, length)


def synth_snp_keys(ref, pos, alts, k=27):
    from . import synthlib
    return synthlib.snp_keys(ref, pos, alts, k)


def synth_reads_host(seed, first_read, n_reads, read_len, haps):
    from . import synthlib
    return synthlib.reads_host(seed, first_read, n_reads, read_len, haps)


class Context:

    def __init__(self, device=0, buffer_mib=100):
        self._l = lib()
        h = C.c_void_p()
        rc = self._l.vgmi_create(device, buffer_mib, C.byref(h))
        if rc:
            raise VgmiError(rc, (self._l.vgmi_last_error(None) or b"").decode())
        self._h = h
        self.n_keys = 0
        self.n_node_entries = 0

    def close(self):
        if getattr(self, "_h", None):
            self._l.vgmi_destroy(self._h)
            self._h = None

    def __del__(self):
        try:
            self.close()
        except Exception:
            pass

    def _chk(self, rc):
        if rc:
            raise VgmiError(rc, (self._l.vgmi_last_error(self._h) or b"").decode())

    @property
    def stream(self):
        return self._l.vgmi_stream(self._h)

    def table_upload(self, keys, k):
        keys = np.ascontiguousarray(keys, dtype=np.uint64)
        self._chk(self._l.vgmi_table_upload(self._h, _ptr(keys), keys.size, k))
        self.n_keys = keys.size
        self.n_node_entries = 0

    def table_image_bytes(self):
        n = C.c_size_t()
        self._chk(self._l.vgmi_table_image_bytes(self._h, C.byref(n)))
        return n.value

    def table_export(self, dev_tensor):
        self._chk(self._l.vgmi_table_export(self._h, _ptr(dev_tensor), dev_tensor.numel()))

    def table_import(self, dev_tensor):
        self._chk(self._l.vgmi_table_import(self._h, _ptr(dev_tensor), dev_tensor.numel()))
        self.n_keys = self.table_info()["n_keys"]
        self.n_node_entries = 0

    def table_clone_from(self, src):
        self._chk(self._l.vgmi_table_clone(self._h, src._h))
        self.n_keys = self.table_info()["n_keys"]
        self.n_node_entries = 0

    def device_memory(self):
        f, t = C.c_size_t(), C.c_size_t()
        self._chk(self._l.vgmi_device_memory(self._h, C.byref(f), C.byref(t)))
        return f.value, t.value

    def table_info(self):
        n, k, s, f = C.c_size_t(), C.c_uint32(), C.c_size_t(), C.c_size_t()
        self._chk(self._l.vgmi_table_info(self._h, C.byref(n), C.byref(k), C.byref(s), C.byref(f)))
        return {"n_keys": n.value, "k": k.value, "n_slots": s.value, "filter_bits": f.value}

    def table_lookup(self, keys):
        keys = np.ascontiguousarray(keys, dtype=np.uint64)
        out = np.empty(keys.size, dtype=np.uint32)
        self._chk(self._l.vgmi_table_lookup(self._h, _ptr(keys) if keys.size else None, keys.size, _ptr(out) if keys.size else None))
        return out

    def xtable_info(self):
        n, o = C.c_size_t(), C.c_size_t()
        self._chk(self._l.vgmi_xtable_info(self._h, C.byref(n), C.byref(o)))
        return {"n_lines": n.value, "overflow_pairs": o.value}

    def ctable_info(self):
        v = [C.c_size_t() for _ in range(5)]
        self._chk(self._l.vgmi_ctable_info(self._h, *[C.byref(x) for x in v]))
        return dict(zip(("n_buckets", "n_entries", "n_unitigs", "moved_entries", "overflow_kmers"), (x.value for x in v)))

    def ctable_defer_info(self):
        v = [C.c_uint64(), C.c_uint64()] + [C.c_uint32() for _ in range(4)]
        self._chk(self._l.vgmi_ctable_defer_info(self._h, *[C.byref(x) for x in v]))
        return dict(zip(("deferred_launches", "plain_launches", "n_bins", "region", "room", "cap"), (x.value for x in v)))

    def nodes_upload(self, node_off, key_index):
        node_off = np.ascontiguousarray(node_off, dtype=np.uint64)
        key_index = np.ascontiguousarray(key_index, dtype=np.uint32)
        self._chk(self._l.vgmi_nodes_upload(self._h, _ptr(node_off), _ptr(key_index), node_off.size - 1))
        self.n_node_entries = int(node_off[-1])

    def flags_upload(self, flags):
        flags = np.ascontiguousarray(flags, dtype=np.uint8)
        assert flags.size == self.n_keys
        self._chk(self._l.vgmi_flags_upload(self._h, _ptr(flags)))

    def counts_reset(self):
        self._chk(self._l.vgmi_counts_reset(self._h))

    def reads_submit(self, block, n_reads, read_off=None):
        block = np.ascontiguousarray(block, dtype=np.uint8)
        if read_off is not None:
            read_off = np.ascontiguousarray(read_off, dtype=np.uint64)
        self._chk(self._l.vgmi_reads_submit(self._h, _ptr(block), block.size, _ptr(read_off), n_reads))

    def reads_submit_device(self, dev_block, n_bytes, n_reads, dev_read_off=None):
        self._chk(self._l.vgmi_reads_submit_device(self._h, _ptr(dev_block), n_bytes, _ptr(dev_read_off), n_reads))

    def read_base(self):
        v = C.c_uint64()
        self._chk(self._l.vgmi_read_base(self._h, C.byref(v)))
        return v.value

    def counts_finish(self, nodes=False, hist=False):
        cov = np.empty(self.n_keys, dtype=np.uint8)
        cov_node = np.empty(self.n_node_entries, dtype=np.uint8) if nodes else None
        h = np.zeros(256, dtype=np.uint64) if hist else None
        self._chk(self._l.vgmi_counts_finish(self._h, _ptr(cov), _ptr(cov_node), _ptr(h)))
        return cov, cov_node, h

    def counts_finish_device(self, dev_cov=None, dev_cov_node=None, dev_hist=None):
        self._chk(self._l.vgmi_counts_finish_device(self._h, _ptr(dev_cov), _ptr(dev_cov_node), _ptr(dev_hist)))

    def counts_export_device(self, dev_u32):
        self._chk(self._l.vgmi_counts_export_device(self._h, _ptr(dev_u32)))

    def counts_import_device(self, dev_u32):
        self._chk(self._l.vgmi_counts_import_device(self._h, _ptr(dev_u32)))

    def count_kernel_ms(self):
        ms, n = C.c_float(), C.c_uint64()
        self._chk(self._l.vgmi_count_kernel_ms(self._h, C.byref(ms), C.byref(n)))
        return ms.value, n.value

    def fastq_text(self, text, piece=None):
        fq = C.c_void_p()
        self._chk(self._l.vgmi_fastq_open(self._h, C.byref(fq)))
        return self._text_stream(fq, text, piece)

    def fasta_text(self, text, piece=None):
        fq = C.c_void_p()
        self._chk(self._l.vgmi_fastq_open_fasta(self._h, C.byref(fq)))
        return self._text_stream(fq, text, piece)

    def _text_stream(self, fq, text, piece):
        mv = memoryview(text)
        pos = 0
        try:
            while True:
                buf, cap = C.c_void_p(), C.c_size_t()
                self._chk(self._l.vgmi_fastq_acquire(fq, C.byref(buf), C.byref(cap)))
                n = min(cap.value if piece is None else min(piece, cap.value), len(mv) - pos)
                C.memmove(buf, bytes(mv[pos:pos + n]), n)
                self._chk(self._l.vgmi_fastq_commit(fq, n))
                pos += n
                if pos >= len(mv):
                    break
        finally:
            nr, nb, cons, st, tl = C.c_uint64(), C.c_uint64(), C.c_uint64(), C.c_int(), C.c_size_t()
            tail = C.create_string_buffer(1 << 20)
            rc = self._l.vgmi_fastq_close(fq, C.byref(nr), C.byref(nb), C.byref(cons), C.byref(st), tail, 1 << 20, C.byref(tl))
        self._chk(rc)
        return {"n_records": nr.value, "n_bases": nb.value, "consumed": cons.value, "stopped": bool(st.value),
                "tail": tail.raw[:tl.value]}

    def fastq_bgzf(self, comp, piece=None):
        fq = C.c_void_p()
        self._chk(self._l.vgmi_fastq_open(self._h, C.byref(fq)))
        return self._bgzf_stream(fq, comp, piece)

    def fasta_bgzf(self, comp, piece=None):
        fq = C.c_void_p()
        self._chk(self._l.vgmi_fastq_open_fasta(self._h, C.byref(fq)))
        return self._bgzf_stream(fq, comp, piece)

    def bam_bgzf(self, comp, header_bytes, n_ref, piece=None):
        fq = C.c_void_p()
        self._chk(self._l.vgmi_fastq_open_bam(self._h, header_bytes, n_ref, C.byref(fq)))
        return self._bgzf_stream(fq, comp, piece)

    def _bgzf_stream(self, fq, comp, piece):
        comp = bytes(comp)
        pos, carry, total_taken, n_call = 0, b"", 0, 0
        failed, good, reason = C.c_int(), C.c_uint64(), C.c_uint32()
        try:
            while True:
                buf, cap = C.c_void_p(), C.c_size_t()
                self._chk(self._l.vgmi_fastq_acquire(fq, C.byref(buf), C.byref(cap)))
                if isinstance(piece, (list, tuple)):
                    want = piece[min(n_call, len(piece) - 1)]
                else:
                    want = piece
                n_call += 1
                room = (cap.value if want is None else min(want, cap.value)) - len(carry)
                new = comp[pos:pos + max(room, 0)]
                pos += len(new)
                data = carry + new
                C.memmove(buf, data, len(data))
                taken, n_text, nb = C.c_size_t(), C.c_size_t(), C.c_int()
                self._chk(self._l.vgmi_fastq_commit_bgzf(fq, len(data), C.byref(taken), C.byref(n_text), C.byref(nb)))
                total_taken += taken.value
                carry = data[taken.value:]
                if nb.value or (pos >= len(comp) and (taken.value == 0 or not carry)):
                    break
            self._chk(self._l.vgmi_fastq_bgzf_status(fq, C.byref(failed), C.byref(good), C.byref(reason)))
        finally:
            nr, nbs, cons, st, tl = C.c_uint64(), C.c_uint64(), C.c_uint64(), C.c_int(), C.c_size_t()
            tail = C.create_string_buffer(1 << 20)
            rc = self._l.vgmi_fastq_close(fq, C.byref(nr), C.byref(nbs), C.byref(cons), C.byref(st), tail, 1 << 20, C.byref(tl))
        self._chk(rc)
        return {"n_records": nr.value, "n_bases": nbs.value, "consumed": cons.value, "stopped": bool(st.value),
                "tail": tail.raw[:tl.value], "inflate_failed": bool(failed.value), "good_compressed_bytes": good.value,
                "reason": reason.value, "taken": total_taken}

    def fastq_gzip(self, comp, piece=None):
        fq = C.c_void_p()
        self._chk(self._l.vgmi_fastq_open(self._h, C.byref(fq)))
        return self._gzip_stream(fq, comp, piece)

    def fasta_gzip(self, comp, piece=None):
        fq = C.c_void_p()
        self._chk(self._l.vgmi_fastq_open_fasta(self._h, C.byref(fq)))
        return self._gzip_stream(fq, comp, piece)

    def _gzip_stream(self, fq, comp, piece):
        comp = bytes(comp)
        pos, carry, total_taken, stop, n_call = 0, b"", 0, 0, 0
        dtext, reason = C.c_uint64(), C.c_uint32()
        try:
            while True:
                buf, cap = C.c_void_p(), C.c_size_t()
                self._chk(self._l.vgmi_fastq_acquire(fq, C.byref(buf), C.byref(cap)))
                if isinstance(piece, (list, tuple)):
                    want = piece[min(n_call, len(piece) - 1)]
                else:
                    want = piece
                n_call += 1
                room = (cap.value if want is None else min(want, cap.value)) - len(carry)
                new = comp[pos:pos + max(room, 0)]
                pos += len(new)
                data = carry + new
                C.memmove(buf, data, len(data))
                taken, n_text, st = C.c_size_t(), C.c_size_t(), C.c_int()
                self._chk(self._l.vgmi_fastq_commit_gzip(fq, len(data), int(pos >= len(comp)), C.byref(taken), C.byref(n_text), C.byref(st)))
                total_taken += taken.value
                carry = data[taken.value:]
                stop = st.value
                if stop or (pos >= len(comp) and taken.value == 0):
                    break
            self._chk(self._l.vgmi_fastq_gzip_status(fq, C.byref(dtext), C.byref(reason)))
        finally:
            nr, nbs, cons, sp, tl = C.c_uint64(), C.c_uint64(), C.c_uint64(), C.c_int(), C.c_size_t()
            tail = C.create_string_buffer(1 << 20)
            rc = self._l.vgmi_fastq_close(fq, C.byref(nr), C.byref(nbs), C.byref(cons), C.byref(sp), tail, 1 << 20, C.byref(tl))
        self._chk(rc)
        return {"n_records": nr.value, "n_bases": nbs.value, "consumed": cons.value, "stopped": bool(sp.value), "tail": tail.raw[:tl.value],
                "stop": stop, "device_text_bytes": dtext.value, "reason": reason.value, "taken": total_taken}

    def gunzip(self, comp, cap):
        comp = bytes(comp)
        out = np.empty(max(cap, 1), dtype=np.uint8)
        n_out, cons, fin, why = C.c_size_t(), C.c_size_t(), C.c_int(), C.c_uint32()
        self._chk(self._l.vgmi_gunzip_buffer(self._h, comp, len(comp), _ptr(out), cap, C.byref(n_out), C.byref(cons), C.byref(fin), C.byref(why)))
        return out[:n_out.value].tobytes(), cons.value, bool(fin.value), why.value

    def sketch_keys(self, block, n_reads, k, read_off=None):
        block = np.ascontiguousarray(block, dtype=np.uint8)
        if read_off is not None:
            read_off = np.ascontiguousarray(read_off, dtype=np.uint64)
        out = np.empty(block.size, dtype=np.uint64)
        self._chk(self._l.vgmi_sketch_keys(self._h, _ptr(block), block.size, _ptr(read_off), n_reads, k, _ptr(out)))
        return out

    def bloom_create(self, m, n_hash, seeds):
        seeds = np.ascontiguousarray(seeds, dtype=np.uint64)
        assert seeds.size == n_hash
        self._chk(self._l.vgmi_bloom_create(self._h, m, n_hash, _ptr(seeds)))
        self._bloom_m = m

    def bloom_add_seq(self, seq, k):
        seq = np.ascontiguousarray(seq, dtype=np.uint8)
        self._chk(self._l.vgmi_bloom_add_seq(self._h, _ptr(seq), seq.size, k))

    def bloom_add_seq_device(self, dev_seq, length, k):
        self._chk(self._l.vgmi_bloom_add_seq_device(self._h, _ptr(dev_seq), length, k))

    def hmm_recursion(self, keep, obs, row, restart, pow_tables, uniform, chains, ploidy):
# ... 421 lines not shown
```

Before: 26.88 billion.

## Skip path-table lookups for buckets whose positions are all saturated

Adds per-bucket completion tracking. At build time, each path-table position is mapped to its index bucket and each bucket gets the number of valid positions it covers. When a position's saturation bit is newly set, counters for the affected buckets are incremented, and a bucket is marked done once its counter reaches the required total. The hot count kernel loads the done bitmap with the bucket index and drops lanes whose bucket is done, exiting early when no lane remains. This trades extra atomics on saturation events and one more load per run for skipping place loads and count atomics on saturated regions, and adds a debug checker API.

After: 28.30 billion (median of 6 runs). 1.05x the previous value.

```diff
diff --git a/include/vgmi.h b/include/vgmi.h
--- a/include/vgmi.h
+++ b/include/vgmi.h
@@ -67,6 +67,7 @@
 int vgmi_counts_export_device(vgmi_ctx *ctx, uint32_t *dev_counts_out );
 int vgmi_counts_import_device(vgmi_ctx *ctx, const uint32_t *dev_counts );
 int vgmi_count_kernel_ms(vgmi_ctx *ctx, float *ms, uint64_t *launches);
+int vgmi_pt_done_check(vgmi_ctx *ctx, uint64_t out[4]);
 
 typedef struct vgmi_fastq vgmi_fastq;
 int vgmi_fastq_open(vgmi_ctx *ctx, vgmi_fastq **out);
diff --git a/varigraph_amd/csrc/vgmi_api.cpp b/varigraph_amd/csrc/vgmi_api.cpp
--- a/varigraph_amd/csrc/vgmi_api.cpp
+++ b/varigraph_amd/csrc/vgmi_api.cpp
@@ -68,10 +68,11 @@
     } else if (c->d_ct_buckets) (void)hipFree(c->d_ct_buckets);
     c->d_ct_buckets = nullptr;
     c->ct_entries = c->ct_unitigs = c->ct_moved = 0;
-    for (void* q : {(void*)c->d_pt_index, (void*)c->d_pt_S, (void*)c->d_pt_VB, (void*)c->d_pt_SB, (void*)c->d_pt_SLOT, (void*)c->d_pt_PLACE})
+    for (void* q : {(void*)c->d_pt_index, (void*)c->d_pt_S, (void*)c->d_pt_VB, (void*)c->d_pt_SB, (void*)c->d_pt_SLOT, (void*)c->d_pt_PLACE,
+                    (void*)c->d_pt_BKT, (void*)c->d_pt_NEED})
         if (q) (void)hipFree(q);
     c->d_pt_index = nullptr;
-    c->d_pt_S = c->d_pt_VB = c->d_pt_SB = c->d_pt_SLOT = c->d_pt_PLACE = nullptr;
+    c->d_pt_S = c->d_pt_VB = c->d_pt_SB = c->d_pt_SLOT = c->d_pt_PLACE = c->d_pt_BKT = c->d_pt_NEED = nullptr;
     c->tv.pt = PathView{};
     c->d_xt_lines = nullptr;
     c->d_xt_counts = nullptr;
@@ -673,6 +674,26 @@
     return VGMI_OK;
 }
 
+int vgmi_pt_done_check(vgmi_ctx* c, uint64_t out[4])
+{
+    if (!c || !out) return VGMI_E_INVALID;
+    if (!c->has_table) return fail(c, VGMI_E_STATE, "no table");
+    out[0] = out[1] = out[2] = out[3] = 0;
+    if (!c->tv.pt.index) return VGMI_OK;
+    HIPCHK(c, hipSetDevice(c->device));
+    int rc = sync_stages(c);
+    if (rc) return rc;
+    unsigned long long* d = nullptr;
+    HIPCHK(c, hipMalloc(reinterpret_cast<void**>(&d), 32));
+    hipError_t he = hipMemsetAsync(d, 0, 32, c->stream);
+    if (he == hipSuccess) he = launch_ptable_done_check(c->tv.pt, c->hdr.k, d, c->stream);
+    if (he == hipSuccess) he = hipStreamSynchronize(c->stream);
+    if (he == hipSuccess) he = hipMemcpy(out, d, 32, hipMemcpyDeviceToHost);
+    (void)hipFree(d);
+    HIPCHK(c, he);
+    return VGMI_OK;
+}
+
 
 int vgmi_sketch_keys(vgmi_ctx* c, const char* bases, size_t n_bytes, const uint64_t* read_off, size_t n_reads,
                      uint32_t k, uint64_t* keys_out)
diff --git a/varigraph_amd/csrc/vgmi_api_table.cpp b/varigraph_amd/csrc/vgmi_api_table.cpp
--- a/varigraph_amd/csrc/vgmi_api_table.cpp
+++ b/varigraph_amd/csrc/vgmi_api_table.cpp
@@ -499,16 +499,59 @@
     }
     c->pt_slow_cx = slow_cx;
     c->pt_bucket_ovf = bucket_ovf;
+    const char* dnv = getenv("VGMI_PT_DONE");
+    const bool pt_done = !(dnv && dnv[0] == '0');
+    const size_t n_buckets = (size_t)1 << bucket_log2;
+    const uint32_t W = K == 27 ? 16u : 8u, flip = (uint32_t)Tp - (K == 27 ? 42u : 2u * K - 12u);
+    std::vector<uint32_t> BKT, NEED;
+    if (pt_done) {
+        BKT.assign((size_t)Tp + 64, VG_PT_NO_BUCKET);
+        NEED.assign(n_buckets, 0u);
+        std::vector<uint8_t> never(n_buckets, 0);
+        for (size_t b = 0; b < n_buckets; ++b) {
+            const unsigned long long* B = &index[b << 2];
+            if (B[0] >> 62 & 1) never[b] = 1;
+            for (int e = 0; e < 2; ++e) {
+                const unsigned long long lo = B[2 * e], hi = B[2 * e + 1];
+                if (hi >> 38 & 1) never[b] = 1;
+                const uint32_t q[4] = {(uint32_t)(lo >> 24) & 0x7FFFFu, (uint32_t)(lo >> 43) & 0x7FFFFu, (uint32_t)hi & 0x7FFFFu, (uint32_t)(hi >> 19) & 0x7FFFFu};
+                for (int i = 0; i < 4 && q[0] != 0; ++i) {
+                    if (q[i] == 0) continue;
+                    for (const uint32_t at : {q[i], flip - q[i]}) {
+                        if (at >= Tp || (BKT[at] != VG_PT_NO_BUCKET && BKT[at] != (uint32_t)b)) {
+                            never[b] = 1;
+                            if (at < Tp) never[BKT[at]] = 1;
+                            continue;
+                        }
+                        BKT[at] = (uint32_t)b;
+                    }
+                }
+            }
+        }
+        for (uint64_t at = 0; at < Tp; ++at) {
+            if (BKT[at] == VG_PT_NO_BUCKET) continue;
+            for (uint32_t j = 0; j < W && at + j < Tp; ++j) NEED[BKT[at]] += vb[at + j];
+        }
+        for (size_t b = 0; b < n_buckets; ++b)
+            if (never[b] || NEED[b] == 0) NEED[b] = 0xFFFFFFFFu;
+    }
     he = hipMalloc(reinterpret_cast<void**>(&c->d_pt_index), index.size() * 8);
     if (he == hipSuccess) he = hipMalloc(reinterpret_cast<void**>(&c->d_pt_S), S.size() * 4);
     if (he == hipSuccess) he = hipMalloc(reinterpret_cast<void**>(&c->d_pt_VB), VB.size() * 4);
-    const size_t pc_words = (size_t)Tp + 64;
-    if (he == hipSuccess) he = hipMalloc(reinterpret_cast<void**>(&c->d_pt_SB), (VB.size() + pc_words) * 4);
+    const size_t pc_words = (size_t)Tp + 64, cnt_words = pt_done ? n_buckets : 0, done_words = pt_done ? (n_buckets + 31) / 32 : 0;
+    const size_t sb_words = VB.size() + pc_words + cnt_words + done_words;
+    if (he == hipSuccess) he = hipMalloc(reinterpret_cast<void**>(&c->d_pt_SB), sb_words * 4);
+    if (pt_done) {
+        if (he == hipSuccess) he = hipMalloc(reinterpret_cast<void**>(&c->d_pt_BKT), BKT.size() * 4);
+        if (he == hipSuccess) he = hipMalloc(reinterpret_cast<void**>(&c->d_pt_NEED), NEED.size() * 4);
+        if (he == hipSuccess) he = hipMemcpy(c->d_pt_BKT, BKT.data(), BKT.size() * 4, hipMemcpyHostToDevice);
+        if (he == hipSuccess) he = hipMemcpy(c->d_pt_NEED, NEED.data(), NEED.size() * 4, hipMemcpyHostToDevice);
+    }
     if (he == hipSuccess) he = hipMalloc(reinterpret_cast<void**>(&c->d_pt_SLOT), (size_t)(Tp + 64) * 4);
     if (he == hipSuccess) he = hipMemcpy(c->d_pt_index, index.data(), index.size() * 8, hipMemcpyHostToDevice);
     if (he == hipSuccess) he = hipMemcpy(c->d_pt_S, S.data(), S.size() * 4, hipMemcpyHostToDevice);
     if (he == hipSuccess) he = hipMemcpy(c->d_pt_VB, VB.data(), VB.size() * 4, hipMemcpyHostToDevice);
-    if (he == hipSuccess) he = hipMemset(c->d_pt_SB, 0, (VB.size() + pc_words) * 4);
+    if (he == hipSuccess) he = hipMemset(c->d_pt_SB, 0, sb_words * 4);
     if (he == hipSuccess) he = hipMemset(c->d_pt_SLOT, 0, (size_t)(Tp + 64) * 4);
     if (he == hipSuccess) he = hipMemcpy(c->d_pt_SLOT, slot.data(), (size_t)Tp * 4, hipMemcpyHostToDevice);
     {
@@ -518,7 +561,7 @@
         if (he == hipSuccess) he = hipMemcpy(c->d_pt_PLACE, place_of_slot.data(), h.cap * 4, hipMemcpyHostToDevice);
     }
     HIPCHK(c, he);
-    c->pt_sb_bytes = (VB.size() + pc_words) * 4;
+    c->pt_sb_bytes = sb_words * 4;
     if (getenv("VGMI_VERBOSE"))
         fprintf(stderr, "[vgmi] path table: %llu k-mers in %llu chains, %llu bases, %llu 12-mers with a fifth place, %llu buckets with a third 12-mer\n",
                 (unsigned long long)n, (unsigned long long)chains, (unsigned long long)Tp, (unsigned long long)slow_cx, (unsigned long long)bucket_ovf);
@@ -530,6 +573,12 @@
     c->tv.pt.PLACE = c->d_pt_PLACE;
     const char* pcv = getenv("VGMI_PT_POSCOUNT");
     c->tv.pt.PC = pcv && pcv[0] == '0' ? nullptr : c->d_pt_SB + VB.size();
+    if (pt_done) {
+        c->tv.pt.BKT = c->d_pt_BKT;
+        c->tv.pt.NEED = c->d_pt_NEED;
+        c->tv.pt.CNT = c->d_pt_SB + VB.size() + pc_words;
+        c->tv.pt.DONE = c->tv.pt.CNT + cnt_words;
+    }
     c->tv.pt.bucket_log2 = bucket_log2;
     c->tv.pt.Tp = (uint32_t)Tp;
     return VGMI_OK;
diff --git a/varigraph_amd/csrc/vgmi_ctx.h b/varigraph_amd/csrc/vgmi_ctx.h
--- a/varigraph_amd/csrc/vgmi_ctx.h
+++ b/varigraph_amd/csrc/vgmi_ctx.h
@@ -86,6 +86,7 @@
     uint64_t ct_entries = 0, ct_unitigs = 0, ct_moved = 0;
     unsigned long long* d_pt_index = nullptr;
     uint32_t *d_pt_S = nullptr, *d_pt_VB = nullptr, *d_pt_SB = nullptr, *d_pt_SLOT = nullptr, *d_pt_PLACE = nullptr;
+    uint32_t *d_pt_BKT = nullptr, *d_pt_NEED = nullptr;
     size_t pt_sb_bytes = 0;
     uint64_t pt_slow_cx = 0, pt_bucket_ovf = 0;
     uint64_t xt_over_keys = 0;
diff --git a/varigraph_amd/csrc/vgmi_kernels.h b/varigraph_amd/csrc/vgmi_kernels.h
--- a/varigraph_amd/csrc/vgmi_kernels.h
+++ b/varigraph_amd/csrc/vgmi_kernels.h
@@ -40,9 +40,14 @@
     const uint32_t* SLOT;
     const uint32_t* PLACE;
     uint32_t* PC;
+    const uint32_t* BKT;
+    const uint32_t* NEED;
+    uint32_t* CNT;
+    uint32_t* DONE;
     uint32_t bucket_log2;
     uint32_t Tp;
 };
+#define VG_PT_NO_BUCKET 0xFFFFFFFFu
 
 struct TableView {
     VgSlot* slots;
@@ -355,6 +360,7 @@
 hipError_t launch_ptable_order(const TableView& t, const uint32_t* key_slot, uint64_t n, uint32_t* key_of_slot, uint32_t* link, uint32_t* link2,
                                uint32_t* pos_of_key, unsigned long long* cursor, uint32_t* mark, uint32_t* status, hipStream_t st, uint32_t align = 1);
 hipError_t launch_ptable_check(const uint32_t* pos_of_key, uint64_t n, uint64_t total, uint32_t* mark, uint32_t* status, hipStream_t st);
+hipError_t launch_ptable_done_check(const PathView& pt, uint32_t k, unsigned long long* out, hipStream_t st);
 hipError_t launch_ptable_fill(const TableView& t, const uint32_t* key_slot, const uint32_t* pos_of_key, uint64_t n, ulonglong2* P, hipStream_t st);
 hipError_t launch_rows(int mode, bool flds, const RowParams& p, uint32_t grid, uint32_t block, hipStream_t st);
 hipError_t launch_bloom_even(const RowParams& p, hipStream_t st);
diff --git a/varigraph_amd/csrc/vgmi_kernels.hip b/varigraph_amd/csrc/vgmi_kernels.hip
--- a/varigraph_amd/csrc/vgmi_kernels.hip
+++ b/varigraph_amd/csrc/vgmi_kernels.hip
@@ -112,6 +112,31 @@
 {
     const uint32_t* const pc = pt_cell(t, s);
     return pc ? *pc : 0u;
+}
+
+__device__ __forceinline__ uint32_t vm_load_dword_sync(const uint32_t* ptr);
+__device__ __forceinline__ void vm_load_and_inc_sync(const uint32_t* ld, uint32_t* at, uint32_t one, uint32_t& v, uint32_t& old);
+__device__ __forceinline__ void vm_atomic_or_sync(uint32_t* ptr, uint32_t bits);
+template <bool HOT>
+__device__ __forceinline__ void pt_done_step(const uint32_t* BKT, const uint32_t* NEED, uint32_t* CNT, uint32_t* DONE, uint32_t q)
+{
+    if constexpr (HOT) {
+        const uint32_t b = vm_load_dword_sync(BKT + q);
+        if (b == VG_PT_NO_BUCKET) return;
+        uint32_t need, old;
+        vm_load_and_inc_sync(NEED + b, CNT + b, 1u, need, old);
+        if (old + 1u == need) vm_atomic_or_sync(DONE + (b >> 5), 1u << (b & 31u));
+    } else {
+        const uint32_t b = BKT[q];
+        if (b == VG_PT_NO_BUCKET) return;
+        if (atomicAdd(&CNT[b], 1u) + 1u == NEED[b]) atomicOr(&DONE[b >> 5], 1u << (b & 31u));
+    }
+}
+__device__ __forceinline__ void pt_done_event(const PathView& pt, uint32_t k, uint32_t x)
+{
+    if (!pt.DONE) return;
+    const uint32_t W = k == 27u ? 16u : 8u;
+    for (uint32_t j = 0; j < W; ++j) pt_done_step<false>(pt.BKT, pt.NEED, pt.CNT, pt.DONE, x - j);
 }
 
 __device__ __forceinline__ uint64_t table_home(const TableView& t, uint64_t canon)
@@ -143,8 +168,8 @@
                         const uint32_t pos = t.pt.PLACE[s];
                         if (pos != 0u) {
                             const uint32_t mir = t.pt.Tp - t.k - pos;
-                            atomicOr(&t.pt.SB[pos >> 5], 1u << (pos & 31u));
-                            atomicOr(&t.pt.SB[mir >> 5], 1u << (mir & 31u));
+                            if (!(atomicOr(&t.pt.SB[pos >> 5], 1u << (pos & 31u)) >> (pos & 31u) & 1u)) pt_done_event(t.pt, t.k, pos);
+                            if (!(atomicOr(&t.pt.SB[mir >> 5], 1u << (mir & 31u)) >> (mir & 31u) & 1u)) pt_done_event(t.pt, t.k, mir);
                         }
                     }
                 }
@@ -482,6 +507,16 @@
 {
     asm volatile("global_load_dwordx4 v[108:111], %0, off ; VGHOT\n\tglobal_load_dwordx4 v[112:115], %0, off offset:16 ; VGHOT" : : "v"(ptr) : VG_HOT_CLOBBERS_P);
 }
+__device__ __forceinline__ void vmp_load_done(const void* ptr)
+{
+    asm volatile("global_load_dword v76, %0, off ; VGHOT" : : "v"(ptr) : VG_HOT_CLOBBERS_P);
+}
+__device__ __forceinline__ uint32_t vmp_done_value()
+{
+    uint32_t v;
+    asm volatile("v_mov_b32 %0, v76 ; VGHOT" : "=v"(v));
+    return v;
+}
 #define VG_SEQ_ASM(C, SQ, VBR, SBR) \
     if (c == C) asm volatile("global_load_dwordx4 " SQ ", %0, off ; VGHOT\n\tglobal_load_dwordx2 " VBR ", %1, off ; VGHOT\n\tglobal_load_dwordx2 " SBR ", %2, off ; VGHOT" \
                              : : "v"(sq), "v"(vb), "v"(sb) : VG_HOT_CLOBBERS_P)
@@ -560,6 +595,17 @@
 {
     uint32_t old;
     asm volatile("global_atomic_add %0, %1, %2, off sc0 ; VGHOT\n\ts_waitcnt vmcnt(0) ; VGHOT" : "=&v"(old) : "v"(ptr), "v"(one) : "memory");
+    return old;
+}
+__device__ __forceinline__ void vm_load_and_inc_sync(const uint32_t* ld, uint32_t* at, uint32_t one, uint32_t& v, uint32_t& old)
+{
+    asm volatile("global_load_dword %0, %2, off ; VGHOT\n\tglobal_atomic_add %1, %3, %4, off sc0 ; VGHOT\n\ts_waitcnt vmcnt(0) ; VGHOT"
+                 : "=&v"(v), "=&v"(old) : "v"(ld), "v"(at), "v"(one) : "memory");
+}
+__device__ __forceinline__ uint32_t vm_atomic_or_ret_sync(uint32_t* ptr, uint32_t bits)
+{
+    uint32_t old;
+    asm volatile("global_atomic_or %0, %1, %2, off sc0 ; VGHOT\n\ts_waitcnt vmcnt(0) ; VGHOT" : "=&v"(old) : "v"(ptr), "v"(bits) : "memory");
     return old;
 }
 __device__ __forceinline__ void vm_wait4(uint32_t n)
@@ -1086,6 +1132,10 @@
     uint32_t* const ptSB = p.table.pt.SB;
     const uint32_t* const ptSLOT = p.table.pt.SLOT;
     uint32_t* const ptPC = p.table.pt.PC;
+    const uint32_t* const ptBKT = p.table.pt.BKT;
+    const uint32_t* const ptNEED = p.table.pt.NEED;
+    uint32_t* const ptCNT = p.table.pt.CNT;
+    uint32_t* const ptDONE = p.table.pt.DONE;
     const uint32_t pt_Tp = p.table.pt.Tp, pt_bshift = 32u - p.table.pt.bucket_log2;
     const uint32_t l1_min = (uint32_t)__builtin_amdgcn_readfirstlane((int)p.l1_min);
     uint32_t n_after_idx = 8, n_after_seq = 8;
@@ -1093,12 +1143,29 @@
     uint32_t l1_n = 0, l1_phase = 0;
     uint32_t pl[4] = {0u, 0u, 0u, 0u};
     bool l1_slow = false;
+    uint32_t l1_done_bit = 0;
     auto hot = [&](uint32_t k) __attribute__((always_inline)) {
         n_after_row += k;
         n_after_idx += k;
         n_after_seq += k;
     };
-    auto slow_count = [&](uint32_t klo, uint32_t khi) __attribute__((always_inline)) {
+    auto set_saturated = [&](uint32_t pos, uint32_t mir) __attribute__((always_inline)) -> uint32_t {
+        const uint32_t a = vm_atomic_or_ret_sync(ptSB + (pos >> 5), 1u << (pos & 31u));
+        const uint32_t b = vm_atomic_or_ret_sync(ptSB + (mir >> 5), 1u << (mir & 31u));
+        return ((~a >> (pos & 31u)) & 1u) | (((~b >> (mir & 31u)) & 1u) << 1);
+    };
+    auto done_events = [&](uint32_t fired, uint32_t pos) __attribute__((always_inline)) {
+        constexpr uint32_t W = K == 27 ? 16u : 8u;
+        uint64_t ev = __builtin_amdgcn_ballot_w64(fired != 0);
+        while (ev != 0) {
+            const uint32_t src = (uint32_t)__builtin_ctzll(ev);
+            ev &= ev - 1;
+            const uint32_t f = (uint32_t)__builtin_amdgcn_readlane((int)fired, (int)src), x0 = (uint32_t)__builtin_amdgcn_readlane((int)pos, (int)src);
+            const uint32_t x = lane < 16u ? x0 : pt_Tp - K - x0;
+            if (lane < 32u && (lane & 15u) < W && ((f >> (lane >> 4)) & 1u)) pt_done_step<true>(ptBKT, ptNEED, ptCNT, ptDONE, x - (lane & 15u));
+        }
+    };
+    auto slow_count = [&](uint32_t klo, uint32_t khi, uint32_t& fired, uint32_t& at) __attribute__((always_inline)) {
         const uint64_t kmer = (uint64_t)khi << 32 | klo, rc = vg_revcomp(kmer, K);
         if (!(K & 1u) && kmer == rc) return;
         const uint64_t canon = kmer < rc ? kmer : rc;
@@ -1113,9 +1180,8 @@
                     vm_store_byte_sync(p.table.sat_dirty + (sl >> VG_SAT_REGION_LOG2), 1u);
                     const uint32_t pos = vm_load_dword_sync(p.table.pt.PLACE + sl);
                     if (pos != 0u) {
-                        const uint32_t mir = pt_Tp - K - pos;
-                        vm_atomic_or_sync(ptSB + (pos >> 5), 1u << (pos & 31u));
-                        vm_atomic_or_sync(ptSB + (mir >> 5), 1u << (mir & 31u));
+                        fired = set_saturated(pos, pt_Tp - K - pos);
+                        at = pos;
                     }
                 }
                 break;
@@ -1128,11 +1194,16 @@
         l1_n = run_n < 64u ? run_n : 64u;
         if (lane < l1_n && !(VG_DBG(p.dbg) & 2048u)) {
             l1_run = *reinterpret_cast<lds_u4_rw*>((uintptr_t)(rq_base + rq_wrap(run_head + lane) * 16u));
-            vmp_load_index(pt_index + ((uint64_t)(vg_idx_hash(l1_run.w & 0xFFFFFFu) >> pt_bshift) << 2));
+            const uint32_t bucket = vg_idx_hash(l1_run.w & 0xFFFFFFu) >> pt_bshift;
+            if (ptDONE != nullptr) {
+                vmp_load_done(ptDONE + (bucket >> 5));
+                l1_done_bit = 1u << (bucket & 31u);
+            }
+            vmp_load_index(pt_index + ((uint64_t)bucket << 2));
         }
         run_head = rq_wrap(run_head + l1_n);
         run_n -= l1_n;
-        hot(2);
+        hot(ptDONE != nullptr ? 3 : 2);
         n_after_idx = 0;
         l1_phase = 1;
         __builtin_amdgcn_wave_barrier();
@@ -1141,7 +1212,8 @@
         vm_wait4(n_after_idx);
         const uint4 e0 = vmp_index_value<0>(), e1 = vmp_index_value<1>();
         const uint32_t cx = l1_run.w & 0xFFFFFFu;
-        const bool act = lane < l1_n && !(VG_DBG(p.dbg) & (1024u | 2048u));
+        const bool done = ptDONE != nullptr && (vmp_done_value() & l1_done_bit) != 0;
+        const bool act = lane < l1_n && !done && !(VG_DBG(p.dbg) & (1024u | 2048u));
         const bool as_is = ((l1_run.w >> 24) & 1u) != 0;
         const bool m0 = ((e0.x ^ cx) & 0xFFFFFFu) == 0 && (((e0.x >> 24) | (e0.y << 8)) & 0x7FFFFu) != 0;
         const bool m1 = ((e1.x ^ cx) & 0xFFFFFFu) == 0 && (((e1.x >> 24) | (e1.y << 8)) & 0x7FFFFu) != 0;
@@ -1157,6 +1229,10 @@
         pl[1] = ok && q1 != 0 ? (as_is ? q1 : flip - q1) : 0u;
         pl[2] = ok && q2 != 0 ? (as_is ? q2 : flip - q2) : 0u;
         pl[3] = ok && q3 != 0 ? (as_is ? q3 : flip - q3) : 0u;
+        if (__builtin_amdgcn_ballot_w64(ok || l1_slow) == 0) {
+            l1_phase = 0;
+            return;
+        }
         if (__builtin_amdgcn_ballot_w64(pl[0] != 0)) {
             if (pl[0] != 0) vmp_load_place<0>(ptS + (pl[0] >> 4), ptVB + (pl[0] >> 5), ptSB + (pl[0] >> 5));
             hot(3);
@@ -1227,6 +1303,7 @@
                     off[q] = on && ((t >> (lane & 15u)) & 1u) ? (pos < mir ? pos : mir) << 2 : 0xFFFFFFFFu;
                 }
                 vm_atomic_inc4_masked_sync(ptPC, off, one, old);
+                uint32_t fired[4] = {0u, 0u, 0u, 0u};
 #pragma unroll
                 for (int q = 0; q < 4; ++q) {
                     if (off[q] != 0xFFFFFFFFu && old[q] == 254u) {
@@ -1235,17 +1312,21 @@
                         if (!(K & 1u) && (int32_t)vm_load_dword_sync(counts + sl) < 0) continue;
                         vm_atomic_or_sync(reinterpret_cast<uint32_t*>(&slots8[sl]) + 1, (uint32_t)(VG_SLOT_SAT >> 32));
                         vm_store_byte_sync(p.table.sat_dirty + (sl >> VG_SAT_REGION_LOG2), 1u);
-                        vm_atomic_or_sync(ptSB + (pos >> 5), 1u << (pos & 31u));
-                        vm_atomic_or_sync(ptSB + (mir >> 5), 1u << (mir & 31u));
+                        fired[q] = set_saturated(pos, mir);
                     }
                 }
+                if (ptDONE != nullptr && __builtin_amdgcn_ballot_w64((fired[0] | fired[1] | fired[2] | fired[3]) != 0) != 0) {
+#pragma unroll
+                    for (int q = 0; q < 4; ++q) done_events(fired[q], off[q] >> 2);
+                }
             }
             return;
         }
 #pragma unroll 1
         while (__builtin_amdgcn_ballot_w64(todo != 0) != 0) {
+            uint32_t pos[4] = {0u, 0u, 0u, 0u}, fired[4] = {0u, 0u, 0u, 0u};
             if (todo != 0) {
-                uint32_t pos[4], sl[4], old[4];
+                uint32_t sl[4], old[4];
                 bool live[4];
 #pragma unroll
                 for (int q = 0; q < 4; ++q) {
@@ -1262,11 +1343,13 @@
                     if (live[q] && old[q] == 254u) {
                         vm_atomic_or_sync(reinterpret_cast<uint32_t*>(&slots8[sl[q]]) + 1, (uint32_t)(VG_SLOT_SAT >> 32));
                         vm_store_byte_sync(p.table.sat_dirty + (sl[q] >> VG_SAT_REGION_LOG2), 1u);
-                        const uint32_t mir = pt_Tp - K - pos[q];
-                        vm_atomic_or_sync(ptSB + (pos[q] >> 5), 1u << (pos[q] & 31u));
-                        vm_atomic_or_sync(ptSB + (mir >> 5), 1u << (mir & 31u));
+                        fired[q] = set_saturated(pos[q], pt_Tp - K - pos[q]);
                     }
                 }
+            }
+            if (ptDONE != nullptr && __builtin_amdgcn_ballot_w64((fired[0] | fired[1] | fired[2] | fired[3]) != 0) != 0) {
+#pragma unroll
+                for (int q = 0; q < 4; ++q) done_events(fired[q], pos[q]);
             }
         }
     };
@@ -1296,18 +1379,20 @@
                 left &= left - 1;
                 const uint32_t rx = (uint32_t)__builtin_amdgcn_readlane((int)l1_run.x, (int)src), ry = (uint32_t)__builtin_amdgcn_readlane((int)l1_run.y, (int)src);
                 const uint32_t rz = (uint32_t)__builtin_amdgcn_readlane((int)l1_run.z, (int)src), rw = (uint32_t)__builtin_amdgcn_readlane((int)l1_run.w, (int)src);
+                uint32_t fired = 0, at = 0;
                 if constexpr (K != 27) {
                     if (lane < 8u && (((rz & 0xFFu) >> lane) & 1u)) {
                         const uint32_t sh2 = 2u * (7u - lane);
-                        slow_count(funnel(ry, rx, sh2), (ry >> sh2) & MASK_HI);
+                        slow_count(funnel(ry, rx, sh2), (ry >> sh2) & MASK_HI, fired, at);
                     }
-                    continue;
+                } else {
+                    const uint32_t v16 = (rz >> 20) | ((rw >> 28) << 12);
+                    if (lane < 16u && ((v16 >> lane) & 1u)) {
+                        const uint32_t sh2 = 2u * (15u - lane);
+                        slow_count(funnel(ry, rx, sh2), funnel(rz, ry, sh2) & MASK_HI, fired, at);
+                    }
                 }
-                const uint32_t v16 = (rz >> 20) | ((rw >> 28) << 12);
-                if (lane < 16u && ((v16 >> lane) & 1u)) {
-                    const uint32_t sh2 = 2u * (15u - lane);
-                    slow_count(funnel(ry, rx, sh2), funnel(rz, ry, sh2) & MASK_HI);
-                }
+                if (ptDONE != nullptr) done_events(fired, at);
             }
         }
         l1_phase = 0;
diff --git a/varigraph_amd/csrc/vgmi_ptable.hip b/varigraph_amd/csrc/vgmi_ptable.hip
--- a/varigraph_amd/csrc/vgmi_ptable.hip
+++ b/varigraph_amd/csrc/vgmi_ptable.hip
@@ -120,6 +120,46 @@
     P[2 * n - 1 - pos] = make_ulonglong2(as_is ? R : K, slot);
 }
 
+__global__ void pt_done_check_kernel(PathView pt, uint32_t k, unsigned long long* out)
+{
+    const uint32_t b = blockIdx.x * blockDim.x + threadIdx.x;
+    if (b >> pt.bucket_log2) return;
+    const unsigned long long* B = pt.index + ((size_t)b << 2);
+    const uint32_t W = k == 27u ? 16u : 8u, flip = pt.Tp - (k == 27u ? 42u : 2u * k - 12u);
+    bool never = (B[0] >> 62 & 1) != 0, all = true;
+    uint32_t pairs = 0;
+    for (int e = 0; e < 2; ++e) {
+        const unsigned long long lo = B[2 * e], hi = B[2 * e + 1];
+        const uint32_t q[4] = {(uint32_t)(lo >> 24) & 0x7FFFFu, (uint32_t)(lo >> 43) & 0x7FFFFu, (uint32_t)hi & 0x7FFFFu, (uint32_t)(hi >> 19) & 0x7FFFFu};
+        if (q[0] == 0) continue;
+        never |= (hi >> 38 & 1) != 0;
+        for (int i = 0; i < 4; ++i) {
+            if (q[i] == 0) continue;
+            for (int m = 0; m < 2; ++m) {
+                const uint32_t at = m ? flip - q[i] : q[i];
+                for (uint32_t x = at; x < at + W; ++x) {
+                    if (!(pt.VB[x >> 5] >> (x & 31u) & 1u)) continue;
+                    ++pairs;
+                    all &= (pt.SB[x >> 5] >> (x & 31u) & 1u) != 0;
+                }
+            }
+        }
+    }
+    const bool can = !never && pairs != 0;
+    const bool marked = pt.DONE && (pt.DONE[b >> 5] >> (b & 31u) & 1u);
+    if (can) atomicAdd(out + 0, 1ULL);
+    if (marked) atomicAdd(out + 1, 1ULL);
+    if (marked && !(can && all)) atomicAdd(out + 2, 1ULL);
+    if (can && all && !marked) atomicAdd(out + 3, 1ULL);
+}
+
+hipError_t launch_ptable_done_check(const PathView& pt, uint32_t k, unsigned long long* out, hipStream_t st)
+{
+    const uint32_t n = 1u << pt.bucket_log2;
+    hipLaunchKernelGGL(pt_done_check_kernel, dim3((n + 255) / 256), dim3(256), 0, st, pt, k, out);
+    return hipGetLastError();
+}
+
 hipError_t launch_ptable_order(const TableView& t, const uint32_t* key_slot, uint64_t n, uint32_t* key_of_slot, uint32_t* link, uint32_t* link2,
                                uint32_t* pos_of_key, unsigned long long* cursor, uint32_t* mark, uint32_t* status, hipStream_t st, uint32_t align)
 {
diff --git a/varigraph_amd/vgmi.py b/varigraph_amd/vgmi.py
--- a/varigraph_amd/vgmi.py
+++ b/varigraph_amd/vgmi.py
@@ -60,6 +60,7 @@
         "vgmi_counts_finish": (i32, [vp, vp, vp, vp]),
         "vgmi_counts_finish_device": (i32, [vp, vp, vp, vp]),
         "vgmi_count_kernel_ms": (i32, [vp, C.POINTER(C.c_float), C.POINTER(u64)]),
+        "vgmi_pt_done_check": (i32, [vp, C.POINTER(u64)]),
         "vgmi_counts_export_device": (i32, [vp, vp]),
         "vgmi_counts_import_device": (i32, [vp, vp]),
         "vgmi_fastq_open": (i32, [vp, C.POINTER(vp)]),
@@ -315,6 +316,11 @@
         self._chk(self._l.vgmi_count_kernel_ms(self._h, C.byref(ms), C.byref(n)))
         return ms.value, n.value
 
+    def pt_done_check(self):
+        out = (C.c_uint64 * 4)()
+        self._chk(self._l.vgmi_pt_done_check(self._h, out))
+        return tuple(int(v) for v in out)
+
     def fastq_text(self, text, piece=None):
         fq = C.c_void_p()
         self._chk(self._l.vgmi_fastq_open(self._h, C.byref(fq)))
```
